# walaj/SeqLib

Hardware: AMD Instinct MI355X
Metric: aligned reads/sec (150 bp) via BWAAligner (higher is better)
Workload: dtype int32

## Files before the change

### seqlib_amd/csrc/dev_chain.h

```cpp
#pragma once
#include "dev_fm.h"
#include "dev_sort.h"
#include "dev_types.h"
#include "dev_pack.h"
#include "dev_kbtree.h"

__device__ __forceinline__ int next_slot(unsigned int *queue, int per_wave = 0)
{
    const int lane = threadIdx.x & 63;
    const unsigned int base = wave_take(queue, per_wave ? 1u : 64u);
    if (per_wave) return lane == 0 ? (int)base : 0x7fffffff;
    return (int)(base + lane);
}

struct ReadWS {
    int64_t *s_rbeg; qp_t *s_ql; int32_t *s_next; int32_t *s_score;
    int64_t *c_pos; int32_t *c_head, *c_tail, *c_n, *c_rid, *c_w, *c_first; int8_t *c_kept;
    int32_t *ia, *ib, *ic; uint64_t *srt;
    DReg *regs; DHit *hits;
    int cap;
    __device__ __forceinline__ int s_qbeg(int s) const { return QP_HI(s_ql[s]); }
    __device__ __forceinline__ int s_len(int s) const { return QP_LO(s_ql[s]); }
};

__device__ __forceinline__ ReadWS make_ws(const Chunk &ck, int r);

__device__ __forceinline__ ReadWS make_ws_uniform(const Chunk &ck, int r)
{
    const uint64_t o = rfl_u64(ck.seed_off[r]);
    ReadWS w;
    w.s_rbeg = ck.s_rbeg + o; w.s_ql = (qp_t *)ck.s_ql + o; w.s_next = ck.s_next + o; w.s_score = ck.s_score ? ck.s_score + o : nullptr;
    w.c_pos = ck.c_pos + o; w.c_head = ck.c_head + o; w.c_tail = ck.c_tail + o; w.c_n = ck.c_n + o;
    w.c_rid = ck.c_rid + o; w.c_w = ck.c_w + o; w.c_first = ck.c_first + o; w.c_kept = ck.c_kept + o;
    w.ia = ck.ia + o; w.ib = ck.ib + o; w.ic = ck.ic + o; w.srt = ck.srt + o;
    w.regs = ck.regs + o; w.hits = ck.hits + o;
    w.cap = (int)(rfl_u64(ck.seed_off[r + 1]) - o);
    return w;
}

__device__ __forceinline__ ReadWS make_ws(const Chunk &ck, int r)
{
    const uint64_t o = ck.seed_off[r];
    ReadWS w;
    w.s_rbeg = ck.s_rbeg + o; w.s_ql = (qp_t *)ck.s_ql + o; w.s_next = ck.s_next + o; w.s_score = ck.s_score ? ck.s_score + o : nullptr;
    w.c_pos = ck.c_pos + o; w.c_head = ck.c_head + o; w.c_tail = ck.c_tail + o; w.c_n = ck.c_n + o;
    w.c_rid = ck.c_rid + o; w.c_w = ck.c_w + o; w.c_first = ck.c_first + o; w.c_kept = ck.c_kept + o;
    w.ia = ck.ia + o; w.ib = ck.ib + o; w.ic = ck.ic + o; w.srt = ck.srt + o;
    w.regs = ck.regs + o; w.hits = ck.hits + o;
    w.cap = (int)(ck.seed_off[r + 1] - o);
    return w;
}

__device__ inline int dev_chain_weight(const ReadWS &w, int c)
{
    int64_t end = 0;
    int wt = 0, tmp;
    for (int s = w.c_head[c]; s >= 0; s = w.s_next[s]) {
        const int qb = w.s_qbeg(s), l = w.s_len(s);
        if (qb >= end) wt += l;
        else if (qb + l > end) wt += (int)(qb + l - end);
        end = end > qb + l ? end : qb + l;
    }
    tmp = wt; wt = 0; end = 0;
    for (int s = w.c_head[c]; s >= 0; s = w.s_next[s]) {
        const int64_t rb = w.s_rbeg[s]; const int l = w.s_len(s);
        if (rb >= end) wt += l;
        else if (rb + l > end) wt += (int)(rb + l - end);
        end = end > rb + l ? end : rb + l;
    }
    wt = wt < tmp ? wt : tmp;
    return wt < 1 << 30 ? wt : (1 << 30) - 1;
}

template <typename I>
__device__ void dev_chain_read(const DevFM<I> &fm, const DevRef &R, const Chunk &ck, const slx_opt &opt, int r)
{
        ReadWS w = make_ws(ck, r);
        const int len = (int)(ck.offs[r + 1] - ck.offs[r]);
        const int n_intv = (int)ck.intv_n[r];
        const qp_t *iinfo = (const qp_t *)ck.intv_info + (size_t)r * ck.cap_intv;
        const I *ix0 = (const I *)ck.intv_x0 + (size_t)r * ck.cap_intv;
        const I *ix2 = (const I *)ck.intv_x2 + (size_t)r * ck.cap_intv;
        int ns = 0, nc = 0;
        int *ord = w.ia;
        KbTree kb;
        bool tree = false;
        int cc = -1, cc_tail = 0, cc_n = 0, cc_rid = 0;
        qp_t cc_fql = 0, cc_lql = 0;
        int64_t cc_frb = 0, cc_lrb = 0;
        for (int i = 0; i < n_intv; ++i) {
            const int qbeg = QP_HI(iinfo[i]), slen = QP_LO(iinfo[i]) - qbeg;
            const I x2 = ix2[i];
            const I step = x2 > (I)opt.max_occ ? x2 / (I)opt.max_occ : (I)1;
            I k = 0;
            for (int count = 0; k < x2 && count < opt.max_occ; k += step, ++count) {
                const int64_t rbeg = intv_pos<I>(fm, ix0[i], k);
                const int rid = dev_intv2rid(R, rbeg, rbeg + slen);
                if (rid < 0) continue;
                int lo = -1, lower_c = -1;
                bool to_add = true;
                if (nc) {
                    if (tree) lower_c = kb.lower(rbeg);
                    else {
                        int b = 0, e = nc;
                        while (b < e) { int m = (b + e) >> 1; if (w.c_pos[ord[m]] < rbeg) b = m + 1; else e = m; }
                        if (b == nc) lo = nc - 1;
                        else lo = rbeg < w.c_pos[ord[b]] ? b - 1 : b;
                        lower_c = lo >= 0 ? ord[lo] : -1;
                    }
                    if (lower_c >= 0) {
                        const int c = lower_c;
                        if (c != cc) {
                            const int first = w.c_head[c];
                            cc = c; cc_tail = w.c_tail[c]; cc_n = w.c_n[c]; cc_rid = w.c_rid[c];
                            cc_fql = w.s_ql[first]; cc_frb = w.s_rbeg[first];
                            cc_lql = w.s_ql[cc_tail]; cc_lrb = w.s_rbeg[cc_tail];
                        }
                        const int last = cc_tail;
                        const int l_qbeg = QP_HI(cc_lql), l_len = QP_LO(cc_lql);
                        const int64_t l_rbeg = cc_lrb;
                        const int64_t qend = l_qbeg + l_len, rend = l_rbeg + l_len;
                        int res;
                        if (rid != cc_rid) res = 0;
                        else if (qbeg >= QP_HI(cc_fql) && qbeg + slen <= qend && rbeg >= cc_frb && rbeg + slen <= rend) res = 1;
                        else if ((l_rbeg < R.l_pac || cc_frb < R.l_pac) && rbeg >= R.l_pac) res = 0;
                        else {
                            const int64_t x = qbeg - l_qbeg, y = rbeg - l_rbeg;
                            if (y >= 0 && x - y <= opt.w && y - x <= opt.w && x - l_len < opt.max_chain_gap && y - l_len < opt.max_chain_gap) {
                                const int s = ns++;
                                const qp_t ql = QP_PACK(qbeg, slen);
                                w.s_rbeg[s] = rbeg; w.s_ql[s] = ql; w.s_next[s] = -1; if (w.s_score) w.s_score[s] = slen;
                                w.s_next[last] = s; w.c_tail[c] = s; w.c_n[c] = ++cc_n;
                                cc_tail = s; cc_lql = ql; cc_lrb = rbeg;
                                res = 1;
                            } else res = 0;
                        }
                        to_add = !res;
                    }
                }
                if (to_add) {
                    const int s = ns++, c = nc;
                    w.s_rbeg[s] = rbeg; w.s_ql[s] = QP_PACK(qbeg, slen); w.s_next[s] = -1; if (w.s_score) w.s_score[s] = slen;
                    w.c_pos[c] = rbeg; w.c_head[c] = w.c_tail[c] = s; w.c_n[c] = 1; w.c_rid[c] = rid;
                    cc = c; cc_tail = s; cc_n = 1; cc_rid = rid; cc_fql = cc_lql = QP_PACK(qbeg, slen); cc_frb = cc_lrb = rbeg;
                    if (!tree && nc == 2 * KB_T - 1) { kb.from_array((int *)w.regs, ord, w.c_pos, nc); tree = true; }
                    if (tree) kb.put(rbeg, c);
                    else {
                        for (int m = nc; m > lo + 1; --m) ord[m] = ord[m - 1];
                        ord[lo + 1] = c;
                    }
                    ++nc;
                }
            }
        }
        if (tree) kb.traverse(ord);
        ck.frac_rep[r] = (float)ck.l_rep[r] / len;
        int n_chn = 0;
        int *a = w.ia;
        for (int i = 0; i < nc; ++i) {
            const int c = a[i];
            w.c_first[c] = -1; w.c_kept[c] = 0;
            w.c_w[c] = dev_chain_weight(w, c);
            if (w.c_w[c] >= opt.min_chain_weight) a[n_chn++] = c;
        }
        int n_out = 0;
        if (n_chn > 0) {
            ks_introsort_idx(n_chn, a, [&](int x, int y) { return w.c_w[x] > w.c_w[y]; });
            int *kept = w.ib, n_kept = 0;
            auto cbeg = [&](int c) { return w.s_qbeg(w.c_head[c]); };
            auto cend = [&](int c) { return w.s_qbeg(w.c_tail[c]) + w.s_len(w.c_tail[c]); };
            w.c_kept[a[0]] = 3;
            kept[n_kept++] = 0;
            for (int i = 1; i < n_chn; ++i) {
                int large_ovlp = 0, k;
                const int ci = a[i];
                for (k = 0; k < n_kept; ++k) {
                    const int j = kept[k], cj = a[j];
                    const int b_max = cbeg(cj) > cbeg(ci) ? cbeg(cj) : cbeg(ci);
                    const int e_min = cend(cj) < cend(ci) ? cend(cj) : cend(ci);
                    if (e_min > b_max && (!ref_is_alt(R, w.c_rid[cj]) || ref_is_alt(R, w.c_rid[ci]))) {
                        const int li = cend(ci) - cbeg(ci), lj = cend(cj) - cbeg(cj);
                        const int min_l = li < lj ? li : lj;
                        if ((float)(e_min - b_max) >= (float)min_l * opt.mask_level && min_l < opt.max_chain_gap) {
                            large_ovlp = 1;
                            if (w.c_first[cj] < 0) w.c_first[cj] = i;
                            if ((float)w.c_w[ci] < (float)w.c_w[cj] * opt.drop_ratio && w.c_w[cj] - w.c_w[ci] >= opt.min_seed_len << 1) break;
                        }
                    }
                }
                if (k == n_kept) { kept[n_kept++] = i; w.c_kept[ci] = large_ovlp ? 2 : 3; }
            }
            for (int i = 0; i < n_kept; ++i) {
                const int c = a[kept[i]];
                if (w.c_first[c] >= 0) w.c_kept[a[w.c_first[c]]] = 1;
            }
            int i, k;
            for (i = k = 0; i < n_chn; ++i) {
                if (w.c_kept[a[i]] == 0 || w.c_kept[a[i]] == 3) continue;
                if (++k >= opt.max_chain_extend) break;
            }
            for (; i < n_chn; ++i) if (w.c_kept[a[i]] < 3) w.c_kept[a[i]] = 0;
            for (i = 0; i < n_chn; ++i) if (w.c_kept[a[i]] != 0) a[n_out++] = a[i];
        }
        const bool flt = ck.s_score && len < ck.log_lut_n && flt_live(opt, len, ck.log_lut[len > 0 ? len : 1], nullptr);
        if (n_out == 1 && opt.w > 0 && !flt) {
            const int c0 = a[0];
            int s_full = -1, cov = 0;
            bool same_diag = true;
            int64_t diag = 0;
            for (int s = w.c_head[c0]; s >= 0; s = w.s_next[s])
                if (w.s_qbeg(s) == 0 && w.s_len(s) == len) { s_full = s; diag = w.s_rbeg[s]; break; }
            if (s_full >= 0) {
                for (int s = w.c_head[c0]; s >= 0; s = w.s_next[s]) {
                    cov += w.s_len(s);
                    if (w.s_rbeg[s] - w.s_qbeg(s) != diag) same_diag = false;
                }
                if (same_diag) {
                    DReg g;
                    g.rb = diag; g.re = g.rb + len; g.qb = 0; g.qe = len; g.rid = w.c_rid[c0];
                    g.score = g.truesc = len * opt.a; g.sub = g.csub = g.sub_n = 0; g.w = opt.w; g.seedcov = cov; g.secondary = 0;
                    g.seedlen0 = len; g.n_comp = 0; g.frac_rep = ck.frac_rep[r]; g.hash = 0;
                    w.regs[0] = g;
                    ck.n_reg[r] = 1;
                    n_out = -1;
                }
            }
        }
        {
            int off = 0;
            for (int i = 0; i < n_out; ++i) {
                const int c = a[i];
                w.c_first[c] = off;
                for (int s = w.c_head[c]; s >= 0; s = w.s_next[s]) w.c_w[off++] = s;
            }
        }
        ck.n_chain[r] = n_out;
}

template <typename I>
__global__ void __launch_bounds__(128) k_chain(DevFM<I> fm, DevRef R, Chunk ck, DevOpt dopt, const int *order, unsigned int *queue, const unsigned int *n_slots, int per_wave)
{
    const slx_opt &opt = dopt.o;
    const int n_todo = (int)*n_slots;
    if (per_wave) __builtin_amdgcn_s_setprio(3);
    while (true) {
        const int slot = next_slot(queue, per_wave);
        if (__all(slot >= n_todo)) break;
        if (slot >= n_todo) continue;
        const int r = order ? order[slot] : slot;
        dev_chain_read<I>(fm, R, ck, opt, r);
    }
}
```

### seqlib_amd/csrc/dev_sort.h

```cpp
#pragma once
#include <hip/hip_runtime.h>

template <typename LT>
__device__ void ks_insertsort_idx(int *s, int *t, LT lt)
{
    for (int *i = s + 1; i < t; ++i)
        for (int *j = i; j > s && lt(*j, *(j - 1)); --j) { int sw = *j; *j = *(j - 1); *(j - 1) = sw; }
}

template <typename LT>
__device__ void ks_combsort_idx(int n, int *a, LT lt)
{
    const double shrink = 1.2473309501039786540366528676643;
    int do_swap, gap = n;
    do {
        if (gap > 2) {
            gap = (int)(gap / shrink);
            if (gap == 9 || gap == 10) gap = 11;
        }
        do_swap = 0;
        for (int *i = a; i < a + n - gap; ++i) {
            int *j = i + gap;
            if (lt(*j, *i)) { int tmp = *i; *i = *j; *j = tmp; do_swap = 1; }
        }
    } while (do_swap || gap > 2);
    if (gap != 1) ks_insertsort_idx(a, a + n, lt);
}

template <typename LT>
__device__ void ks_introsort_idx(int n, int *a, LT lt)
{
    if (n < 1) return;
    if (n == 2) {
        if (lt(a[1], a[0])) { int sw = a[0]; a[0] = a[1]; a[1] = sw; }
        return;
    }
    int d;
    for (d = 2; (1u << d) < (unsigned)n; ++d);
    int st_l[40], st_r[40], st_d[40], top = 0;
    int s = 0, t = n - 1;
    d <<= 1;
    while (true) {
        if (s < t) {
            if (--d == 0) { ks_combsort_idx(t - s + 1, a + s, lt); t = s; continue; }
            int i = s, j = t, k = i + ((j - i) >> 1) + 1;
            if (lt(a[k], a[i])) { if (lt(a[k], a[j])) k = j; }
            else k = lt(a[j], a[i]) ? i : j;
            int rp = a[k];
            if (k != t) { int sw = a[k]; a[k] = a[t]; a[t] = sw; }
            for (;;) {
                do ++i; while (lt(a[i], rp));
                do --j; while (i <= j && lt(rp, a[j]));
                if (j <= i) break;
                int sw = a[i]; a[i] = a[j]; a[j] = sw;
            }
            { int sw = a[i]; a[i] = a[t]; a[t] = sw; }
            if (i - s > t - i) {
                if (i - s > 16) { st_l[top] = s; st_r[top] = i - 1; st_d[top] = d; ++top; }
                s = t - i > 16 ? i + 1 : t;
            } else {
                if (t - i > 16) { st_l[top] = i + 1; st_r[top] = t; st_d[top] = d; ++top; }
                t = i - s > 16 ? i - 1 : s;
            }
        } else {
            if (top == 0) { ks_insertsort_idx(a, a + n, lt); return; }
            --top; s = st_l[top]; t = st_r[top]; d = st_d[top];
        }
    }
}

template <typename LT>
__device__ void std_unguarded_linear_insert(int *a, int last, LT lt)
{
    int val = a[last], next = last - 1;
    while (lt(val, a[next])) { a[last] = a[next]; last = next; --next; }
    a[last] = val;
}

template <typename LT>
__device__ void std_insertion_sort(int *a, int first, int last, LT lt)
{
    if (first == last) return;
    for (int i = first + 1; i != last; ++i) {
        if (lt(a[i], a[first])) {
            int val = a[i];
            for (int k = i; k > first; --k) a[k] = a[k - 1];
            a[first] = val;
        } else std_unguarded_linear_insert(a, i, lt);
    }
}

template <typename LT>
__device__ void std_adjust_heap(int *a, int first, int hole, int len, int value, LT lt)
{
    const int top = hole;
    int child = hole;
    while (child < (len - 1) / 2) {
        child = 2 * (child + 1);
        if (lt(a[first + child], a[first + child - 1])) --child;
        a[first + hole] = a[first + child];
        hole = child;
    }
    if ((len & 1) == 0 && child == (len - 2) / 2) {
        child = 2 * (child + 1);
        a[first + hole] = a[first + child - 1];
        hole = child - 1;
    }
    int parent = (hole - 1) / 2;
    while (hole > top && lt(a[first + parent], value)) {
        a[first + hole] = a[first + parent];
        hole = parent;
        parent = (hole - 1) / 2;
    }
    a[first + hole] = value;
}

template <typename LT>
__device__ void std_heapsort(int *a, int first, int last, LT lt)
{
    int len = last - first;
    if (len >= 2)
        for (int parent = (len - 2) / 2;; --parent) {
            std_adjust_heap(a, first, parent, len, a[first + parent], lt);
            if (parent == 0) break;
        }
    while (last - first > 1) {
        --last;
        int value = a[last];
        a[last] = a[first];
        std_adjust_heap(a, first, 0, last - first, value, lt);
    }
}

template <typename LT>
__device__ void std_sort_idx(int n, int *a, LT lt)
{
    if (n <= 0) return;
    int st_f[48], st_l[48], st_d[48], top = 0;
    int first = 0, last = n, depth = 0;
    for (int m = n; m > 1; m >>= 1) ++depth;
    depth *= 2;
    while (true) {
        while (last - first > 16) {
            if (depth == 0) { std_heapsort(a, first, last, lt); break; }
            --depth;
            int mid = first + (last - first) / 2;
            int ra = first + 1, rb = mid, rc = last - 1, res = first, pick;
            if (lt(a[ra], a[rb])) { if (lt(a[rb], a[rc])) pick = rb; else if (lt(a[ra], a[rc])) pick = rc; else pick = ra; }
            else if (lt(a[ra], a[rc])) pick = ra; else if (lt(a[rb], a[rc])) pick = rc; else pick = rb;
            { int sw = a[res]; a[res] = a[pick]; a[pick] = sw; }
            int f = first + 1, l = last;
            while (true) {
                while (lt(a[f], a[first])) ++f;
                --l;
                while (lt(a[first], a[l])) --l;
                if (!(f < l)) break;
                int sw = a[f]; a[f] = a[l]; a[l] = sw;
                ++f;
            }
            int cut = f;
            st_f[top] = cut; st_l[top] = last; st_d[top] = depth; ++top;
            last = cut;
        }
        if (top == 0) break;
        --top; first = st_f[top]; last = st_l[top]; depth = st_d[top];
    }
    if (n > 16) {
        std_insertion_sort(a, 0, 16, lt);
        for (int i = 16; i < n; ++i) std_unguarded_linear_insert(a, i, lt);
    } else std_insertion_sort(a, 0, n, lt);
}
```

### seqlib_amd/csrc/slx_align.hip

```cpp
#include <hip/hip_runtime.h>
#include <hipcub/hipcub.hpp>
#include <chrono>
#include <cmath>
#include <functional>
#include <unistd.h>
#include <cstdio>
#include <cstdlib>
#include <cstring>
#include <algorithm>
#include <mutex>
#include <string>
#include <thread>
#include <type_traits>
#include <vector>
#include "slx_internal.h"
#include "dev_seed4.h"
#include "dev_fin.h"
#include "dev_ext_wave.h"
#include "dev_ext_reg.h"
#include "dev_ext_lane.h"
#include "dev_ext_block.h"
#include "dev_ext_seg.h"
#include "dev_fin2.h"
#include "dev_chain_coop.h"
#include "dev_long.h"
#include "dev_cig_lane.h"
#include "dev_cig_band.h"
#include "dev_cig_seg.h"

#include "slx_align_types.h"

static const char *STAGE_NAMES[SLX_N_STAGES] = {"encode", "seed", "scan", "chain", "extend", "finalize", "compact", "total"};
extern "C" const char *slx_stage_name(int i) { return i >= 0 && i < SLX_N_STAGES ? STAGE_NAMES[i] : ""; }

#define SLX_BOUNCE_BYTES (256u << 10)
#define SLX_PACK_PARTS 13
struct PackSpec { const unsigned char *src[SLX_PACK_PARTS]; unsigned int bytes[SLX_PACK_PARTS], at[SLX_PACK_PARTS]; int n; long long hdr[4]; };
__global__ void k_pack_small(PackSpec s, unsigned char *dst)
{
    const unsigned int t = blockIdx.x * blockDim.x + threadIdx.x, nt = gridDim.x * blockDim.x;
    if (t < 32 && s.hdr[0] >= 0) dst[t] = ((const unsigned char *)s.hdr)[t];
    for (int i = 0; i < s.n; ++i)
        for (unsigned int b = t; b < s.bytes[i]; b += nt) dst[s.at[i] + b] = s.src[i][b];
}

__global__ void k_len_stats(const uint64_t *offs, int n, unsigned long long *stat)
{
    const int i = blockIdx.x * blockDim.x + threadIdx.x;
    unsigned long long len = 0;
    bool bad = false;
    if (i < n) {
        const uint64_t a = offs[i], b = offs[i + 1];
        if (b < a) bad = true; else len = b - a;
        if (i == 0) stat[2] = a;
        if (i == n - 1) stat[3] = b;
    }
    for (int o = 32; o; o >>= 1) { const unsigned long long t = __shfl_xor(len, o, 64); len = len > t ? len : t; }
    if ((threadIdx.x & 63) == 0 && len > __hip_atomic_load(stat, __ATOMIC_RELAXED, __HIP_MEMORY_SCOPE_AGENT)) atomicMax(stat, len);
    if (bad) atomicOr(stat + 1, 1ull);
}

template <typename I>
__global__ void k_sa_seed(DevFM<I> fm, I *dense, uint64_t n_sa)
{
    uint64_t j = (uint64_t)blockIdx.x * blockDim.x + threadIdx.x;
    if (j >= n_sa) return;
    dense[j * (uint64_t)fm.sa_intv] = j == 0 ? fm.seq_len : (I)fm.sa_samp[j];
}

template <typename I>
__global__ void k_sa_walk(DevFM<I> fm, I *dense, uint64_t n_sa)
{
    uint64_t j = (uint64_t)blockIdx.x * blockDim.x + threadIdx.x;
    if (j >= n_sa) return;
    I k = (I)(j * (uint64_t)fm.sa_intv);
    I v = j == 0 ? fm.seq_len : (I)fm.sa_samp[j];
    const I mask = (I)fm.sa_intv - 1;
    while (true) {
        if (k == fm.primary) break;
        I x = k - (k > fm.primary ? 1 : 0);
        const uint32_t *blk = fm.bwt + ((size_t)(x >> 7) << 4) + 8;
        int jj = (int)(x & 127);
        int c = (blk[jj >> 4] >> ((~jj & 15) << 1)) & 3;
        I tk[4], tl[4];
        occ4_pair<I>(fm, k, k, tk, tl);
        k = fm.L2[c] + tk[c];
        --v;
        if ((k & mask) == 0) break;
        dense[k] = v;
    }
}

template <typename I>
static int build_lut(slx_aligner *al)
{
    DevFM<I> &fm = fm_of<I>(al);
    fm.lut = nullptr; fm.lut_k = 0;
    int K = al->lut_k;
    if (K < 0) {
        int l4 = 0;
        while ((al->host_idx->seq_len >> (2 * (l4 + 1))) != 0) ++l4;
        K = l4 - 1 > 14 ? 14 : l4 - 1;
    }
    if (K < 2) return SLX_OK;
    const uint64_t n = 1ull << (2 * K);
    int rc;
    if ((rc = al->d_lut.ensure(n * sizeof(LutE<I>))) != SLX_OK) return rc;
    hipLaunchKernelGGL(k_kmer_lut<I>, dim3((unsigned)((n + 255) / 256)), dim3(256), 0, al->stream, fm, K, al->d_lut.as<LutE<I>>());
    HIPCHK(hipGetLastError());
    HIPCHK(slx_wait_stream(al->stream));
    fm.lut = al->d_lut.p; fm.lut_k = K;
    return SLX_OK;
}

template <typename I>
static int upload_fm(slx_aligner *al)
{
    const slx_index *idx = al->host_idx;
    int rc;
    DevFM<I> &fm = fm_of<I>(al);
    memset(&fm, 0, sizeof fm);
    fm.bwt = al->d_bwt.as<uint32_t>();
    {
        const uint64_t n_blocks = ((idx->seq_len ? idx->seq_len - 1 : 0) >> 6) + 1;
        const size_t occ_bytes = (n_blocks + 1) * 32;
        if ((rc = al->d_occ.ensure(occ_bytes)) != SLX_OK) return rc;
        HIPCHK(hipMemsetAsync(al->d_occ.p, 0, occ_bytes, al->stream));
        const uint64_t *sup = nullptr;
        if (sizeof(I) == 8) {
            const uint64_t n_sup = (idx->seq_len >> 32) + 1;
            if ((rc = al->d_sup.ensure(n_sup * 32 + 32)) != SLX_OK) return rc;
            hipLaunchKernelGGL(k_occ_sup, dim3((unsigned)((n_sup * 4 + 63) / 64)), dim3(64), 0, al->stream, al->d_bwt.as<uint32_t>(), n_sup, al->d_sup.as<uint64_t>());
            sup = al->d_sup.as<uint64_t>();
        }
        hipLaunchKernelGGL(k_occ_build, dim3((unsigned)((n_blocks + 255) / 256)), dim3(256), 0, al->stream, al->d_bwt.as<uint32_t>(), (uint64_t)idx->seq_len,
                           al->d_occ.as<uint4>(), n_blocks, sup);
        HIPCHK(hipGetLastError());
        HIPCHK(slx_wait_stream(al->stream));
        fm.occ = al->d_occ.as<uint4>();
        fm.sup = sup;
    }
    fm.primary = (I)idx->primary;
    for (int i = 0; i < 5; ++i) fm.L2[i] = (I)idx->L2[i];
    fm.seq_len = (I)idx->seq_len;
    if ((rc = build_lut<I>(al)) != SLX_OK) return rc;
    fm.sa_dense = nullptr;
    fm.sa_samp = al->d_sa_samp.as<uint64_t>();
    fm.sa_intv = idx->sa_intv;
    const uint64_t n1 = idx->seq_len + 1;
    al->have_dense = false;
    if ((rc = al->d_sa_dense.ensure(n1 * sizeof(I))) != SLX_OK) return rc;
    if (sizeof(I) == 4 && idx->dense_sa32.size() == n1) {
        HIPCHK(hipMemcpy(al->d_sa_dense.p, idx->dense_sa32.data(), n1 * 4, hipMemcpyHostToDevice));
    } else {
        const uint64_t n_sa = idx->sa.size();
        const int bs = 256;
        hipLaunchKernelGGL(k_sa_seed<I>, dim3((unsigned)((n_sa + bs - 1) / bs)), dim3(bs), 0, al->stream, fm, al->d_sa_dense.as<I>(), n_sa);
        hipLaunchKernelGGL(k_sa_walk<I>, dim3((unsigned)((n_sa + bs - 1) / bs)), dim3(bs), 0, al->stream, fm, al->d_sa_dense.as<I>(), n_sa);
        HIPCHK(hipGetLastError());
        HIPCHK(slx_wait_stream(al->stream));
    }
    al->have_dense = true;
    return SLX_OK;
}

template <typename I>
static int build_rep_filter(slx_aligner *al)
{
    al->rep_mask = 0;
    if (al->rep_k <= 0 || al->rep_k > 31 || !al->have_dense || al->host_idx->seq_len < 1024) return SLX_OK;
    uint64_t bits = 1ull << 20;
    while (bits < al->host_idx->seq_len * 8ull) bits <<= 1;
    while (al->d_rep.ensure(bits / 8) != SLX_OK) {
        (void)hipGetLastError();
        bits >>= 1;
        if (bits < al->host_idx->seq_len || bits < (1ull << 20)) { al->d_rep.release(); return SLX_OK; }
    }
    HIPCHK(hipMemsetAsync(al->d_rep.p, 0, bits / 8, al->stream));
    DevFM<I> fm = fm_of<I>(al);
    fm.sa_dense = al->d_sa_dense.as<I>();
    hipLaunchKernelGGL(k_rep_filter<I>, dim3(al->n_cu * 64), dim3(256), 0, al->stream, fm, al->ref, al->rep_k, al->d_rep.as<uint32_t>(), bits - 1);
    HIPCHK(hipGetLastError());
    HIPCHK(slx_wait_stream(al->stream));
    al->rep_mask = bits - 1;
    return SLX_OK;
}

#define SLX_MAX_WORKERS 8
static int env_hw_queues() { const char *e = getenv("GPU_MAX_HW_QUEUES"); const int v = e ? atoi(e) : 0; return v > 0 ? v : 4; }

static int default_workers()
{
    if (const char *e = getenv("SEQLIB_AMD_WORKERS")) { const int v = atoi(e); if (v >= 1 && v <= SLX_MAX_WORKERS) return v; }
    return 3;
}

static int make_worker_stream(slx_aligner *al, Worker *wk)
{
    if (al->stream_prio) {
        int least = 0, greatest = 0;
        HIPCHK(hipDeviceGetStreamPriorityRange(&least, &greatest));
        HIPCHK(hipStreamCreateWithPriority(&wk->stream, hipStreamNonBlocking, greatest));
    } else HIPCHK(hipStreamCreateWithFlags(&wk->stream, hipStreamNonBlocking));
    return SLX_OK;
}

static int set_seed_stream(slx_aligner *al, Worker *wk)
{
    if (wk->seed_stream) { HIPCHK(slx_wait_stream(wk->seed_stream)); HIPCHK(hipStreamDestroy(wk->seed_stream)); wk->seed_stream = nullptr; }
    if (al->seed_free_cus <= 0) return SLX_OK;
    const int words = (al->n_cu + 31) / 32;
    std::vector<uint32_t> mask((size_t)words, 0u);
    for (int cu = 0; cu < al->n_cu; ++cu)
        if ((cu & 31) < 32 - al->seed_free_cus) mask[(size_t)(cu >> 5)] |= 1u << (cu & 31);
    HIPCHK(hipExtStreamCreateWithCUMask(&wk->seed_stream, (uint32_t)words, mask.data()));
    if (!wk->ev_seed_in) HIPCHK(hipEventCreateWithFlags(&wk->ev_seed_in, hipEventDisableTiming));
    if (!wk->ev_seed_out) HIPCHK(hipEventCreateWithFlags(&wk->ev_seed_out, hipEventDisableTiming));
    return SLX_OK;
}

static int add_worker(slx_aligner *al)
{
    Worker *wk = new Worker();
    wk->id = (int)al->workers.size();
    wk->collect();
    al->workers.push_back(wk);
    { const int rc = make_worker_stream(al, wk); if (rc != SLX_OK) return rc; }
    { const int rc = set_seed_stream(al, wk); if (rc != SLX_OK) return rc; }
    HIPCHK(hipHostMalloc((void **)&wk->h_mail, 256, hipHostMallocDefault));
    for (int b = 0; b < 6; ++b) HIPCHK(hipEventCreate(&wk->dbg_ev[b]));
    for (int i = 0; i <= SLX_N_STAGES; ++i) HIPCHK(hipEventCreate(&wk->ev[i]));
    for (int i = 0; i < 6; ++i) HIPCHK(hipEventCreate(&wk->ev_probe[i]));
    return SLX_OK;
}

static int aligner_init(slx_aligner *al, const slx_index *idx, const int *devices, int n_dev)
{
    al->device = (devices && n_dev > 0) ? devices[0] : 0;
    if (!(devices && n_dev > 0)) (void)hipGetDevice(&al->device);
    HIPCHK(hipSetDevice(al->device));
    hipDeviceProp_t prop;
    HIPCHK(hipGetDeviceProperties(&prop, al->device));
    al->n_cu = prop.multiProcessorCount;
    al->max_threads = al->n_cu * al->threads_per_cu;
    int rcw;
    al->n_workers = default_workers();
    al->hw_queues = env_hw_queues();
    for (int k = 0; k < al->n_workers; ++k) if ((rcw = add_worker(al)) != SLX_OK) return rcw;
    HIPCHK(hipStreamCreateWithFlags(&al->stream, hipStreamNonBlocking));
    al->host_idx = idx;
    int rc;
    if ((rc = al->d_bwt.ensure(idx->bwt.size() * 4 + 64)) != SLX_OK) return rc;
    HIPCHK(hipMemcpy(al->d_bwt.p, idx->bwt.data(), idx->bwt.size() * 4, hipMemcpyHostToDevice));
    if ((rc = al->d_sa_samp.ensure(idx->sa.size() * 8)) != SLX_OK) return rc;
    HIPCHK(hipMemcpy(al->d_sa_samp.p, idx->sa.data(), idx->sa.size() * 8, hipMemcpyHostToDevice));
    al->wide = idx->seq_len + 1 >= (1ULL << 32);
    if ((rc = al->wide ? upload_fm<uint64_t>(al) : upload_fm<uint32_t>(al)) != SLX_OK) return rc;
    if ((rc = al->d_pac.ensure(idx->pac.size() + 16)) != SLX_OK) return rc;
    HIPCHK(hipMemcpy(al->d_pac.p, idx->pac.data(), idx->pac.size(), hipMemcpyHostToDevice));
    std::vector<int64_t> aoff; std::vector<int32_t> alen;
    for (const slx_ann &a : idx->anns) { aoff.push_back(a.offset); alen.push_back(a.len); }
    if ((rc = al->d_ann_off.ensure(aoff.size() * 8 + 8)) != SLX_OK) return rc;
    if ((rc = al->d_ann_len.ensure(alen.size() * 4 + 8)) != SLX_OK) return rc;
    HIPCHK(hipMemcpy(al->d_ann_off.p, aoff.data(), aoff.size() * 8, hipMemcpyHostToDevice));
    HIPCHK(hipMemcpy(al->d_ann_len.p, alen.data(), alen.size() * 4, hipMemcpyHostToDevice));
    al->ref.pac = al->d_pac.as<uint8_t>();
    al->ref.l_pac = idx->l_pac;
    al->ref.n_seqs = (int)idx->anns.size();
    al->ref.ann_off = al->d_ann_off.as<int64_t>();
    al->ref.ann_len = al->d_ann_len.as<int32_t>();
    {
        std::vector<uint8_t> alt;
        bool any = false;
        for (const slx_ann &a : idx->anns) { alt.push_back(a.is_alt ? 1 : 0); any = any || a.is_alt; }
        al->ref.ann_alt = nullptr;
        if (any) {
            if ((rc = al->d_ann_alt.ensure(alt.size() + 8)) != SLX_OK) return rc;
            HIPCHK(hipMemcpy(al->d_ann_alt.p, alt.data(), alt.size(), hipMemcpyHostToDevice));
            al->ref.ann_alt = al->d_ann_alt.as<uint8_t>();
        }
    }
    if ((rc = al->wide ? build_rep_filter<uint64_t>(al) : build_rep_filter<uint32_t>(al)) != SLX_OK) return rc;
    const int LUT_N = SLX_LOG_LUT_N;
    std::vector<double> lut((size_t)LUT_N);
    lut[0] = -INFINITY;
    for (int i = 1; i < LUT_N; ++i) lut[(size_t)i] = log((double)i);
    if ((rc = al->d_loglut.ensure((size_t)LUT_N * 8)) != SLX_OK) return rc;
    HIPCHK(hipMemcpy(al->d_loglut.p, lut.data(), (size_t)LUT_N * 8, hipMemcpyHostToDevice));
    return SLX_OK;
}


static std::mutex g_live_mu;
static int g_live_aligners = 0;
static void pin_pool_release_all();

static int create_one(const slx_index *idx, int device, bool current, slx_aligner **out)
{
    slx_aligner *al = new slx_aligner();
    { std::lock_guard<std::mutex> g(g_live_mu); ++g_live_aligners; }
    const int rc = aligner_init(al, idx, current ? nullptr : &device, current ? 0 : 1);
    if (rc != SLX_OK) { slx_aligner_free(al); return rc; }
    *out = al;
    return SLX_OK;
}

extern "C" int slx_device_count(void)
{
    int ndev = 0;
    if (hipGetDeviceCount(&ndev) != hipSuccess) { (void)hipGetLastError(); return 0; }
    return ndev;
}

extern "C" int slx_aligner_create(const slx_index *idx, const int *devices, int n_dev, slx_aligner **out)
{
    if (!out) return SLX_EINVAL;
    *out = nullptr;
    if (!idx) { slx_set_error("slx_aligner_create: index is null"); return SLX_EINVAL; }
    const int ndev = slx_device_count();
    if (ndev == 0) {
        slx_set_error("no HIP device: the BWAAligner hot path runs on MI355X only (no CPU fallback)");
        return SLX_ENODEVICE;
    }
    if (n_dev < 0 || (n_dev > 0 && !devices)) { slx_set_error("slx_aligner_create: bad device list"); return SLX_EINVAL; }
    for (int i = 0; i < n_dev; ++i)
        if (devices[i] < 0 || devices[i] >= ndev) { slx_set_error("slx_aligner_create: device %d is not one of the %d visible", devices[i], ndev); return SLX_EINVAL; }
    if (n_dev <= 1) return create_one(idx, n_dev ? devices[0] : 0, n_dev == 0, out);
    slx_aligner *grp = new slx_aligner();
    grp->is_group = true;
    grp->subs.assign((size_t)n_dev, nullptr);
    grp->host_idx = idx;
    std::vector<int> rcs((size_t)n_dev, SLX_OK);
    std::vector<std::string> errs((size_t)n_dev);
    std::vector<std::thread> th;
    for (int i = 0; i < n_dev; ++i)
        th.emplace_back([&, i]() {
            rcs[(size_t)i] = create_one(idx, devices[i], false, &grp->subs[(size_t)i]);
            if (rcs[(size_t)i] != SLX_OK) errs[(size_t)i] = slx_last_error();
        });
    for (auto &t : th) t.join();
    for (int i = 0; i < n_dev; ++i)
        if (rcs[(size_t)i] != SLX_OK) {
            slx_set_error("device %d: %s", devices[i], errs[(size_t)i].c_str());
            const int rc = rcs[(size_t)i];
            slx_aligner_free(grp);
            return rc;
        }
    *out = grp;
    return SLX_OK;
}

extern "C" void slx_aligner_free(slx_aligner *al)
{
    if (!al) return;
    if (al->is_group) {
        for (slx_aligner *sub : al->subs) slx_aligner_free(sub);
        delete al;
        return;
    }
    (void)hipSetDevice(al->device);
    DevBuf *bufs[] = {&al->d_bwt, &al->d_occ, &al->d_sup, &al->d_lut, &al->d_rep, &al->d_sa_samp, &al->d_sa_dense, &al->d_pac, &al->d_ann_off, &al->d_ann_len, &al->d_ann_alt, &al->d_loglut, &al->o_hit_off,
                      &al->o_rid, &al->o_pos, &al->o_flag, &al->o_mapq, &al->o_score, &al->o_nm, &al->o_na, &al->o_ncig, &al->o_cig_off, &al->o_cigar, &al->o_xa, &al->o_sub,
                      &al->st_bases, &al->st_offs, &al->st_pack};
    for (DevBuf *b : bufs) b->release();
    for (Worker *wk : al->workers) {
        for (DevBuf *b : wk->all) b->release();
        for (int i = 0; i <= SLX_N_STAGES; ++i) if (wk->ev[i]) (void)hipEventDestroy(wk->ev[i]);
        for (int i = 0; i < 6; ++i) if (wk->dbg_ev[i]) (void)hipEventDestroy(wk->dbg_ev[i]);
        for (int i = 0; i < 6; ++i) if (wk->ev_probe[i]) (void)hipEventDestroy(wk->ev_probe[i]);
        if (wk->h_mail) (void)hipHostFree(wk->h_mail);
        if (wk->stream) (void)hipStreamDestroy(wk->stream);
        if (wk->seed_stream) (void)hipStreamDestroy(wk->seed_stream);
        if (wk->ev_seed_in) (void)hipEventDestroy(wk->ev_seed_in);
        if (wk->ev_seed_out) (void)hipEventDestroy(wk->ev_seed_out);
        delete wk;
    }
    if (al->h_bounce) (void)hipHostFree(al->h_bounce);
    if (al->stream) (void)hipStreamDestroy(al->stream);
    delete al;
    bool last;
    { std::lock_guard<std::mutex> g(g_live_mu); last = --g_live_aligners == 0; }
    if (last) pin_pool_release_all();
}

extern "C" int slx_aligner_set(slx_aligner *al, const char *key, int64_t value)
{
    if (!al || !key) return SLX_EINVAL;
    if (al->is_group) {
        std::lock_guard<std::mutex> call(al->call_mu);
        for (slx_aligner *sub : al->subs) { const int rc = slx_aligner_set(sub, key, value); if (rc != SLX_OK) return rc; }
        return SLX_OK;
    }
    std::lock_guard<std::mutex> call(al->call_mu);
    if (!strcmp(key, "chunk_reads")) { if (value < 1) return SLX_EINVAL; al->chunk_reads = value; }
    else if (!strcmp(key, "cap_intv")) { if (value < 1) return SLX_EINVAL; al->cap_intv = (int)value; }
    else if (!strcmp(key, "dense_sa")) al->dense_sa = value != 0;
    else if (!strcmp(key, "wide_index")) {
        const bool want = value != 0 || al->host_idx->seq_len + 1 >= (1ULL << 32);
        if (want != al->wide) {
            HIPCHK(hipSetDevice(al->device));
            al->wide = want;
            int rc = want ? upload_fm<uint64_t>(al) : upload_fm<uint32_t>(al);
            if (rc != SLX_OK) return rc;
            if ((rc = want ? build_rep_filter<uint64_t>(al) : build_rep_filter<uint32_t>(al)) != SLX_OK) return rc;
        }
    }
    else if (!strcmp(key, "chain_mode")) al->chain_mode = (int)value;
    else if (!strcmp(key, "keep_stages")) al->keep_stages = (int)value;
    else if (!strcmp(key, "lut_k")) {
        if (value != 0 && value != -1 && (value < 2 || value > 14)) return SLX_EINVAL;
        al->lut_k = (int)value;
        (void)hipSetDevice(al->device);
        return al->wide ? build_lut<uint64_t>(al) : build_lut<uint32_t>(al);
    }
    else if (!strcmp(key, "cand_mode")) al->cand_mode = (int)value;
    else if (!strcmp(key, "cand_seeds")) { if (value < 1) return SLX_EINVAL; al->cand_seeds = (int)value; }
    else if (!strcmp(key, "heavy_sorted")) al->heavy_sorted = (int)value;
    else if (!strcmp(key, "ext_split")) al->ext_split = (int)value;
    else if (!strcmp(key, "coop_lim1")) { if (value < 1) return SLX_EINVAL; al->coop_lim1 = (int)value; }
    else if (!strcmp(key, "coop_lim2")) { if (value < 1) return SLX_EINVAL; al->coop_lim2 = (int)value; }
    else if (!strcmp(key, "long_coop")) al->long_coop = value != 0;
    else if (!strcmp(key, "long_seed3")) al->long_seed3 = value != 0;
    else if (!strcmp(key, "long_predict")) al->long_predict = value != 0;
    else if (!strcmp(key, "long_block")) { if (value < 0 || value > (1 << 24)) return SLX_EINVAL; al->long_block = (int)value; }
    else if (!strcmp(key, "long_guess")) al->long_guess = value != 0;
    else if (!strcmp(key, "long_seg")) al->long_seg = value != 0;
    else if (!strcmp(key, "bwd_direct")) al->bwd_direct = value != 0;
    else if (!strcmp(key, "xseg_wave_min")) { if (value < 0) return SLX_EINVAL; al->xseg_wave_min = (int)value; }
    else if (!strcmp(key, "xseg_fail")) { if (value < 0) return SLX_EINVAL; al->xseg_fail = (int)value; }
    else if (!strcmp(key, "long_budget")) { if (value < 0 || value > (1 << 20)) return SLX_EINVAL; al->long_budget = (int)value; }
    else if (!strcmp(key, "regs_big")) { if (value < 2) return SLX_EINVAL; al->regs_big = (int)value; }
    else if (!strcmp(key, "regs_defer")) al->regs_defer = value != 0;
    else if (!strcmp(key, "hits_wave")) al->hits_wave = value != 0;
    else if (!strcmp(key, "cig_fast_coop")) al->cig_fast_coop = value != 0;
    else if (!strcmp(key, "cig_lane_il")) al->cig_lane_il = value != 0;
    else if (!strcmp(key, "small_coop")) al->small_coop = value != 0;
    else if (!strcmp(key, "small_spread")) al->small_spread = value != 0;
    else if (!strcmp(key, "chain_sorted")) al->chain_sorted = value != 0;
    else if (!strcmp(key, "regs_sorted")) al->regs_sorted = value != 0;
    else if (!strcmp(key, "cand_top")) { if (value < 0) return SLX_EINVAL; al->cand_top = (int)value; }
    else if (!strcmp(key, "cand_rep_max")) { if (value < 0) return SLX_EINVAL; al->cand_rep_max = (int)value; }
    else if (!strcmp(key, "cand_rep")) { if (value < -1 || value > 101) return SLX_EINVAL; al->cand_rep = (int)value; }
    else if (!strcmp(key, "cand_lanes")) { if (value < -1 || value > 1) return SLX_EINVAL; al->cand_lanes = (int)value; }
    else if (!strcmp(key, "cig_lanes")) al->cig_lanes = value != 0;
    else if (!strcmp(key, "first_diag")) al->first_diag = value != 0;
    else if (!strcmp(key, "first_lanes")) al->first_lanes = value != 0;
    else if (!strcmp(key, "lane_narrow")) al->lane_narrow = value != 0;
    else if (!strcmp(key, "lane_pad")) al->lane_pad = (int)value;
    else if (!strcmp(key, "cand_lane_seeds")) { if (value < 1) return SLX_EINVAL; al->cand_lane_seeds = (int)value; }
    else if (!strcmp(key, "cand_cap")) { if (value < 1) return SLX_EINVAL; al->cand_cap = (int)value; }
    else if (!strcmp(key, "split_min")) al->split_min = (int)value;
    else if (!strcmp(key, "heavy_seeds")) { if (value < 1) return SLX_EINVAL; al->heavy_seeds = (int)value; }
    else if (!strcmp(key, "workers")) {
        if (value < 1 || value > SLX_MAX_WORKERS) return SLX_EINVAL;
        HIPCHK(hipSetDevice(al->device));
        while ((int)al->workers.size() < (int)value) { const int rc = add_worker(al); if (rc != SLX_OK) return rc; }
        al->n_workers = (int)value;
    }
    else if (!strcmp(key, "min_split")) { if (value < 1) return SLX_EINVAL; al->min_split = value; }
    else if (!strcmp(key, "seed_quota")) { if (value < 0 || value > (1 << 24)) return SLX_EINVAL; al->seed_quota = (int)value; }
    else if (!strcmp(key, "rep_k")) {
        if (value < 0 || value > 31) return SLX_EINVAL;
        al->rep_k = (int)value;
        HIPCHK(hipSetDevice(al->device));
        return al->wide ? build_rep_filter<uint64_t>(al) : build_rep_filter<uint32_t>(al);
    }
    else if (!strcmp(key, "top_heavy")) al->top_heavy = value != 0;
    else if (!strcmp(key, "top_reuse")) al->top_reuse = value != 0;
    else if (!strcmp(key, "p2_items")) al->p2_items = value != 0;
    else if (!strcmp(key, "p2_coop")) al->p2_coop = value != 0;
    else if (!strcmp(key, "p2_items_cap")) al->p2_items_cap = (int)value;
    else if (!strcmp(key, "seed_free_cus")) {
        if (value < 0 || value > 24) return SLX_EINVAL;
        HIPCHK(hipSetDevice(al->device));
        al->seed_free_cus = (int)value;
        for (Worker *wk : al->workers) { const int rc = set_seed_stream(al, wk); if (rc != SLX_OK) return rc; }
    }
    else if (!strcmp(key, "stream_prio")) {
        if (value < 0 || value > 1) return SLX_EINVAL;
        HIPCHK(hipSetDevice(al->device));
        al->stream_prio = (int)value;
        for (Worker *wk : al->workers) {
            HIPCHK(slx_wait_stream(wk->stream));
            HIPCHK(hipStreamDestroy(wk->stream));
            wk->stream = nullptr;
            const int rc = make_worker_stream(al, wk);
            if (rc != SLX_OK) return rc;
        }
    }
    else if (!strcmp(key, "threads")) { if (value < 64) return SLX_EINVAL; al->max_threads = (int)value; }
    else if (!strcmp(key, "zarena_bytes")) { if (value < 1024) return SLX_EINVAL; al->zcap = (unsigned long long)value; }
    else { slx_set_error("slx_aligner_set: unknown key %s", key); return SLX_EINVAL; }
    return SLX_OK;
}

extern "C" int slx_aligner_stage_ms(const slx_aligner *al, float ms[SLX_N_STAGES])
{
    if (!al || !ms) return SLX_EINVAL;
    if (al->is_group) {
        for (int i = 0; i < SLX_N_STAGES; ++i) { ms[i] = 0; for (const slx_aligner *sub : al->subs) ms[i] = std::max(ms[i], sub->stage_ms[i]); }
        return SLX_OK;
    }
    for (int i = 0; i < SLX_N_STAGES; ++i) ms[i] = al->stage_ms[i];
    return SLX_OK;
}

extern "C" int slx_aligner_probe_ms(const slx_aligner *al, float ms[SLX_N_PROBES], int64_t *n_reads)
{
    if (!al || !ms) return SLX_EINVAL;
    if (al->is_group) {
        int64_t n = 0;
        for (int i = 0; i < SLX_N_PROBES; ++i) ms[i] = 0;
        for (const slx_aligner *sub : al->subs) { for (int i = 0; i < SLX_N_PROBES; ++i) ms[i] += sub->probe_ms[i]; n += sub->probe_reads; }
        if (n_reads) *n_reads = n;
        return SLX_OK;
    }
    for (int i = 0; i < SLX_N_PROBES; ++i) ms[i] = al->probe_ms[i];
    if (n_reads) *n_reads = al->probe_reads;
    return SLX_OK;
}

extern "C" int64_t slx_aligner_counter(const slx_aligner *al, const char *key)
{
    if (!al || !key) return -1;
    if (!strcmp(key, "workers")) return al->is_group ? al->subs[0]->n_workers : al->n_workers;
    if (!strcmp(key, "hw_queues")) return al->hw_queues;
    if (!strcmp(key, "long_rounds") || !strcmp(key, "long_jobs")) {
        long long v = 0;
        const bool rounds = key[5] == 'r';
        auto take = [&](const slx_aligner *a) { for (const Worker *wk : a->workers) v = std::max(v, rounds ? (long long)wk->long_rounds_run : (long long)wk->long_jobs_run); };
        if (al->is_group) for (const slx_aligner *sub : al->subs) take(sub); else take(al);
        return v;
    }
    {
        if (!strcmp(key, "pseg_jobs")) {
            long long v = 0;
            auto take = [&](const slx_aligner *a) { for (const Worker *wk : a->workers) v += wk->pseg_stat; };
            if (al->is_group) for (const slx_aligner *sub : al->subs) take(sub); else take(al);
            return v;
        }
        if (!strcmp(key, "retries")) {
            long long v = 0;
            if (al->is_group) for (const slx_aligner *sub : al->subs) v += sub->n_retries; else v = al->n_retries;
            return v;
        }
        if (!strcmp(key, "regs_deferred") || !strcmp(key, "hits_wave_reads")) {
            long long v = 0;
            const int which = key[0] == 'h';
            auto take = [&](const slx_aligner *a) { for (const Worker *wk : a->workers) v += (long long)wk->fin_stat[which]; };
            if (al->is_group) for (const slx_aligner *sub : al->subs) take(sub); else take(al);
            return v;
        }
        static const char *const gs[3] = {"gseg_ok", "gseg_redo", "gseg_jobs"};
        for (int i = 0; i < 3; ++i)
            if (!strcmp(key, gs[i])) {
                long long v = 0;
                auto take = [&](const slx_aligner *a) { for (const Worker *wk : a->workers) v += wk->gseg_stat[i]; };
                if (al->is_group) for (const slx_aligner *sub : al->subs) take(sub); else take(al);
                return v;
            }
        static const char *const xs[4] = {"xseg_ok", "xseg_redo", "xseg_retry", "xseg_sides"};
        for (int i = 0; i < 4; ++i)
            if (!strcmp(key, xs[i])) {
                long long v = 0;
                auto take = [&](const slx_aligner *a) { for (const Worker *wk : a->workers) v += wk->xseg_stat[i]; };
                if (al->is_group) for (const slx_aligner *sub : al->subs) take(sub); else take(al);
                return v;
            }
    }
    if (!strcmp(key, "group_merge_us")) return al->merge_us;
    if (!strcmp(key, "group_call_us")) return al->call_us;
    static const char *const names[4] = {"heavy_reads", "p2_calls", "p2_coop_calls", "p2_whole_reads"};
    for (int i = 0; i < 4; ++i)
        if (!strcmp(key, names[i])) {
            if (!al->is_group) return al->counters[i];
            long long n = 0;
            for (const slx_aligner *sub : al->subs) n += sub->counters[i];
            return n;
        }
    return -1;
}

extern "C" int slx_aligner_probe_launches(const slx_aligner *al)
{
    if (!al) return 0;
    if (al->is_group) { int n = 0; for (const slx_aligner *sub : al->subs) n += sub->probe_launches; return n; }
    return al->probe_launches;
}

#include "slx_chunk.inc"


__global__ void k_shift_offsets(int64_t *dst, const int64_t *src, int64_t n, int64_t add)
{
    int64_t i = (int64_t)blockIdx.x * blockDim.x + threadIdx.x;
    if (i < n) dst[i] = src[i] + add;
}

template <typename I>
static int worker_run(slx_aligner *al, Worker *wk, const slx_opt *opt, const uint8_t *d_bases, const uint64_t *d_offs, int64_t r_lo, int64_t r_hi,
                      uint64_t rng_state, uint64_t first_ordinal, int hardclip, double keepSecFrac, int maxSecondary, const char *h_bases, const uint64_t *h_offs)
{
    HIPCHK(hipSetDevice(al->device));
    if (h_offs && r_hi > r_lo) {
        const uint64_t b0 = h_offs[r_lo], b1 = h_offs[r_hi];
        if (b0 < al->h_first || b1 < b0 || b1 > al->h_last) { slx_set_error("read offsets are not monotonic (part [%lld, %lld))", (long long)r_lo, (long long)r_hi); return SLX_EINVAL; }
        if (b1 > b0) HIPCHK(hipMemcpyAsync((void *)(d_bases + b0), h_bases + b0, b1 - b0, hipMemcpyHostToDevice, wk->stream));
        HIPCHK(hipMemcpyAsync((void *)(d_offs + r_lo), h_offs + r_lo, ((size_t)(r_hi - r_lo) + 1) * 8, hipMemcpyHostToDevice, wk->stream));
    }
    for (int i = 0; i < SLX_N_STAGES; ++i) wk->stage_ms[i] = 0;
    for (int i = 0; i < SLX_N_PROBES; ++i) wk->probe_ms[i] = 0;
    wk->n_chunks = 0;
    for (long long &c : wk->cnt) c = 0;
    int rc;
    const int64_t n_part = r_hi - r_lo;
    if ((rc = wk->o_hit_off.ensure(((size_t)n_part + 1) * 8)) != SLX_OK) return rc;
    if ((rc = wk->len_stat.ensure(32)) != SLX_OK) return rc;
    int64_t hit_base = 0, cig_base = 0;
    for (int64_t r0 = r_lo, step = 0; r0 < r_hi; r0 += step) {
        const int n = (int)std::min<int64_t>(al->chunk_reads, r_hi - r0);
        step = n;
        unsigned long long stat[4] = {0, 0, 0, 0};
        HIPCHK(hipMemsetAsync(wk->len_stat.p, 0, 32, wk->stream));
        hipLaunchKernelGGL(k_len_stats, dim3((unsigned)((n + 255) / 256)), dim3(256), 0, wk->stream, d_offs + r0, n, wk->len_stat.as<unsigned long long>());
        { MailSpec ms{}; ms.src[0] = wk->len_stat.as<unsigned int>(); ms.words[0] = 8; ms.n = 1;
          hipLaunchKernelGGL(k_mail, dim3(1), dim3(64), 0, wk->stream, ms, wk->h_mail); }
        HIPCHK(slx_wait_stream(wk->stream));
        memcpy(stat, wk->h_mail, 32);
        if (stat[1]) { slx_set_error("read offsets are not monotonic in reads [%lld, %lld)", (long long)r0, (long long)(r0 + n)); return SLX_EINVAL; }
        const int max_len = (int)std::min<unsigned long long>(stat[0], 1u << 30);
        if (max_len > SLX_MAX_READ_LEN) {
            slx_set_error("read of %d bp: the GPU path supports reads up to %d bp", max_len, SLX_MAX_READ_LEN);
            return SLX_EUNSUPPORTED;
        }
        uint64_t pair[2] = {stat[2], stat[3]};
        ChunkCaps caps;
        {
            std::lock_guard<std::mutex> g(al->mu);
            caps.cap_intv = al->cap_intv;
            caps.zcap = std::max<unsigned long long>(al->zcap, (unsigned long long)n * al->z_per_read);
            if (max_len > 704) {
                caps.cap_intv = std::max(std::max(caps.cap_intv, al->cap_intv_long), max_len / 8 + 64);
                caps.zcap = std::max(caps.zcap, std::min<unsigned long long>((unsigned long long)n * (unsigned long long)max_len * 208ull, 4ull << 30));
            }
            caps.cigcap = std::max<unsigned long long>(al->cig_floor, (unsigned long long)n * al->cig_per_read + 4096);
        }
        const unsigned long long lane_blocks = (unsigned long long)std::min<long long>((long long)al->n_cu * 16, (long long)n * 4 / 64 + 1);
        const unsigned long long z_waves = (unsigned long long)std::min(n, al->n_cu * 32) * CIG_WAVE_Z +
                                           (al->cig_lane_il ? lane_blocks * ((unsigned long long)LANE_IL_WORDS(max_len) * 256ull + 255ull) : 0ull);
        const unsigned long long cig_waves = (unsigned long long)std::min(n, al->n_cu * 32) * CIG_WAVE_WORDS;
        caps.zcap += z_waves; caps.cigcap += cig_waves;
        for (int attempt = 0;; ++attempt) {
            uint32_t fl = 0;
            int64_t hb = hit_base, cb = cig_base;
            if (max_len > SLX_NARROW_MAX_LEN)
                rc = sizeof(I) == 8 ? slx_run_chunk_wide_u64(al, wk, opt, d_bases, d_offs, pair, r0, r_lo, n, max_len, rng_state, first_ordinal, hardclip, keepSecFrac, maxSecondary,
                                                             caps, &hb, &cb, &fl)
                                    : slx_run_chunk_wide_u32(al, wk, opt, d_bases, d_offs, pair, r0, r_lo, n, max_len, rng_state, first_ordinal, hardclip, keepSecFrac, maxSecondary,
                                                             caps, &hb, &cb, &fl);
            else
            rc = run_chunk<I>(al, wk, opt, d_bases, d_offs, pair, r0, r_lo, n, max_len, rng_state, first_ordinal, hardclip, keepSecFrac, maxSecondary,
                              caps, &hb, &cb, &fl);
            if (rc != SLX_OK) return rc;
            if (!fl) {
                hit_base = hb; cig_base = cb;
                ++wk->n_chunks;
                std::lock_guard<std::mutex> g(al->mu);
                if (max_len > 704) al->cap_intv_long = std::max(al->cap_intv_long, caps.cap_intv);
                else al->cap_intv = std::max(al->cap_intv, caps.cap_intv);
                if (attempt > 0) {
                    if (n >= 65536) {
                        al->z_per_read = std::max<unsigned long long>(al->z_per_read, (caps.zcap - z_waves + n - 1) / (unsigned long long)n);
                        al->cig_per_read = std::max<unsigned long long>(al->cig_per_read, (caps.cigcap - cig_waves + n - 1) / (unsigned long long)n);
                    } else {
                        al->zcap = std::max(al->zcap, caps.zcap - z_waves);
                        al->cig_floor = std::max(al->cig_floor, caps.cigcap - cig_waves);
                    }
                }
                al->n_retries += attempt;
                break;
            }
            if (getenv("SLX_DEBUG_RETRY")) fprintf(stderr, "[retry] worker %d reads %lld+%d attempt %d flags 0x%x (cap_intv %d zcap %llu cigcap %llu)\n", wk->id,
                                                   (long long)r0, n, attempt, fl, caps.cap_intv, caps.zcap, caps.cigcap);
            if (fl & (ERR_LOGLUT | ERR_INTERNAL)) { slx_set_error("device pipeline error flags 0x%x", fl); return SLX_EINTERNAL; }
            if (attempt >= 12) { slx_set_error("chunk still overflows its work areas after %d retries (flags 0x%x)", attempt, fl); return SLX_ENOMEM; }
            if (fl & OVF_INTV) caps.cap_intv *= 2;
            if (fl & OVF_ZARENA) caps.zcap *= 2;
            if (fl & OVF_CIGAR) caps.cigcap *= 2;
        }
    }
    {
        int64_t last[1] = {hit_base};
        HIPCHK(hipMemcpyAsync(wk->o_hit_off.as<int64_t>() + n_part, last, 8, hipMemcpyHostToDevice, wk->stream));
        if ((rc = wk->o_cig_off.grow(((size_t)hit_base + 2) * 8, (size_t)hit_base * 8, wk->stream)) != SLX_OK) return rc;
        int64_t lastc[1] = {cig_base};
        HIPCHK(hipMemcpyAsync(wk->o_cig_off.as<int64_t>() + hit_base, lastc, 8, hipMemcpyHostToDevice, wk->stream));
        HIPCHK(slx_wait_stream(wk->stream));
    }
    wk->n_hits = hit_base; wk->n_cig = cig_base;
    return SLX_OK;
}

struct EventPair {
    hipEvent_t t0 = nullptr, t1 = nullptr;
    ~EventPair() { if (t0) (void)hipEventDestroy(t0); if (t1) (void)hipEventDestroy(t1); }
};

static int align_device_locked(slx_aligner *al, const slx_opt *opt, const void *d_bases, const void *d_offs_, int64_t n_reads,
                               uint64_t rng_state, uint64_t first_ordinal, int hardclip, double keepSecFrac, int maxSecondary, slx_hits *out,
                               const char *h_bases = nullptr, const uint64_t *h_offs = nullptr)
{
    memset(out, 0, sizeof *out);
    HIPCHK(hipSetDevice(al->device));
    if (opt->e_del <= 0 || opt->e_ins <= 0) { slx_set_error("gap extension penalty must be > 0 on the GPU path (bwa divides by it)"); return SLX_EINVAL; }
    const uint64_t *d_offs = (const uint64_t *)d_offs_;
    const int K = (n_reads >= 2 * al->min_split) ? std::min<int>(al->n_workers, (int)al->workers.size()) : 1;
    al->active_k = K;
    EventPair tp;
    HIPCHK(hipEventCreate(&tp.t0)); HIPCHK(hipEventCreate(&tp.t1));
    HIPCHK(hipEventRecord(tp.t0, al->stream));
    HIPCHK(slx_wait_stream(al->stream));
    std::vector<int64_t> lo((size_t)K + 1);
    for (int k = 0; k <= K; ++k) lo[(size_t)k] = n_reads * k / K;
    const bool wide = al->wide;
    const bool sam = (opt->flag & SLX_F_REG2SAM) != 0;
    auto run_worker = [=](Worker *wk, int64_t a, int64_t b) {
        return wide ? worker_run<uint64_t>(al, wk, opt, (const uint8_t *)d_bases, d_offs, a, b, rng_state, first_ordinal, hardclip, keepSecFrac, maxSecondary, h_bases, h_offs)
                    : worker_run<uint32_t>(al, wk, opt, (const uint8_t *)d_bases, d_offs, a, b, rng_state, first_ordinal, hardclip, keepSecFrac, maxSecondary, h_bases, h_offs);
    };
    if (K == 1) {
        Worker *wk = al->workers[0];
        wk->rc = run_worker(wk, 0, n_reads);
        if (wk->rc != SLX_OK) return wk->rc;
    } else {
        std::vector<std::thread> th;
        for (int k = 0; k < K; ++k) {
            Worker *wk = al->workers[(size_t)k];
            const int64_t a = lo[(size_t)k], b = lo[(size_t)k + 1];
            th.emplace_back([=]() {
                wk->rc = run_worker(wk, a, b);
                if (wk->rc != SLX_OK) wk->err = slx_last_error();
            });
        }
        for (auto &t : th) t.join();
        for (int k = 0; k < K; ++k)
            if (al->workers[(size_t)k]->rc != SLX_OK) { slx_set_error("%s", al->workers[(size_t)k]->err.c_str()); return al->workers[(size_t)k]->rc; }
    }
    for (int i = 0; i < SLX_N_STAGES; ++i) {
        al->stage_ms[i] = 0;
        for (int k = 0; k < K; ++k) al->stage_ms[i] += al->workers[(size_t)k]->stage_ms[i];
    }
    al->probe_reads = n_reads;
    al->probe_launches = 0;
    for (int k = 0; k < K; ++k) al->probe_launches += al->workers[(size_t)k]->n_chunks;
    for (int i = 0; i < 4; ++i) { al->counters[i] = 0; for (int k = 0; k < K; ++k) al->counters[i] += al->workers[(size_t)k]->cnt[i]; }
    for (int i = 0; i < SLX_N_PROBES; ++i) {
        al->probe_ms[i] = 0;
        for (int k = 0; k < K; ++k) al->probe_ms[i] += al->workers[(size_t)k]->probe_ms[i];
    }
    slx_hits r;
    memset(&r, 0, sizeof r);
    r.n_reads = n_reads; r.on_device = 1;
    if (K == 1) {
        Worker *wk = al->workers[0];
        r.n_hits = wk->n_hits; r.n_cigar = wk->n_cig;
        r.hit_off = wk->o_hit_off.as<int64_t>(); r.rid = wk->o_rid.as<int32_t>(); r.pos = wk->o_pos.as<int64_t>();
        r.flag = wk->o_flag.as<uint16_t>(); r.mapq = wk->o_mapq.as<uint8_t>(); r.score = wk->o_score.as<int32_t>();
        r.nm = wk->o_nm.as<int32_t>(); r.na = wk->o_na.as<int32_t>(); r.n_cigar_ops = wk->o_ncig.as<int32_t>();
        r.cig_off = wk->o_cig_off.as<int64_t>(); r.cigar = wk->o_cigar.as<uint32_t>();
        if (sam) { r.xa_parent = wk->o_xa.as<int32_t>(); r.sub = wk->o_sub.as<int32_t>(); }
    } else {
        int64_t H = 0, C = 0;
        for (int k = 0; k < K; ++k) { H += al->workers[(size_t)k]->n_hits; C += al->workers[(size_t)k]->n_cig; }
        int rc;
#define ENSO(buf, bytes) if ((rc = al->buf.ensure((size_t)(bytes))) != SLX_OK) return rc
        ENSO(o_hit_off, ((size_t)n_reads + 1) * 8); ENSO(o_rid, ((size_t)H + 1) * 4); ENSO(o_pos, ((size_t)H + 1) * 8); ENSO(o_flag, ((size_t)H + 1) * 2);
        ENSO(o_mapq, (size_t)H + 1); ENSO(o_score, ((size_t)H + 1) * 4); ENSO(o_nm, ((size_t)H + 1) * 4); ENSO(o_na, ((size_t)H + 1) * 4);
        ENSO(o_ncig, ((size_t)H + 1) * 4); ENSO(o_cig_off, ((size_t)H + 2) * 8); ENSO(o_cigar, ((size_t)C + 1) * 4);
        if (sam) { ENSO(o_xa, ((size_t)H + 1) * 4); ENSO(o_sub, ((size_t)H + 1) * 4); }
#undef ENSO
        int64_t hb = 0, cb = 0;
        hipStream_t st = al->stream;
        for (int k = 0; k < K; ++k) {
            Worker *wk = al->workers[(size_t)k];
            const int64_t np = lo[(size_t)k + 1] - lo[(size_t)k], h = wk->n_hits, c = wk->n_cig;
            const int last = k == K - 1 ? 1 : 0;
            hipLaunchKernelGGL(k_shift_offsets, dim3((unsigned)((np + last + 255) / 256)), dim3(256), 0, st, al->o_hit_off.as<int64_t>() + lo[(size_t)k],
                               wk->o_hit_off.as<int64_t>(), np + last, hb);
            hipLaunchKernelGGL(k_shift_offsets, dim3((unsigned)((h + last + 255) / 256)), dim3(256), 0, st, al->o_cig_off.as<int64_t>() + hb,
                               wk->o_cig_off.as<int64_t>(), h + last, cb);
#define CAT(buf, type, cnt, base) if ((cnt) > 0) HIPCHK(hipMemcpyAsync(al->buf.as<type>() + (base), wk->buf.as<type>(), (size_t)(cnt) * sizeof(type), hipMemcpyDeviceToDevice, st))
            CAT(o_rid, int32_t, h, hb); CAT(o_pos, int64_t, h, hb); CAT(o_flag, uint16_t, h, hb); CAT(o_mapq, uint8_t, h, hb); CAT(o_score, int32_t, h, hb);
            CAT(o_nm, int32_t, h, hb); CAT(o_na, int32_t, h, hb); CAT(o_ncig, int32_t, h, hb); CAT(o_cigar, uint32_t, c, cb);
            if (sam) { CAT(o_xa, int32_t, h, hb); CAT(o_sub, int32_t, h, hb); }
#undef CAT
            hb += h; cb += c;
        }
        HIPCHK(hipGetLastError());
        r.n_hits = H; r.n_cigar = C;
        r.hit_off = al->o_hit_off.as<int64_t>(); r.rid = al->o_rid.as<int32_t>(); r.pos = al->o_pos.as<int64_t>();
        r.flag = al->o_flag.as<uint16_t>(); r.mapq = al->o_mapq.as<uint8_t>(); r.score = al->o_score.as<int32_t>();
        r.nm = al->o_nm.as<int32_t>(); r.na = al->o_na.as<int32_t>(); r.n_cigar_ops = al->o_ncig.as<int32_t>();
        r.cig_off = al->o_cig_off.as<int64_t>(); r.cigar = al->o_cigar.as<uint32_t>();
        if (sam) { r.xa_parent = al->o_xa.as<int32_t>(); r.sub = al->o_sub.as<int32_t>(); }
    }
    HIPCHK(hipEventRecord(tp.t1, al->stream));
    HIPCHK(slx_wait_stream(al->stream));
    float tot = 0;
    (void)hipEventElapsedTime(&tot, tp.t0, tp.t1);
    al->stage_ms[7] = tot;
    *out = r;
    return SLX_OK;
}

extern "C" int slx_align_batch_device(slx_aligner *al, const slx_opt *opt, const void *d_bases, const void *d_offs, int64_t n_reads,
                                      uint64_t rng_state, uint64_t first_ordinal, int hardclip, double keepSecFrac, int maxSecondary,
                                      slx_hits *out)
{
    if (!al || !opt || !out || n_reads < 0) { slx_set_error("slx_align_batch_device: bad argument"); return SLX_EINVAL; }
    if (al->is_group) { slx_set_error("slx_align_batch_device: reads resident on one GPU cannot be sharded -- use one aligner per device, or slx_align_batch"); return SLX_EINVAL; }
    std::lock_guard<std::mutex> call(al->call_mu);
    return align_device_locked(al, opt, d_bases, d_offs, n_reads, rng_state, first_ordinal, hardclip, keepSecFrac, maxSecondary, out);
}

namespace {
struct PinBlock { void *p; uint64_t cap; };
std::mutex g_pin_mu;
std::vector<PinBlock> g_pin_pool;
const size_t PIN_KEEP = 4;
const uint64_t PIN_KEEP_BYTES = 8ull << 30;
void *pin_acquire(uint64_t bytes, uint64_t *cap)
{
    {
        std::lock_guard<std::mutex> g(g_pin_mu);
        size_t best = g_pin_pool.size();
        for (size_t i = 0; i < g_pin_pool.size(); ++i)
            if (g_pin_pool[i].cap >= bytes && (best == g_pin_pool.size() || g_pin_pool[i].cap < g_pin_pool[best].cap)) best = i;
        if (best < g_pin_pool.size()) { void *p = g_pin_pool[best].p; *cap = g_pin_pool[best].cap; g_pin_pool.erase(g_pin_pool.begin() + (long)best); return p; }
    }
    void *p = nullptr;
    const uint64_t want = bytes + bytes / 16;
    if (hipHostMalloc(&p, want, hipHostMallocPortable | hipHostMallocMapped) != hipSuccess) { (void)hipGetLastError(); return nullptr; }
    *cap = want;
    return p;
}
void pin_release(void *p, uint64_t cap)
{
    {
        std::lock_guard<std::mutex> g(g_pin_mu);
        uint64_t held = cap;
        for (const PinBlock &b : g_pin_pool) held += b.cap;
        bool alive;
        { std::lock_guard<std::mutex> g2(g_live_mu); alive = g_live_aligners > 0; }
        if (alive && g_pin_pool.size() < PIN_KEEP && held <= PIN_KEEP_BYTES) { g_pin_pool.push_back({p, cap}); return; }
    }
    (void)hipHostFree(p);
}
}
static void pin_pool_release_all()
{
    std::vector<PinBlock> drop;
    { std::lock_guard<std::mutex> g(g_pin_mu); drop.swap(g_pin_pool); }
    for (const PinBlock &b : drop) (void)hipHostFree(b.p);
}

extern "C" void *slx_host_alloc(uint64_t bytes)
{
    void *p = nullptr;
    if (hipHostMalloc(&p, bytes ? bytes : 1, hipHostMallocDefault) != hipSuccess) { (void)hipGetLastError(); slx_set_error("cannot pin %llu bytes of host memory", (unsigned long long)bytes); return nullptr; }
    return p;
}
extern "C" void slx_host_free(void *p) { if (p) (void)hipHostFree(p); }
extern "C" void slx_host_trim(void) { pin_pool_release_all(); }

static uint64_t packed_base(uint64_t N, uint64_t H, uint64_t Cg) { return 32 + 8 * (N + 1) + 8 * H + 8 * (H + 1) + 5 * 4 * H + 4 * Cg + 2 * H + H; }
static uint64_t packed_size(uint64_t N, uint64_t H, uint64_t Cg, bool sam = false) { const uint64_t b = packed_base(N, H, Cg); return sam ? ((b + 3) & ~3ull) + 8 * H : b; }

static int pack_locked(slx_aligner *al, const slx_hits *h, void *dst);

static void view_packed(slx_hits *out, uint8_t *blk, int64_t N, int64_t H, int64_t C, bool sam = false)
{
    uint8_t *d = blk + 32;
    out->hit_off = (int64_t *)d; d += 8 * ((size_t)N + 1);
    out->pos = (int64_t *)d; d += 8 * (size_t)H;
    out->cig_off = (int64_t *)d; d += 8 * ((size_t)H + 1);
    out->rid = (int32_t *)d; d += 4 * (size_t)H;
    out->score = (int32_t *)d; d += 4 * (size_t)H;
    out->nm = (int32_t *)d; d += 4 * (size_t)H;
    out->na = (int32_t *)d; d += 4 * (size_t)H;
    out->n_cigar_ops = (int32_t *)d; d += 4 * (size_t)H;
    out->cigar = (uint32_t *)d; d += 4 * (size_t)C;
    out->flag = (uint16_t *)d; d += 2 * (size_t)H;
    out->mapq = (uint8_t *)d;
    out->xa_parent = out->sub = nullptr;
    if (sam) {
        uint8_t *e = blk + ((packed_base((uint64_t)N, (uint64_t)H, (uint64_t)C) + 3) & ~3ull);
        out->xa_parent = (int32_t *)e; out->sub = (int32_t *)(e + 4 * (size_t)H);
    }
}

static int align_host_locked(slx_aligner *al, const slx_opt *opt, const char *bases, const uint64_t *offs, int64_t n_reads, uint64_t rng_state,
                             uint64_t first_ordinal, int hardclip, double keepSecFrac, int maxSecondary, slx_hits *dv);

static int group_align_batch(slx_aligner *grp, const slx_opt *opt, const char *bases, const uint64_t *offs, int64_t n_reads, uint64_t rng_state,
                             uint64_t first_ordinal, int hardclip, double keepSecFrac, int maxSecondary, slx_hits *out)
{
    std::lock_guard<std::mutex> call(grp->call_mu);
    const auto t_call = std::chrono::steady_clock::now();
    const int G = (int)grp->subs.size();
    std::vector<int64_t> lo((size_t)G + 1);
    for (int g = 0; g <= G; ++g) lo[(size_t)g] = n_reads * g / G;
    std::vector<slx_hits> part((size_t)G);
    std::vector<int> rcs((size_t)G, SLX_OK);
    std::vector<std::string> errs((size_t)G);
    for (auto &h : part) memset(&h, 0, sizeof h);
    auto on_all = [&](const std::function<int(int)> &fn) {
// ... 275 lines not shown
```

### seqlib_amd/csrc/slx_align_types.h

```cpp
#pragma once
#include <hip/hip_runtime.h>
#include <mutex>
#include <string>
#include <vector>
#include "slx_internal.h"
#include "dev_fm.h"
#include "dev_types.h"

#define HIPCHK(x)                                                                                   \
    do {                                                                                            \
        hipError_t e_ = (x);                                                                        \
        if (e_ != hipSuccess) {                                                                     \
            slx_set_error("HIP error %s at %s:%d (%s)", hipGetErrorString(e_), __FILE__, __LINE__, #x); \
            return e_ == hipErrorOutOfMemory ? SLX_ENOMEM : SLX_ENODEVICE;                          \
        }                                                                                           \
    } while (0)

struct DevBuf {
    void *p = nullptr;
    size_t cap = 0;
    int ensure(size_t bytes)
    {
        if (bytes <= cap) return SLX_OK;
        if (p) (void)hipFree(p);
        p = nullptr; cap = 0;
        size_t want = bytes + bytes / 8 + 256;
        HIPCHK(hipMalloc(&p, want));
        cap = want;
        return SLX_OK;
    }
    int grow(size_t bytes, size_t keep, hipStream_t st)
    {
        if (bytes <= cap) return SLX_OK;
        void *q = nullptr;
        size_t want = bytes + bytes / 2 + 256;
        HIPCHK(hipMalloc(&q, want));
        if (p && keep) {
            hipError_t e = hipMemcpyAsync(q, p, keep, hipMemcpyDeviceToDevice, st);
            if (e == hipSuccess) e = hipStreamSynchronize(st);
            if (e != hipSuccess) { (void)hipFree(q); HIPCHK(e); }
        }
        if (p) (void)hipFree(p);
        p = q; cap = want;
        return SLX_OK;
    }
    void release() { if (p) (void)hipFree(p); p = nullptr; cap = 0; }
    template <typename T> T *as() const { return (T *)p; }
};

#define SLX_MAIL_PARTS 6
struct MailSpec { const unsigned int *src[SLX_MAIL_PARTS]; int words[SLX_MAIL_PARTS]; int n; };
static __global__ void k_mail(MailSpec s, unsigned int *dst)
{
    int at = 0;
    for (int i = 0; i < s.n; ++i) {
        for (int w = (int)threadIdx.x; w < s.words[i]; w += (int)blockDim.x) dst[at + w] = s.src[i][w];
        at += s.words[i];
    }
}
struct slx_aligner;
#define SMALL_SPREAD_MAX 512

struct Worker {
    hipStream_t stream = nullptr;
    hipStream_t seed_stream = nullptr;
    hipEvent_t ev_seed_in = nullptr, ev_seed_out = nullptr;
    unsigned int *h_mail = nullptr;
    DevBuf codes, offs_rel, intv_n, intv_info, intv_x0, intv_x2, l_rep, seed_cnt, seed_off, scan_tmp;
    DevBuf s_rbeg, s_ql, s_next, c_pos, c_head, c_tail, c_n, c_rid, c_w, c_first, c_kept, ia, ib, ic, srt, regs, hits;
    DevBuf n_chain, n_reg, n_hit, na, frac_rep, zarena, cigpool, counters, lists, hit_cnt, cig_cnt, hit_off_c, cig_off_c;
    DevBuf order_key_in, order_key_out, order_in, order_out, queues, sort_tmp, jobs, fast_list, dp_list, part_flag, part_pos, cand, cand_base,
        cand_cnt, cand_off, dbg_cyc, order_tmp, first_tab, first_cnt, first_off, fb_list, first_jobs, len_stat, s_score, long_list, long_scratch, huge_rows;
    DevBuf order_bin, bin_cnt;
    DevBuf defer_list, hits_big;
    DevBuf first_sorted, first_bins;
    DevBuf p2mask, p2list, p2items, p2long, lane_jobs, first_dp, cig_lane_list;
    DevBuf job_key_in, job_key_out, job_val_in, job_val_out, job_sort_tmp;
    DevBuf seed3_buf;
    DevBuf memo_idx, memo_jobs, memo_tab, round_list, todo_a, todo_b, spec_cnt;
    int long_rounds_run = 0; unsigned int long_jobs_run = 0;
    DevBuf xseg_jobs, xseg_state, xseg_units, xseg_out, xseg_wrec, xseg_wout, xseg_scratch, xseg_cnt;
    DevBuf gseg_jobs, gseg_units, gseg_wrec, gseg_wout, gseg_scratch, gseg_cnt;
    DevBuf pseg_jobs, pseg_idx, pseg_cnt;
    unsigned long long fin_stat[2] = {0, 0};
    unsigned int pseg_stat = 0;
    unsigned int gseg_stat[3] = {0, 0, 0};
    unsigned int xseg_stat[4] = {0, 0, 0, 0};
    DevBuf snap_ia, snap_regs, snap_nreg;
    Chunk last_ck;
    size_t last_S1 = 0;
    bool last_valid = false, last_wide = false;
    int id = 0;
    unsigned int max_seed_cnt = 0;
    hipEvent_t dbg_ev[6] = {nullptr, nullptr, nullptr, nullptr, nullptr, nullptr};
    DevBuf o_hit_off, o_rid, o_pos, o_flag, o_mapq, o_score, o_nm, o_na, o_ncig, o_cig_off, o_cigar, o_xa, o_sub;
    hipEvent_t ev[SLX_N_STAGES + 1];
    hipEvent_t ev_probe[6] = {nullptr, nullptr, nullptr, nullptr, nullptr, nullptr};
    float stage_ms[SLX_N_STAGES];
    float probe_ms[SLX_N_PROBES] = {0, 0, 0, 0, 0, 0};
    int n_chunks = 0;
    long long cnt[4] = {0, 0, 0, 0};
    int64_t n_hits = 0, n_cig = 0;
    int rc = SLX_OK;
    std::string err;
    std::vector<DevBuf *> all;
    void collect()
    {
        all = {&codes, &offs_rel, &intv_n, &intv_info, &intv_x0, &intv_x2, &l_rep, &seed_cnt, &seed_off, &scan_tmp, &s_rbeg, &s_ql, &s_next,
               &c_pos, &c_head, &c_tail, &c_n, &c_rid, &c_w, &c_first, &c_kept, &ia, &ib, &ic, &srt, &regs, &hits, &n_chain, &n_reg, &n_hit,
               &na, &frac_rep, &zarena, &cigpool, &counters, &lists, &hit_cnt, &cig_cnt, &hit_off_c, &cig_off_c, &order_key_in,
               &order_key_out, &order_in, &order_out, &queues, &sort_tmp, &jobs, &fast_list, &dp_list, &part_flag, &part_pos, &cand, &cand_base,
               &cand_cnt, &cand_off, &dbg_cyc, &order_tmp, &first_tab, &first_cnt, &first_off, &fb_list, &first_jobs, &len_stat, &s_score, &long_list, &long_scratch, &huge_rows, &p2mask, &p2list, &p2items, &p2long, &lane_jobs, &first_dp, &first_sorted, &first_bins, &cig_lane_list, &defer_list, &hits_big, &order_bin, &bin_cnt, &snap_ia, &snap_regs, &snap_nreg,
               &memo_idx, &memo_jobs, &memo_tab, &round_list, &todo_a, &todo_b, &spec_cnt, &seed3_buf, &job_key_in, &job_key_out, &job_val_in, &job_val_out, &job_sort_tmp, &pseg_jobs, &pseg_idx, &pseg_cnt, &gseg_jobs, &gseg_units, &gseg_wrec, &gseg_wout, &gseg_scratch, &gseg_cnt, &xseg_jobs, &xseg_state, &xseg_units, &xseg_out, &xseg_wrec, &xseg_wout, &xseg_scratch, &xseg_cnt,
               &o_hit_off, &o_rid, &o_pos, &o_flag, &o_mapq, &o_score, &o_nm, &o_na, &o_ncig, &o_cig_off, &o_cigar, &o_xa, &o_sub};
        for (auto &e : ev) e = nullptr;
    }
};

struct slx_aligner {
    std::vector<slx_aligner *> subs;
    bool is_group = false;
    int64_t merge_us = 0, call_us = 0;
    int device = 0;
    hipStream_t stream = nullptr;
    DevBuf d_bwt, d_occ, d_sup, d_lut, d_rep, d_sa_samp, d_sa_dense, d_pac, d_ann_off, d_ann_len, d_ann_alt, d_loglut;
    uint64_t rep_mask = 0;
    int rep_k = 19;
    bool wide = false;
    DevFM<uint32_t> fm32;
    DevFM<uint64_t> fm64;
    DevRef ref;
    bool dense_sa = true;
    bool have_dense = false;
    const slx_index *host_idx = nullptr;
    int64_t chunk_reads = 1 << 24;
    int cap_intv = 40;
    int cap_intv_long = 0;
    int long_predict = 0;
    int long_block = 32768;
    int long_seed3 = 1;
    int long_coop = 1;
    int bwd_direct = 0;
    int long_seg = 1;
    int xseg_wave_min = 2048;
    int xseg_fail = 0;
    int long_guess = 0;
    int long_budget = 1024;
    int regs_sorted = 0;
    int chain_sorted = 0;
    int small_spread = 1;
    int cig_fast_coop = 1;
    int cig_lane_il = 1;
    int hits_wave = 1;
    int small_coop = 1;
    int regs_defer = 1;
    int regs_big = 48;
    int coop_lim1 = 1 << 30, coop_lim2 = 1 << 30;
    int ext_split = 1;
    int heavy_sorted = 1;
    int cand_lanes = -1;
    int cand_lane_seeds = 64;
    int cig_lanes = 1;
    int first_lanes = 1;
    int first_diag = 1;
    int lane_narrow = 1;
    int lane_pad = 0;
    int cand_mode = 1;
    int cand_seeds = 256;
    int cand_top = 512;
    int cand_rep = -1;
    int cand_rep_max = 4096;
    int cand_cap = 1 << 23;
    int lut_k = -1;
    int keep_stages = 0;
    int chain_mode = 1;
    int heavy_seeds = 64;
    int split_min = 4096;
    int seed_quota = 0;
    int top_heavy = 0;
    int p2_items = 1;
    int p2_coop = 1;
    int p2_items_cap = 0;
    int top_reuse = 1;
    int seed_free_cus = 0;
    int stream_prio = 0;
    int n_workers = 3;
    int hw_queues = 4;
    int active_k = 1;
    int64_t min_split = 1 << 18;
    int max_threads = 0;
    int threads_per_cu = 1536;
    int n_cu = 256;
    unsigned long long zcap = 1ull << 26;
    unsigned long long z_per_read = 512;
    unsigned long long cig_per_read = 8;
    unsigned long long cig_floor = 0;
    int n_retries = 0;
    std::mutex mu;
    std::mutex call_mu;
    std::vector<Worker *> workers;
    DevBuf o_hit_off, o_rid, o_pos, o_flag, o_mapq, o_score, o_nm, o_na, o_ncig, o_cig_off, o_cigar, o_xa, o_sub;
    DevBuf st_bases, st_offs, st_pack;
    unsigned char *h_bounce = nullptr;
    float stage_ms[SLX_N_STAGES];
    float probe_ms[SLX_N_PROBES] = {0, 0, 0, 0, 0, 0};
    int64_t probe_reads = 0;
    long long counters[4] = {0, 0, 0, 0};
    int probe_launches = 0;
    uint64_t h_first = 0, h_last = 0;
};

template <typename I> static DevFM<I> &fm_of(slx_aligner *al);
template <> DevFM<uint32_t> &fm_of<uint32_t>(slx_aligner *al) { return al->fm32; }
template <> DevFM<uint64_t> &fm_of<uint64_t>(slx_aligner *al) { return al->fm64; }

struct ChunkCaps { int cap_intv; unsigned long long zcap, cigcap; };

#define SLX_LOG_LUT_N (1 << 21)
#define SLX_NARROW_MAX_LEN 65000

int slx_run_chunk_wide_u32(slx_aligner *al, Worker *wk, const slx_opt *opt, const uint8_t *d_ascii, const uint64_t *d_offs, const uint64_t *h_offs_pair,
                           int64_t r0, int64_t part_lo, int n, int max_len, uint64_t rng_state, uint64_t first_ordinal, int hardclip, double ksf, int maxsec,
                           const ChunkCaps &caps, int64_t *hit_base, int64_t *cig_base, uint32_t *flags_out);
int slx_run_chunk_wide_u64(slx_aligner *al, Worker *wk, const slx_opt *opt, const uint8_t *d_ascii, const uint64_t *d_offs, const uint64_t *h_offs_pair,
                           int64_t r0, int64_t part_lo, int n, int max_len, uint64_t rng_state, uint64_t first_ordinal, int hardclip, double ksf, int maxsec,
                           const ChunkCaps &caps, int64_t *hit_base, int64_t *cig_base, uint32_t *flags_out);
```

### seqlib_amd/csrc/slx_chunk.inc

```

__device__ __forceinline__ uint32_t nt4_of(uint32_t b)
{
    const uint32_t u = b & 0xDFu;
    const uint32_t x = (b >> 1) & 3u;
    const bool letter = u == 'A' || u == 'C' || u == 'G' || u == 'T';
    return b < 4u ? b : (letter ? (x ^ (x >> 1)) : 4u);
}

__global__ void k_encode(const uint8_t *ascii, uint8_t *codes, size_t n)
{
    const size_t n16 = (n + 15) >> 4;
    const size_t stride = (size_t)gridDim.x * blockDim.x;
    const bool aligned = ((uintptr_t)ascii & 3) == 0;
    for (size_t t = (size_t)blockIdx.x * blockDim.x + threadIdx.x; t < n16; t += stride) {
        const size_t i = t << 4;
        uint32_t w[4];
        if (aligned && i + 16 <= n) {
            const uint32_t *src = (const uint32_t *)(ascii + i);
#pragma unroll
            for (int k = 0; k < 4; ++k) w[k] = src[k];
        } else {
#pragma unroll
            for (int k = 0; k < 4; ++k) {
                w[k] = 0;
// ... 174 lines not shown
    return sort_keys_largest_first(wk, st, n);
}

static bool sort_keys_largest_first(Worker *wk, hipStream_t st, unsigned int n)
{
    if (wk->job_key_in.ensure((size_t)n * 4) != SLX_OK || wk->job_key_out.ensure((size_t)n * 4) != SLX_OK || wk->job_val_in.ensure((size_t)n * 4) != SLX_OK ||
        wk->job_val_out.ensure((size_t)n * 4) != SLX_OK) return false;
    size_t tb = 0;
    if (hipcub::DeviceRadixSort::SortPairsDescending(nullptr, tb, wk->job_key_in.as<unsigned int>(), wk->job_key_out.as<unsigned int>(), wk->job_val_in.as<unsigned int>(),
                                                     wk->job_val_out.as<unsigned int>(), (int)n, 0, 32, st) != hipSuccess) return false;
    if (wk->job_sort_tmp.ensure(tb + 256) != SLX_OK) return false;
    return hipcub::DeviceRadixSort::SortPairsDescending(wk->job_sort_tmp.p, tb, wk->job_key_in.as<unsigned int>(), wk->job_key_out.as<unsigned int>(), wk->job_val_in.as<unsigned int>(),
                                                        wk->job_val_out.as<unsigned int>(), (int)n, 0, 32, st) == hipSuccess;
}

static bool launch_ext_jobs_seg(slx_aligner *al, Worker *wk, const Chunk &ck, const DevOpt &dopt, hipStream_t st, unsigned int n_jobs, const FirstJob *jobs, DReg *out,
                                const unsigned int *job_list, unsigned first_smem)
{
    if (!al->long_seg || n_jobs == 0) return false;
    if (wk->xseg_jobs.ensure((size_t)n_jobs * sizeof(XJob)) != SLX_OK || wk->xseg_state.ensure((size_t)n_jobs * sizeof(XState)) != SLX_OK || wk->xseg_cnt.ensure(64) != SLX_OK) return false;
    XPlan P;
    P.xjobs = wk->xseg_jobs.as<XJob>(); P.state = wk->xseg_state.as<XState>(); P.cnt = wk->xseg_cnt.as<unsigned int>(); P.fail_mod = al->xseg_fail;
    P.units = nullptr; P.out = nullptr; P.wrec = P.wout = P.scratch = nullptr;
    if (hipMemsetAsync(P.cnt, 0, 64, st) != hipSuccess) return false;
    const int g_join = std::max(1, std::min((int)std::min<unsigned int>(n_jobs, 1u << 30), HUGE_BLOCKS));
    size_t slots_have = 0;
    auto mid_pass_failure = [&]() { (void)hipGetLastError(); hipLaunchKernelGGL(k_or_u32, dim3(1), dim3(1), 0, st, ck.flags, (unsigned int)ERR_INTERNAL); (void)slx_wait_stream(st); };
    for (int pass = 0; pass < 3; ++pass) {
        P.pass = pass;
        (void)hipMemsetAsync(P.cnt + 1, 0, 12, st);
        (void)hipMemsetAsync(P.cnt + 8, 0, 4, st);
        hipLaunchKernelGGL(k_xseg_plan, dim3((n_jobs + 255) / 256), dim3(256), 0, st, ck, dopt, jobs, job_list, n_jobs, P);
        unsigned int h[2] = {0, 0};
        if (hipMemcpyAsync(h, P.cnt, 8, hipMemcpyDeviceToHost, st) != hipSuccess || slx_wait_stream(st) != hipSuccess) {
            if (pass == 0) return false;
            mid_pass_failure();
            return true;
        }
        if (pass == 0 && h[1] == 0) return false;
        if (wk->xseg_units.ensure((size_t)std::max(h[1], 1u) * sizeof(XUnit)) != SLX_OK || wk->xseg_out.grow((size_t)h[0] * sizeof(XSegOut), slots_have * sizeof(XSegOut), st) != SLX_OK ||
            wk->xseg_wrec.grow((size_t)h[0] * XSEG_WIN * 4, slots_have * XSEG_WIN * 4, st) != SLX_OK || wk->xseg_wout.grow((size_t)h[0] * XSEG_WIN * 4, slots_have * XSEG_WIN * 4, st) != SLX_OK ||
            wk->xseg_scratch.ensure((size_t)g_join * XSEG_WIN * 4) != SLX_OK) {
            (void)hipGetLastError();
            if (pass == 0) return false;
            mid_pass_failure();
            return true;
        }
        slots_have = h[0];
        P.units = wk->xseg_units.as<XUnit>(); P.out = wk->xseg_out.as<XSegOut>(); P.wrec = wk->xseg_wrec.as<int>(); P.wout = wk->xseg_wout.as<int>(); P.scratch = wk->xseg_scratch.as<int>();
        if (h[1]) {
            hipLaunchKernelGGL(k_xseg_units, dim3((n_jobs + 255) / 256), dim3(256), 0, st, n_jobs, P);
            if (al->xseg_wave_min > 0 && h[1] >= (unsigned int)al->xseg_wave_min)
                hipLaunchKernelGGL(k_xseg_run_w, dim3(std::max(1, std::min((int)std::min<unsigned int>((h[1] + 3) / 4, 1u << 30), al->n_cu * 8))), dim3(XB_THREADS), 0, st, al->ref, ck, dopt, jobs, job_list, P, h[1]);
            else
            hipLaunchKernelGGL(k_xseg_run, dim3(std::max(1, std::min((int)std::min<unsigned int>(h[1], 1u << 30), al->n_cu * 8))), dim3(XB_THREADS), 0, st, al->ref, ck, dopt, jobs, job_list, P, h[1]);
        }
        hipLaunchKernelGGL(k_xseg_join, dim3(g_join), dim3(XB_THREADS), first_smem, st, al->ref, ck, dopt, jobs, out, job_list, n_jobs, P);
        unsigned int waiting = 0;
        if (hipMemcpyAsync(&waiting, P.cnt + 8, 4, hipMemcpyDeviceToHost, st) != hipSuccess || slx_wait_stream(st) != hipSuccess) { mid_pass_failure(); return true; }
        if (waiting == 0) break;
    }
    unsigned int stat[4] = {0, 0, 0, 0};
    if (hipMemcpyAsync(stat, P.cnt + 4, 16, hipMemcpyDeviceToHost, st) == hipSuccess && slx_wait_stream(st) == hipSuccess)
        for (int i = 0; i < 4; ++i) wk->xseg_stat[i] += stat[i];
    return true;
}

template <int MAXQ>
static void launch_tail(slx_aligner *al, Worker *wk, const Chunk &ck, const DevOpt &dopt, unsigned int *q, const unsigned int *n_slots, int grid, int bs, int n,
                        const int *ext_light, const int *ext_heavy, const unsigned int *n_heavy, const unsigned int *ext_slots,
                        const unsigned int *top_off = nullptr, unsigned int top_cap = 0, const DReg *top_tab = nullptr, bool predict = false)
{
    hipStream_t st = wk->stream;
    hipEvent_t *dbg = wk->dbg_ev;
    const bool dbg_on = getenv("SLX_DEBUG_SUB") != nullptr;
    if (dbg_on) (void)hipEventRecord(dbg[1], st);
    const int g = std::max(1, std::min(n, ck.huge_rows ? HUGE_BLOCKS : al->n_cu * 32));
    const unsigned ext_smem = (MAXQ > 704 && !ck.huge_rows) ? (unsigned)(3 * ck.long_stride * 4) : 0u;
    if (ext_heavy) hipLaunchKernelGGL(k_extend_reg<MAXQ>, dim3(g), dim3(64), ext_smem, st, al->ref, ck, dopt, ext_light, q + 1, ext_slots ? ext_slots : n_slots, 0,
                                      ext_heavy, n_heavy, top_off, top_cap, top_tab);
    else {
        bool in_rounds = false;
        if constexpr (MAXQ > 704) {
            const size_t S1 = wk->last_S1;
            if (al->long_budget > 0 && (top_tab || predict) && top_off && S1 > 0 && wk->memo_idx.ensure(S1 * 4) == SLX_OK && wk->memo_jobs.ensure(S1 * sizeof(FirstJob)) == SLX_OK &&
                wk->memo_tab.ensure(S1 * sizeof(DReg)) == SLX_OK && wk->round_list.ensure(S1 * 4) == SLX_OK && wk->todo_a.ensure((size_t)n * 4 + 4) == SLX_OK &&
                wk->todo_b.ensure((size_t)n * 4 + 4) == SLX_OK && wk->spec_cnt.ensure(64) == SLX_OK) {
                in_rounds = true;
                unsigned int *cnt = wk->spec_cnt.as<unsigned int>();
                (void)hipMemsetAsync(wk->memo_idx.p, 0xff, S1 * 4, st);
                (void)hipMemsetAsync(cnt, 0, 64, st);
                ExtSpec sp;
                sp.memo_idx = wk->memo_idx.as<int>(); sp.memo_jobs = wk->memo_jobs.as<FirstJob>(); sp.memo_tab = wk->memo_tab.as<DReg>();
                sp.n_jobs = cnt; sp.round_list = wk->round_list.as<unsigned int>(); sp.n_round = cnt + 1; sp.n_todo_next = cnt + 2; sp.budget = al->long_budget; sp.guess = al->long_guess;
                const int *todo = nullptr;
                int n_todo = n, round = 0;
                unsigned int jobs_total = 0;
                for (;; ++round) {
                    sp.todo_next = (round & 1 ? wk->todo_b : wk->todo_a).as<int>();
                    sp.predict = predict && round == 0;
                    (void)hipMemsetAsync(cnt + 1, 0, 12, st);
                    const int gw = std::max(1, std::min(n_todo, g));
                    hipLaunchKernelGGL(k_extend_reg<MAXQ>, dim3(gw), dim3(64), ext_smem, st, al->ref, ck, dopt, todo, cnt + 3, round ? cnt + 4 : n_slots, 0, (const int *)nullptr,
                                       (const unsigned int *)nullptr, top_off, top_cap, top_tab, sp);
                    unsigned int h[3] = {0, 0, 0};
                    if (hipMemcpyAsync(h, cnt, 12, hipMemcpyDeviceToHost, st) != hipSuccess || slx_wait_stream(st) != hipSuccess) break;
                    if (h[1]) {
                        (void)hipMemsetAsync(cnt + 3, 0, 4, st);
                        const unsigned first_smem = ck.huge_rows ? 0u : (unsigned)(2 * ck.long_stride * 4);
                        if (h[1] > 1 && sort_jobs_longest_first(wk, st, wk->memo_jobs.as<FirstJob>(), wk->round_list.as<unsigned int>(), h[1]))
                            (void)hipMemcpyAsync(wk->round_list.p, wk->job_val_out.p, (size_t)h[1] * 4, hipMemcpyDeviceToDevice, st);
                        const int gj = std::max(1, std::min((int)std::min<unsigned int>(h[1], 1u << 30), ck.huge_rows ? HUGE_BLOCKS : al->n_cu * 8));
                        if (al->long_block && h[1] <= (unsigned int)al->long_block && launch_ext_jobs_seg(al, wk, ck, dopt, st, h[1], wk->memo_jobs.as<FirstJob>(), wk->memo_tab.as<DReg>(),
                                                                                                         wk->round_list.as<unsigned int>(), first_smem)) {}
                        else if (al->long_block && h[1] <= (unsigned int)al->long_block)
                            hipLaunchKernelGGL(k_ext_block, dim3(std::max(1, std::min((int)h[1], HUGE_BLOCKS))), dim3(XB_THREADS), first_smem, st, al->ref, ck, dopt, top_off + n, top_cap,
                                               cnt + 3, wk->memo_jobs.as<FirstJob>(), wk->memo_tab.as<DReg>(), wk->round_list.as<unsigned int>(), cnt + 1);
                        else
                        hipLaunchKernelGGL(k_ext_first<MAXQ>, dim3(gj), dim3(64), first_smem, st, al->ref, ck, dopt, n, top_off, top_cap, cnt + 3, wk->memo_jobs.as<FirstJob>(),
                                           wk->memo_tab.as<DReg>(), wk->round_list.as<unsigned int>(), cnt + 1);
                    }
                    jobs_total = h[0];
                    if (h[2] == 0) break;
                    (void)hipMemcpyAsync(cnt + 4, cnt + 2, 4, hipMemcpyDeviceToDevice, st);
                    todo = sp.todo_next; n_todo = (int)h[2];
                }
                wk->long_rounds_run = round + 1; wk->long_jobs_run = jobs_total;
            }
        }
        if (!in_rounds)
            hipLaunchKernelGGL(k_extend_reg<MAXQ>, dim3(g), dim3(64), ext_smem, st, al->ref, ck, dopt, (const int *)nullptr, q + 1, n_slots, 0, (const int *)nullptr,
                               (const unsigned int *)nullptr, top_off, top_cap, top_tab);
    }
#ifdef EXT_STATS
    ext_stats_print(st, "extend_reg", n, nullptr);
#endif
    if (al->keep_stages && wk->last_S1) {
        if (wk->snap_ia.ensure(wk->last_S1 * 4) == SLX_OK && wk->snap_regs.ensure(wk->last_S1 * sizeof(DReg)) == SLX_OK && wk->snap_nreg.ensure((size_t)n * 4) == SLX_OK) {
            (void)hipMemcpyAsync(wk->snap_ia.p, ck.ia, wk->last_S1 * 4, hipMemcpyDeviceToDevice, st);
            (void)hipMemcpyAsync(wk->snap_regs.p, ck.regs, wk->last_S1 * sizeof(DReg), hipMemcpyDeviceToDevice, st);
            (void)hipMemcpyAsync(wk->snap_nreg.p, ck.n_reg, (size_t)n * 4, hipMemcpyDeviceToDevice, st);
        }
    }
    (void)hipEventRecord(wk->ev[5], st);
    (void)hipEventRecord(wk->ev_probe[3], st);
    if (dbg_on) (void)hipEventRecord(dbg[2], st);
    FinLists fl;
    fl.jobs = wk->jobs.as<DJob>();
    fl.fast_list = wk->fast_list.as<uint32_t>();
    fl.dp_list = wk->dp_list.as<uint32_t>();
    fl.n_fast = q + 4; fl.n_dp = q + 5; fl.q_dp = q + 6;
    bool cig_lanes = al->cig_lanes && MAXQ <= 704 && n >= 256;
    {
        int pen = std::max(std::max(dopt.o.e_del, dopt.o.e_ins), 1), amax = 0;
        for (int i = 0; i < 25; ++i) { pen = std::max(pen, -(int)dopt.o.mat[i]); amax = std::max(amax, (int)dopt.o.mat[i]); }
        if ((int64_t)(LANE_CIG_MAXQ + LANE_CIG_MAXT) * pen + dopt.o.o_del + dopt.o.o_ins >= LANE_FIN_LIMIT || (int64_t)amax * LANE_CIG_MAXQ >= LANE_FIN_LIMIT ||
            dopt.o.o_del < 0 || dopt.o.o_ins < 0 || dopt.o.e_del < 1 || dopt.o.e_ins < 1) cig_lanes = false;
    }
    fl.lane_list = cig_lanes ? wk->cig_lane_list.as<uint32_t>() : nullptr; fl.n_lane = q + 42;
    unsigned int *cnt2 = q + 32;
    hipLaunchKernelGGL(k_part_flags_nreg, dim3((unsigned)((n + 255) / 256)), dim3(256), 0, st, ck.n_reg, n, wk->part_flag.as<unsigned int>());
    size_t tb = wk->scan_tmp.cap;
    (void)hipcub::DeviceScan::ExclusiveSum(wk->scan_tmp.p, tb, wk->part_flag.as<unsigned int>(), wk->part_pos.as<unsigned int>(), n, st);
    hipLaunchKernelGGL(k_part_scatter, dim3((unsigned)((n + 255) / 256)), dim3(256), 0, st, wk->part_flag.as<unsigned int>(),
                       wk->part_pos.as<unsigned int>(), n, wk->order_in.as<int>(), wk->order_out.as<int>(), cnt2);
    hipLaunchKernelGGL(k_regs1, dim3(std::max(1, std::min(n / 256 + 1, al->n_cu * 8))), dim3(256), 0, st, ck, dopt, fl, wk->order_in.as<int>(), cnt2);
    int *multi = wk->order_out.as<int>();
    if constexpr (MAXQ <= 704) {
        if (al->regs_sorted && wk->order_bin.ensure((size_t)n * 4) == SLX_OK && wk->bin_cnt.ensure(512) == SLX_OK && hipMemsetAsync(wk->bin_cnt.p, 0, 512, st) == hipSuccess) {
            const dim3 gb((unsigned)((n + 255) / 256));
            unsigned int *bins = wk->bin_cnt.as<unsigned int>();
            hipLaunchKernelGGL(k_nreg_bin_count<int>, gb, dim3(256), 0, st, (const int *)wk->order_out.as<int>(), (const unsigned int *)(cnt2 + 1), (const int *)ck.n_reg, bins);
            hipLaunchKernelGGL(k_nreg_bin_scan, dim3(1), dim3(64), 0, st, bins);
            hipLaunchKernelGGL(k_nreg_bin_scatter<int>, gb, dim3(256), 0, st, (const int *)wk->order_out.as<int>(), (const unsigned int *)(cnt2 + 1), (const int *)ck.n_reg, bins, wk->order_bin.as<int>());
            multi = wk->order_bin.as<int>();
        } else (void)hipGetLastError();
    }
    if constexpr (MAXQ <= 704) {
        if (al->regs_big < (1 << 20)) {
            const int mid = std::max(al->regs_big, REGS_MID_N);
            if (al->regs_big <= REGS_MID_N)
                hipLaunchKernelGGL((k_regs_wave<MAXQ, REGS_MID_N>), dim3(std::max(1, std::min(n / 64 + 1, al->n_cu * 8))), dim3(64), 0, st, al->ref, ck, dopt, fl,
                                   multi, q + 11, cnt2 + 1, al->regs_big, REGS_MID_N);
            if (mid < 512 || wk->max_seed_cnt > (unsigned int)mid)
                hipLaunchKernelGGL((k_regs_wave<MAXQ, REGS_BIG_N>), dim3(std::max(1, std::min(n / 4096 + 1, al->n_cu))), dim3(64), 0, st, al->ref, ck, dopt, fl,
                                   multi, q + 15, cnt2 + 1, al->regs_big <= REGS_MID_N ? mid + 1 : al->regs_big, 1 << 30);
        }
        int *defer_list = (al->regs_defer && wk->defer_list.ensure((size_t)n * 4) == SLX_OK) ? wk->defer_list.as<int>() : nullptr;
        hipLaunchKernelGGL(k_regs<MAXQ>, dim3(ck.spread > 1 ? std::max(grid, (n + 1) / 2) : grid), dim3(bs), 0, st, al->ref, ck, dopt, fl, multi, q + 9, cnt2 + 1, ck.spread > 1 ? 1 : 0, al->regs_big,
                           defer_list, q + 46);
        if (defer_list)
            hipLaunchKernelGGL((k_regs_wave<MAXQ, REGS_SMALL_N>), dim3(std::max(1, std::min(n / 64 + 1, al->n_cu * 16))), dim3(64), 0, st, al->ref, ck, dopt, fl, (const int *)defer_list, q + 47,
                               (const unsigned int *)(q + 46), 0, 1 << 30);
    } else {
        unsigned int n_multi = 0;
        if (hipMemcpyAsync(&n_multi, cnt2 + 1, 4, hipMemcpyDeviceToHost, st) == hipSuccess && slx_wait_stream(st) == hipSuccess && n_multi > 1 &&
            wk->job_key_in.ensure((size_t)n_multi * 4) == SLX_OK && wk->job_val_in.ensure((size_t)n_multi * 4) == SLX_OK) {
            hipLaunchKernelGGL(k_read_len_keys, dim3((n_multi + 255) / 256), dim3(256), 0, st, ck.offs, (const int *)wk->order_out.as<int>(), n_multi, wk->job_key_in.as<unsigned int>(),
                               wk->job_val_in.as<unsigned int>());
            if (sort_keys_largest_first(wk, st, n_multi)) (void)hipMemcpyAsync(wk->order_out.p, wk->job_val_out.p, (size_t)n_multi * 4, hipMemcpyDeviceToDevice, st);
        }
        PMemo pm; pm.jobs = nullptr; pm.off = pm.n = nullptr;
        if (al->long_seg && n_multi > 0) {
            const unsigned int job_cap = n_multi * PSEG_MAX_PAIRS;
            const unsigned int g_pj = (unsigned int)std::max(1, std::min((int)std::min<unsigned int>(job_cap, 1u << 20), al->n_cu * 4));
            if (wk->pseg_jobs.ensure((size_t)job_cap * sizeof(GJob)) == SLX_OK && wk->pseg_idx.ensure((size_t)n * 8 + 64) == SLX_OK && wk->pseg_cnt.ensure(64) == SLX_OK &&
                wk->gseg_scratch.ensure((size_t)g_pj * GSEG_WIN * 4) == SLX_OK && hipMemsetAsync(wk->pseg_cnt.p, 0, 64, st) == hipSuccess &&
                hipMemsetAsync(wk->pseg_idx.p, 0, (size_t)n * 8, st) == hipSuccess) {
                GPlan PP;
                PP.gjobs = wk->pseg_jobs.as<GJob>(); PP.units = nullptr; PP.wrec = PP.wout = nullptr; PP.scratch = wk->gseg_scratch.as<int>(); PP.cnt = wk->pseg_cnt.as<unsigned int>();
                PP.fail_mod = al->xseg_fail;
                int *memo_off = wk->pseg_idx.as<int>(), *memo_n = memo_off + n;
                hipLaunchKernelGGL(k_pseg_plan, dim3((n_multi + 255) / 256), dim3(256), 0, st, al->ref, ck, dopt, (const int *)wk->order_out.as<int>(), n_multi, PP, memo_off, memo_n, job_cap);
                unsigned int hp[8] = {0, 0, 0, 0, 0, 0, 0, 0};
                if (hipMemcpyAsync(hp, PP.cnt, 32, hipMemcpyDeviceToHost, st) == hipSuccess && slx_wait_stream(st) == hipSuccess && hp[7] > 0 && hp[7] <= job_cap &&
                    wk->gseg_units.ensure((size_t)std::max(hp[1], 1u) * sizeof(GUnit)) == SLX_OK && wk->gseg_wrec.ensure((size_t)std::max(hp[0], 1u) * GSEG_WIN * 4) == SLX_OK &&
                    wk->gseg_wout.ensure((size_t)std::max(hp[0], 1u) * GSEG_WIN * 4) == SLX_OK) {
                    PP.units = wk->gseg_units.as<GUnit>(); PP.wrec = wk->gseg_wrec.as<int>(); PP.wout = wk->gseg_wout.as<int>();
                    if (hp[1]) {
                        hipLaunchKernelGGL(k_gseg_units, dim3((hp[7] + 255) / 256), dim3(256), 0, st, (const unsigned int *)nullptr, hp[7], PP);
                        hipLaunchKernelGGL(k_gseg_run, dim3(std::max(1u, std::min(hp[1], (unsigned int)(al->n_cu * 8)))), dim3(GB_THREADS), 0, st, al->ref, ck, dopt, PP, hp[1]);
                    }
                    hipLaunchKernelGGL(k_pseg_join, dim3(std::min(g_pj, hp[7])), dim3(GB_THREADS), 0, st, al->ref, ck, dopt, PP, hp[7]);
                    pm.jobs = PP.gjobs; pm.off = memo_off; pm.n = memo_n;
                    wk->pseg_stat += hp[7];
                } else (void)hipGetLastError();
            } else (void)hipGetLastError();
        }
        hipLaunchKernelGGL((k_regs_wave_long<MAXQ, REGS_BIG_N>), dim3(std::max(1, std::min(n, ck.long_threads / 64))), dim3(GB_THREADS), 0, st, al->ref, ck, dopt, fl,
                           wk->order_out.as<int>(), q + 9, cnt2 + 1, pm);
    }
    if (dbg_on) (void)hipEventRecord(dbg[3], st);
    (void)hipEventRecord(wk->ev_probe[4], st);
    if (al->cig_fast_coop) hipLaunchKernelGGL(k_cig_fast_coop, dim3(std::max(1, std::min(n / 256 + 1, al->n_cu * 8))), dim3(256), 0, st, al->ref, ck, fl);
    else hipLaunchKernelGGL(k_cig_fast, dim3(std::max(1, std::min(n / 256 + 1, al->n_cu * 8))), dim3(256), 0, st, al->ref, ck, fl);
    if (cig_lanes) {
        if (al->cig_lane_il) hipLaunchKernelGGL(k_cig_lanes<true>, dim3(al->n_cu * 16), dim3(64), 0, st, al->ref, ck, dopt, fl, wk->cig_lane_list.as<uint32_t>(), q + 42, q + 43);
        else hipLaunchKernelGGL(k_cig_lanes<false>, dim3(al->n_cu * 16), dim3(64), 0, st, al->ref, ck, dopt, fl, wk->cig_lane_list.as<uint32_t>(), q + 42, q + 43);
    }
    if constexpr (MAXQ <= 704) hipLaunchKernelGGL(k_cig_dp<MAXQ>, dim3(g), dim3(64), 0, st, al->ref, ck, dopt, fl, 0);
    else {
        FinLists rest = fl;
        rest.dp_list = wk->cig_lane_list.as<uint32_t>(); rest.n_dp = q + 42; rest.q_dp = q + 43;
        unsigned int n_dp_h = 0;
        if (hipMemcpyAsync(&n_dp_h, fl.n_dp, 4, hipMemcpyDeviceToHost, st) == hipSuccess && slx_wait_stream(st) == hipSuccess && n_dp_h > 1 &&
            wk->job_key_in.ensure((size_t)n_dp_h * 4) == SLX_OK && wk->job_val_in.ensure((size_t)n_dp_h * 4) == SLX_OK) {
            (void)hipMemsetAsync(q + 44, 0, 8, st);
            hipLaunchKernelGGL(k_cig_job_keys, dim3((n_dp_h + 255) / 256), dim3(256), 0, st, (const DJob *)fl.jobs, (const uint32_t *)fl.dp_list, n_dp_h, dopt, wk->job_key_in.as<unsigned int>(),
                               wk->job_val_in.as<unsigned int>(), q + 44, al->long_seg);
            if (sort_keys_largest_first(wk, st, n_dp_h)) {
                (void)hipMemcpyAsync(fl.dp_list, wk->job_val_out.p, (size_t)n_dp_h * 4, hipMemcpyDeviceToDevice, st);
                unsigned int n_big = 0;
                if (al->long_block && hipMemcpyAsync(&n_big, q + 44, 4, hipMemcpyDeviceToHost, st) == hipSuccess && slx_wait_stream(st) == hipSuccess && n_big) {
                    const unsigned int bb = std::min(n_big, (unsigned int)(al->n_cu * 4));
                    const unsigned int wb = std::min((n_dp_h - std::min(n_dp_h, n_big) + 3) / 4, (unsigned int)(al->n_cu * 4));
                    GPlan GP;
                    GP.gjobs = nullptr; GP.units = nullptr; GP.wrec = GP.wout = GP.scratch = nullptr; GP.cnt = nullptr; GP.fail_mod = al->xseg_fail;
                    if (al->long_seg && wk->gseg_jobs.ensure((size_t)n_big * sizeof(GJob)) == SLX_OK && wk->gseg_cnt.ensure(64) == SLX_OK &&
                        wk->gseg_scratch.ensure((size_t)(bb + wb) * GSEG_WIN * 4) == SLX_OK && hipMemsetAsync(wk->gseg_cnt.p, 0, 64, st) == hipSuccess) {
                        GP.gjobs = wk->gseg_jobs.as<GJob>(); GP.cnt = wk->gseg_cnt.as<unsigned int>(); GP.scratch = wk->gseg_scratch.as<int>();
                        (void)hipMemcpyAsync(GP.cnt + 8, ck.zused, 8, hipMemcpyDeviceToDevice, st);
                        hipLaunchKernelGGL(k_gseg_plan, dim3((n_big + 255) / 256), dim3(256), 0, st, al->ref, ck, dopt, fl, n_big, GP);
                        unsigned int hh[2] = {0, 0};
                        if (hipMemcpyAsync(hh, GP.cnt, 8, hipMemcpyDeviceToHost, st) != hipSuccess || slx_wait_stream(st) != hipSuccess) hh[1] = 0;
                        if (hh[1] && wk->gseg_units.ensure((size_t)hh[1] * sizeof(GUnit)) == SLX_OK && wk->gseg_wrec.ensure((size_t)hh[0] * GSEG_WIN * 4) == SLX_OK &&
                            wk->gseg_wout.ensure((size_t)hh[0] * GSEG_WIN * 4) == SLX_OK) {
                            GP.units = wk->gseg_units.as<GUnit>(); GP.wrec = wk->gseg_wrec.as<int>(); GP.wout = wk->gseg_wout.as<int>();
                            hipLaunchKernelGGL(k_gseg_units, dim3((n_big + 255) / 256), dim3(256), 0, st, (const unsigned int *)fl.n_dp, n_big, GP);
                            hipLaunchKernelGGL(k_gseg_run, dim3(std::max(1u, std::min(hh[1], (unsigned int)(al->n_cu * 8)))), dim3(GB_THREADS), 0, st, al->ref, ck, dopt, GP, hh[1]);
                        } else if (hh[1]) {
                            (void)hipGetLastError();
                            (void)hipMemcpyAsync(ck.zused, GP.cnt + 8, 8, hipMemcpyDeviceToDevice, st);
                            GP.gjobs = nullptr;
                        } else GP.gjobs = nullptr;
                    } else (void)hipGetLastError();
                    hipLaunchKernelGGL(k_set_u32, dim3(1), dim3(1), 0, st, fl.q_dp, n_big);
                    hipLaunchKernelGGL(k_cig_band_block, dim3(bb + wb), dim3(GB_THREADS), 0, st, al->ref, ck, dopt, fl, n_big, bb, q + 45,
                                       wk->cig_lane_list.as<uint32_t>(), q + 42, GP);
                    if (GP.gjobs) {
                        unsigned int stat[3] = {0, 0, 0};
                        if (hipMemcpyAsync(stat, GP.cnt + 4, 12, hipMemcpyDeviceToHost, st) == hipSuccess && slx_wait_stream(st) == hipSuccess)
                            for (int i = 0; i < 3; ++i) wk->gseg_stat[i] += stat[i];
                    }
                }
            }
        }
        hipLaunchKernelGGL(k_cig_band, dim3(std::max(1, std::min(n * 4, al->n_cu * 16))), dim3(64), 0, st, al->ref, ck, dopt, fl, wk->cig_lane_list.as<uint32_t>(), q + 42);
        hipLaunchKernelGGL(k_cig_long, dim3(grid), dim3(bs), 0, st, al->ref, ck, dopt, rest);
    }
    (void)hipEventRecord(wk->ev_probe[5], st);
    if (dbg_on) (void)hipEventRecord(dbg[4], st);
    if (ck.sam_mode) hipLaunchKernelGGL(k_hits_sam, dim3(grid), dim3(bs), 0, st, al->ref, ck, dopt, (const int *)multi, q + 3, q + 33);
    else {
        int *big = (al->hits_wave && wk->hits_big.ensure((size_t)n * 4) == SLX_OK) ? wk->hits_big.as<int>() : nullptr;
        hipLaunchKernelGGL(k_hits, dim3(ck.spread > 1 ? std::max(grid, (n + 1) / 2) : grid), dim3(bs), 0, st, ck, (const int *)multi, q + 3, q + 33, ck.spread > 1 ? 1 : 0, big, q + 48);
        if (big) hipLaunchKernelGGL(k_hits_wave, dim3(std::max(1, std::min(n / 256 + 1, al->n_cu * 4))), dim3(64), 0, st, ck, (const int *)big, (const unsigned int *)(q + 48), q + 49);
    }
    if (dbg_on) (void)hipEventRecord(dbg[5], st);
}

struct CvtI32U64 { __host__ __device__ unsigned long long operator()(int v) const { return (unsigned long long)v; } };

template <typename I>
static void launch_coop(slx_aligner *al, Worker *wk, const Chunk &ck, const DevOpt &dopt, const DevFM<I> &fm, hipStream_t st, unsigned int *q,
                        unsigned int *counts, int n, bool both_tables = false)
{
    constexpr int N1 = COOP_N1;
    constexpr int WAVES_PER_CU = N1 <= 512 ? 8 : N1 <= 768 ? 6 : N1 <= 1024 ? 4 : 3;
    hipLaunchKernelGGL((k_chain_coop<I, N1, false>), dim3(std::max(1, std::min(n / 8 + 1, al->n_cu * WAVES_PER_CU))), dim3(64), 0, st, fm, al->ref, ck, dopt,
                       wk->order_out.as<int>(), q + 8, counts + 1, al->coop_lim1);
    if (both_tables || std::min(N1, al->coop_lim1) < 512 || wk->max_seed_cnt > (unsigned int)std::min(N1, al->coop_lim1))
        hipLaunchKernelGGL((k_chain_coop<I, 4096, true>), dim3(std::max(1, std::min(n / 4096 + 1, N1 < 1536 ? al->n_cu : 16))), dim3(64), 0, st, fm, al->ref, ck, dopt,
                           wk->order_out.as<int>(), q + 10, counts + 1, al->coop_lim2);
}


static bool production_seed(const slx_aligner *al, int n, bool has_long) { return n >= al->split_min && !has_long; }

template <typename I>
static int run_chunk(slx_aligner *al, Worker *wk, const slx_opt *opt, const uint8_t *d_ascii, const uint64_t *d_offs, const uint64_t *h_offs_pair,
                     int64_t r0, int64_t part_lo, int n, int max_len, uint64_t rng_state, uint64_t first_ordinal, int hardclip, double ksf, int maxsec,
                     const ChunkCaps &caps, int64_t *hit_base, int64_t *cig_base, uint32_t *flags_out)
{
    hipStream_t st = wk->stream;
    int rc;
    const uint64_t base0 = h_offs_pair[0], n_bases = h_offs_pair[1] - h_offs_pair[0];
    const int bs = 128;
    const bool has_long = max_len > 704 || flt_live(*opt, max_len, log((double)std::max(max_len, 1)), nullptr);
    int n_threads = (int)std::min<int64_t>(((int64_t)n + bs - 1) / bs * bs, (int64_t)(has_long ? std::min(al->max_threads, 16384) : al->max_threads));
    if (has_long) {
        const int64_t per_thread = (int64_t)2 * (max_len + 1) * (int64_t)sizeof(IntvE<I>) + (int64_t)2 * (max_len + 8) * 4;
        const int64_t fit = std::max<int64_t>(bs, ((int64_t)8 << 30) / per_thread / bs * bs);
        n_threads = (int)std::min<int64_t>(n_threads, fit);
    }
    const int grid = n_threads / bs;
    int seed_grid = grid;
    uint32_t seed_quota = 0;
    if (al->seed_quota > 0 && !has_long && n >= al->split_min) {
        seed_quota = (uint32_t)((al->seed_quota + SEED_POOL - 1) / SEED_POOL * SEED_POOL);
        seed_grid = (int)(((int64_t)n + 2 * (int64_t)seed_quota - 1) / (2 * (int64_t)seed_quota));
        n_threads = std::max(n_threads, seed_grid * bs);
    }
    const int spread = (al->small_spread && n <= SMALL_SPREAD_MAX && n >= 2 && !has_long && n < al->split_min) ? 64 : 1;
    if (spread > 1) {
        seed_grid = std::max(seed_grid, (n + 1) / 2);
        n_threads = std::max(n_threads, seed_grid * bs);
    }
    const int cap_list = max_len + 1;
#define ENS(buf, bytes) if ((rc = wk->buf.ensure((size_t)(bytes))) != SLX_OK) return rc
    ENS(codes, n_bases + 16); ENS(offs_rel, ((size_t)n + 1) * 8);
    ENS(intv_n, (size_t)n * 4); ENS(intv_info, (size_t)n * caps.cap_intv * sizeof(qp_t)); ENS(intv_x0, (size_t)n * caps.cap_intv * sizeof(I));
    ENS(intv_x2, (size_t)n * caps.cap_intv * sizeof(I)); ENS(l_rep, (size_t)n * 4); ENS(seed_cnt, ((size_t)n + 1) * 8); ENS(seed_off, ((size_t)n + 1) * 8);
    ENS(n_chain, (size_t)n * 4); ENS(n_reg, (size_t)n * 4); ENS(n_hit, ((size_t)n + 1) * 4); ENS(na, (size_t)n * 4); ENS(frac_rep, (size_t)n * 4);
    ENS(lists, (size_t)2 * cap_list * n_threads * sizeof(IntvE<I>));
    ENS(zarena, caps.zcap); ENS(cigpool, caps.cigcap * 4);
    ENS(hit_cnt, ((size_t)n + 1) * 8); ENS(cig_cnt, ((size_t)n + 1) * 8); ENS(hit_off_c, ((size_t)n + 1) * 8); ENS(cig_off_c, ((size_t)n + 1) * 8);
    ENS(counters, 64); ENS(p2mask, (size_t)n * 8); ENS(p2list, (size_t)n * 4); ENS(p2items, (size_t)n * 4); ENS(p2long, (size_t)n * 4);
    HIPCHK(hipMemsetAsync(wk->counters.p, 0, 64, st));
    ENS(queues, 256);
    HIPCHK(hipMemsetAsync(wk->queues.p, 0, 256, st));
    HIPCHK(hipMemsetAsync(wk->seed_cnt.as<unsigned long long>() + n, 0, 8, st));

    Chunk ck;
    memset(&ck, 0, sizeof ck);
    ck.n_reads = n;
    ck.spread = spread;
    ck.codes = wk->codes.as<uint8_t>();
    ck.offs = wk->offs_rel.as<uint64_t>();
    ck.first_ordinal = first_ordinal + (uint64_t)r0;
    ck.rng_state = rng_state;
    ck.cap_intv = caps.cap_intv;
    ck.intv_n = wk->intv_n.as<uint32_t>(); ck.intv_info = wk->intv_info.as<uint32_t>();
    ck.intv_x0 = wk->intv_x0.p; ck.intv_x2 = wk->intv_x2.p;
    ck.l_rep = wk->l_rep.as<int32_t>();
    ck.seed_off = wk->seed_off.as<uint64_t>();
    ck.n_chain = wk->n_chain.as<int32_t>(); ck.n_reg = wk->n_reg.as<int32_t>(); ck.n_hit = wk->n_hit.as<int32_t>();
    ck.na = wk->na.as<int32_t>(); ck.frac_rep = wk->frac_rep.as<float>();
    ck.zarena = wk->zarena.as<uint8_t>(); ck.zcap = caps.zcap; ck.zused = wk->counters.as<unsigned long long>();
    ck.cigpool = wk->cigpool.as<uint32_t>(); ck.cigcap = caps.cigcap; ck.cigused = wk->counters.as<unsigned long long>() + 1;
    ck.flags = (uint32_t *)(wk->counters.as<unsigned long long>() + 2);
    ck.log_lut = al->d_loglut.as<double>(); ck.log_lut_n = SLX_LOG_LUT_N;
    ck.lists = wk->lists.p; ck.cap_list = cap_list; ck.n_threads = n_threads;
    ck.hardclip = hardclip; ck.keepSecFrac = ksf; ck.maxSecondary = maxsec;
    ck.sam_mode = (opt->flag & SLX_F_REG2SAM) ? 1 : 0;
    ck.seed_cnt = wk->seed_cnt.as<unsigned long long>();
    const bool production = al->chain_mode == 1 && n >= al->split_min && !has_long;
    const bool use_cand = al->cand_mode == 1 && production;
    if (use_cand) {
        ENS(cand, (size_t)al->cand_cap * sizeof(DReg)); ENS(cand_base, (size_t)n * 4); ENS(cand_cnt, ((size_t)n + 2) * 8); ENS(cand_off, ((size_t)n + 2) * 8);
        HIPCHK(hipMemsetAsync(wk->cand_base.p, 0xff, (size_t)n * 4, st));
        ck.cand = wk->cand.as<DReg>(); ck.cand_base = wk->cand_base.as<int32_t>();
    }
    if (getenv("SLX_DEBUG_CYC")) {
        ENS(dbg_cyc, (size_t)n * 32);
        HIPCHK(hipMemsetAsync(wk->dbg_cyc.p, 0, (size_t)n * 32, st));
        ck.dbg_cyc = wk->dbg_cyc.as<unsigned long long>();
        ck.dbg_stage = atoi(getenv("SLX_DEBUG_CYC"));
    }
    DevOpt dopt; dopt.o = *opt;
    DevFM<I> fm = fm_of<I>(al);
    fm.sa_dense = (al->dense_sa && al->have_dense) ? al->d_sa_dense.as<I>() : nullptr;
    fm.rep = al->rep_mask ? al->d_rep.as<uint32_t>() : nullptr; fm.rep_mask = al->rep_mask; fm.rep_k = al->rep_k;
    fm.bwd_direct = (al->bwd_direct && fm.sa_dense && (sizeof(I) == 8 || (uint64_t)fm.seq_len < (1ULL << 31))) ? 1 : 0;

    (void)hipEventRecord(wk->ev[0], st);
    {
        const unsigned g = (unsigned)std::min<uint64_t>((n_bases / 16 + 255) / 256 + 1, 65535u * 4);
        hipLaunchKernelGGL(k_encode, dim3(g), dim3(256), 0, st, d_ascii + base0, wk->codes.as<uint8_t>(), (size_t)n_bases);
        hipLaunchKernelGGL(k_rel_offsets, dim3((unsigned)((n + 1 + 255) / 256)), dim3(256), 0, st, d_offs + r0, wk->offs_rel.as<uint64_t>(), n, base0);
    }
    (void)hipEventRecord(wk->ev[1], st);
    (void)hipEventRecord(wk->ev_probe[0], st);
    {
        hipStream_t ss = st;
        if (wk->seed_stream && production_seed(al, n, has_long)) {
            ss = wk->seed_stream;
            HIPCHK(hipEventRecord(wk->ev_seed_in, st));
            HIPCHK(hipStreamWaitEvent(ss, wk->ev_seed_in, 0));
        }
        unsigned int *qq = wk->queues.as<unsigned int>();
        hipLaunchKernelGGL((k_seed12m<I, 1>), dim3(seed_grid), dim3(bs), 0, ss, fm, al->ref, ck, dopt, qq + 29, seed_quota,
                           (const int *)nullptr, (const unsigned int *)nullptr, (const unsigned long long *)nullptr, (const uint32_t *)nullptr, (const unsigned int *)nullptr, 0u,
                           (uint32_t *)nullptr, (unsigned int *)nullptr, 0u);
        const uint32_t cap_items = (al->p2_items && n < (1 << 26)) ? (uint32_t)(al->p2_items_cap > 0 ? std::min(al->p2_items_cap, n) : n) : 0u;
        const uint32_t cap_long = (cap_items && al->p2_coop) ? cap_items : 0u;
        hipLaunchKernelGGL(k_seed2_select<I>, dim3((unsigned)(((int64_t)n * spread + bs - 1) / bs)), dim3(bs), 0, ss, fm, ck, dopt, wk->p2mask.as<unsigned long long>(), wk->p2list.as<int>(), qq + 35,
                           wk->p2items.as<uint32_t>(), qq + 37, cap_items);
        hipLaunchKernelGGL((k_seed12m<I, 2>), dim3(grid), dim3(bs), 0, ss, fm, al->ref, ck, dopt, qq + 36, 0u, wk->p2list.as<int>(), qq + 35,
                           wk->p2mask.as<unsigned long long>(), wk->p2items.as<uint32_t>(), qq + 37, cap_items, wk->p2long.as<uint32_t>(), qq + 38, cap_long);
        if (cap_long) hipLaunchKernelGGL(k_seed2_coop<I>, dim3((unsigned)(al->n_cu * 8)), dim3(64), 0, ss, fm, al->ref, ck, dopt, qq + 39, wk->p2long.as<uint32_t>(), qq + 38, cap_long);
        const int seed3_par = (max_len > 8192 && al->long_seed3) ? 4096 : 0x7fffffff;
        hipLaunchKernelGGL(k_seed3m<I>, dim3((unsigned)(((int64_t)n * spread + bs - 1) / bs)), dim3(bs), 0, ss, fm, al->ref, ck, dopt, seed3_par);
        if (seed3_par != 0x7fffffff) {
            ENS(seed3_buf, (size_t)n_bases * sizeof(Seed3Next<I>));
            hipLaunchKernelGGL(k_seed3_next<I>, dim3((unsigned)((n_bases + 255) / 256)), dim3(256), 0, ss, fm, al->ref, ck, dopt, seed3_par, (uint64_t)n_bases, wk->seed3_buf.as<Seed3Next<I>>());
            hipLaunchKernelGGL(k_seed3_chase<I>, dim3((unsigned)((n + 63) / 64)), dim3(64), 0, ss, ck, dopt, seed3_par, (const Seed3Next<I> *)wk->seed3_buf.as<Seed3Next<I>>());
        }
        hipLaunchKernelGGL(k_seed_epi<I>, dim3((unsigned)((n + 63) / 64)), dim3(64), 0, ss, ck, dopt, wk->queues.as<unsigned int>() + 31,
                           (unsigned int)al->heavy_seeds, wk->queues.as<unsigned int>() + 34);
        if (ss != st) {
            HIPCHK(hipEventRecord(wk->ev_seed_out, ss));
            HIPCHK(hipStreamWaitEvent(st, wk->ev_seed_out, 0));
        }
    }
    (void)hipEventRecord(wk->ev_probe[1], st);
    (void)hipEventRecord(wk->ev[2], st);
    {
        size_t tmp_bytes = 0;
        hipcub::DeviceScan::ExclusiveSum(nullptr, tmp_bytes, (unsigned long long *)wk->seed_cnt.p, (unsigned long long *)wk->seed_off.p, n + 1, st);
        ENS(scan_tmp, tmp_bytes + 256);
        HIPCHK(hipcub::DeviceScan::ExclusiveSum(wk->scan_tmp.p, tmp_bytes, (unsigned long long *)wk->seed_cnt.p, (unsigned long long *)wk->seed_off.p, n + 1, st));
    }
    {
        MailSpec ms{};
        ms.src[0] = (const unsigned int *)(wk->seed_off.as<uint64_t>() + n); ms.words[0] = 2;
        ms.src[1] = (const unsigned int *)ck.flags; ms.words[1] = 1;
        ms.src[2] = wk->queues.as<unsigned int>() + 31; ms.words[2] = 1;
        ms.src[3] = wk->queues.as<unsigned int>() + 34; ms.words[3] = 1;
        ms.src[4] = wk->queues.as<unsigned int>() + 35; ms.words[4] = 4;
        ms.n = 5;
        hipLaunchKernelGGL(k_mail, dim3(1), dim3(64), 0, st, ms, wk->h_mail);
    }
    HIPCHK(slx_wait_stream(st));
    unsigned long long S = 0;
    memcpy(&S, wk->h_mail, 8);
    const uint32_t fl0 = wk->h_mail[2];
    const unsigned int max_cnt = wk->h_mail[3], n_heavy_h = wk->h_mail[4];
    unsigned int n_p2_h = 0, n_long_h = 0, n_it_h = 0;
    unsigned int p2c[4] = {wk->h_mail[5], wk->h_mail[6], wk->h_mail[7], wk->h_mail[8]};
    n_p2_h = p2c[0]; n_it_h = p2c[2]; n_long_h = p2c[3];
    wk->cnt[0] += n_heavy_h; wk->cnt[1] += n_it_h; wk->cnt[2] += n_long_h; wk->cnt[3] += n_p2_h;
    if (getenv("SLX_DEBUG_SEED")) fprintf(stderr, "[seed] worker %d: %d reads, pass 2: %u single calls (%u of them one wave each) + %u whole reads (repeat filter k = %d), %u heavy\n", wk->id, n, n_it_h, n_long_h, n_p2_h, fm.rep ? fm.rep_k : 0, n_heavy_h);
    if (fl0) { *flags_out = fl0; return SLX_OK; }
    wk->max_seed_cnt = max_cnt;
    const size_t S1 = (size_t)S + 1;
    ENS(s_rbeg, S1 * 8); ENS(s_ql, S1 * sizeof(qp_t)); ENS(s_next, S1 * 4); ENS(c_pos, S1 * 8); ENS(c_head, S1 * 4); ENS(c_tail, S1 * 4);
    ENS(c_n, S1 * 4); ENS(c_rid, S1 * 4); ENS(c_w, S1 * 4); ENS(c_first, S1 * 4); ENS(c_kept, S1); ENS(ia, S1 * 4); ENS(ib, S1 * 4);
    ENS(ic, S1 * 4); ENS(srt, S1 * 8); ENS(regs, S1 * sizeof(DReg)); ENS(hits, S1 * sizeof(DHit));
    ENS(jobs, S1 * sizeof(DJob)); ENS(fast_list, S1 * 4); ENS(dp_list, S1 * 4); ENS(cig_lane_list, S1 * 4);
    ck.s_rbeg = wk->s_rbeg.as<int64_t>(); ck.s_ql = wk->s_ql.as<uint32_t>(); ck.s_next = wk->s_next.as<int32_t>();
    ck.c_pos = wk->c_pos.as<int64_t>(); ck.c_head = wk->c_head.as<int32_t>(); ck.c_tail = wk->c_tail.as<int32_t>();
    ck.c_n = wk->c_n.as<int32_t>(); ck.c_rid = wk->c_rid.as<int32_t>(); ck.c_w = wk->c_w.as<int32_t>();
    ck.c_first = wk->c_first.as<int32_t>(); ck.c_kept = wk->c_kept.as<int8_t>();
    ck.ia = wk->ia.as<int32_t>(); ck.ib = wk->ib.as<int32_t>(); ck.ic = wk->ic.as<int32_t>(); ck.srt = wk->srt.as<uint64_t>();
    ck.regs = wk->regs.as<DReg>(); ck.hits = wk->hits.as<DHit>();
    wk->last_S1 = S1;
    if (has_long) {
        ENS(s_score, S1 * 4); ENS(long_list, (size_t)n * 4);
        ck.s_score = wk->s_score.as<int32_t>();
        ck.long_stride = max_len + 8; ck.long_threads = n_threads;
        ENS(long_scratch, (size_t)n_threads * 2 * ck.long_stride * 4);
        ck.long_scratch = wk->long_scratch.as<int>();
        if (3 * (max_len + 8) * 4 > 64 * 1024) {
            ck.huge_stride = max_len + 8;
            ENS(huge_rows, (size_t)HUGE_BLOCKS * 3 * ck.huge_stride * 4);
            ck.huge_rows = wk->huge_rows.as<int>();
        }
    }
    (void)hipEventRecord(wk->ev[3], st);
    {
        unsigned int *q = wk->queues.as<unsigned int>();
        unsigned int *counts = q + 24;
        ENS(part_flag, (size_t)n * 4); ENS(part_pos, (size_t)n * 4); ENS(order_in, (size_t)n * 4); ENS(order_out, (size_t)n * 4);
        {
            size_t tb = 0;
            HIPCHK(hipcub::DeviceScan::ExclusiveSum(nullptr, tb, wk->part_flag.as<unsigned int>(), wk->part_pos.as<unsigned int>(), n + 1, st));
            ENS(scan_tmp, tb + 256);
        }
        const bool dbg_on = getenv("SLX_DEBUG_SUB") != nullptr;
        if (dbg_on) (void)hipEventRecord(wk->dbg_ev[0], st);
        const bool hsort = al->heavy_sorted && al->heavy_seeds <= 0xfffff;
        if (!production) {
            if ((max_len > 704 && al->long_coop) || (max_len <= 704 && al->small_coop && n_heavy_h > 0)) {
                hipLaunchKernelGGL(k_part_flags, dim3((unsigned)((n + 255) / 256)), dim3(256), 0, st, wk->seed_cnt.as<unsigned long long>(), n,
                                   (unsigned int)al->heavy_seeds, wk->part_flag.as<unsigned int>());
                size_t tb = wk->scan_tmp.cap;
                HIPCHK(hipcub::DeviceScan::ExclusiveSum(wk->scan_tmp.p, tb, wk->part_flag.as<unsigned int>(), wk->part_pos.as<unsigned int>(), n, st));
                hipLaunchKernelGGL(k_part_scatter, dim3((unsigned)((n + 255) / 256)), dim3(256), 0, st, wk->part_flag.as<unsigned int>(),
                                   wk->part_pos.as<unsigned int>(), n, wk->order_in.as<int>(), wk->order_out.as<int>(), counts);
                hipLaunchKernelGGL(k_chain<I>, dim3(spread > 1 ? seed_grid : grid), dim3(bs), 0, st, fm, al->ref, ck, dopt, wk->order_in.as<int>(), q + 0, counts, spread > 1 ? 1 : 0);
                launch_coop<I>(al, wk, ck, dopt, fm, st, q, counts, n, max_len > 704);
                hipLaunchKernelGGL(k_set_u32, dim3(1), dim3(1), 0, st, counts, (unsigned int)n);
            } else {
            hipLaunchKernelGGL(k_set_u32, dim3(1), dim3(1), 0, st, counts, (unsigned int)n);
            hipLaunchKernelGGL(k_chain<I>, dim3(spread > 1 ? seed_grid : grid), dim3(bs), 0, st, fm, al->ref, ck, dopt, (const int *)nullptr, q + 0, counts, spread > 1 ? 1 : 0);
            }
            if (has_long) {
                hipLaunchKernelGGL(k_long_list, dim3((unsigned)((n + 255) / 256)), dim3(256), 0, st, ck, dopt, wk->long_list.as<int>(), q + 16);
                hipLaunchKernelGGL(k_flt_score, dim3((unsigned)std::min<int64_t>((int64_t)n * FLT_PARTS, 0x7fffffff)), dim3(64), 0, st, al->ref, ck, dopt, wk->long_list.as<int>(), q + 16);
                hipLaunchKernelGGL(k_flt_seeds, dim3(std::max(1, std::min(n, al->n_cu * 8))), dim3(64), 0, st, al->ref, ck, dopt, wk->long_list.as<int>(), q + 16, q + 17);
            }
            (void)hipEventRecord(wk->ev_probe[2], st);
            (void)hipEventRecord(wk->ev[4], st);
            if (max_len > 8192 && al->long_budget > 0 && al->long_predict) {
                ENS(first_off, ((size_t)n + 2) * 4);
                HIPCHK(hipMemsetAsync(wk->first_off.p, 0, ((size_t)n + 2) * 4, st));
                launch_tail<MAXQ_LONG>(al, wk, ck, dopt, q, counts, grid, bs, n, nullptr, nullptr, nullptr, nullptr, wk->first_off.as<unsigned int>(), 0u, (const DReg *)nullptr, true);
            }
            else if (max_len > 704) {
                const unsigned int top_cap = (unsigned int)std::min<uint64_t>((uint64_t)S1, 0x7fffffffu);
                ENS(first_tab, (size_t)top_cap * sizeof(DReg)); ENS(first_cnt, ((size_t)n + 2) * 4); ENS(first_off, ((size_t)n + 2) * 4);
                ENS(first_jobs, (size_t)top_cap * sizeof(FirstJob));
                HIPCHK(hipMemsetAsync(wk->first_cnt.p, 0, ((size_t)n + 2) * 4, st));
                hipLaunchKernelGGL(k_first_count, dim3((unsigned)((n + 255) / 256)), dim3(256), 0, st, ck, n, 0xffffffffu, wk->first_cnt.as<unsigned int>(), 0);
                size_t tb = wk->scan_tmp.cap;
                HIPCHK(hipcub::DeviceScan::ExclusiveSum(wk->scan_tmp.p, tb, wk->first_cnt.as<unsigned int>(), wk->first_off.as<unsigned int>(), n + 1, st));
                hipLaunchKernelGGL(k_first_prep, dim3(std::max(1, std::min(n / 128 + 1, al->n_cu * 12))), dim3(128), 0, st, al->ref, ck, dopt, n, wk->first_off.as<unsigned int>(),
                                   top_cap, wk->first_jobs.as<FirstJob>());
                const unsigned first_smem = ck.huge_rows ? 0u : (unsigned)(2 * ck.long_stride * 4);
                if (al->long_block && n <= al->long_block / 4 && max_len > 8192) {
                    unsigned int n_top_h = 0;
                    HIPCHK(hipMemcpyAsync(&n_top_h, wk->first_off.as<unsigned int>() + n, 4, hipMemcpyDeviceToHost, st));
                    HIPCHK(slx_wait_stream(st));
                    n_top_h = std::min(n_top_h, top_cap);
                    const bool sorted = n_top_h > 1 && sort_jobs_longest_first(wk, st, wk->first_jobs.as<FirstJob>(), nullptr, n_top_h);
                    if (n_top_h && launch_ext_jobs_seg(al, wk, ck, dopt, st, n_top_h, wk->first_jobs.as<FirstJob>(), wk->first_tab.as<DReg>(),
                                                       sorted ? (const unsigned int *)wk->job_val_out.as<unsigned int>() : (const unsigned int *)nullptr, first_smem)) {}
                    else
                    hipLaunchKernelGGL(k_ext_block, dim3(HUGE_BLOCKS), dim3(XB_THREADS), first_smem, st, al->ref, ck, dopt, wk->first_off.as<unsigned int>() + n, top_cap, q + 22,
                                       wk->first_jobs.as<FirstJob>(), wk->first_tab.as<DReg>(), sorted ? (const unsigned int *)wk->job_val_out.as<unsigned int>() : (const unsigned int *)nullptr,
                                       sorted ? (const unsigned int *)(wk->first_off.as<unsigned int>() + n) : (const unsigned int *)nullptr);
                }
                else
                hipLaunchKernelGGL(k_ext_first<MAXQ_LONG>, dim3(ck.huge_rows ? HUGE_BLOCKS : al->n_cu * 8), dim3(64), first_smem, st, al->ref, ck, dopt, n, wk->first_off.as<unsigned int>(),
                                   top_cap, q + 22, wk->first_jobs.as<FirstJob>(), wk->first_tab.as<DReg>(), (const unsigned int *)nullptr, (const unsigned int *)nullptr);
                launch_tail<MAXQ_LONG>(al, wk, ck, dopt, q, counts, grid, bs, n, nullptr, nullptr, nullptr, nullptr, wk->first_off.as<unsigned int>(), top_cap, wk->first_tab.as<DReg>());
            }
            else with_maxq(max_len, [&](auto mq) {
                launch_tail<decltype(mq)::value>(al, wk, ck, dopt, q, counts, grid, bs, n, nullptr, nullptr, nullptr, nullptr);
            });
        } else {
            hipLaunchKernelGGL(k_part_flags, dim3((unsigned)((n + 255) / 256)), dim3(256), 0, st, wk->seed_cnt.as<unsigned long long>(), n,
                               (unsigned int)al->heavy_seeds, wk->part_flag.as<unsigned int>());
            size_t tb = wk->scan_tmp.cap;
            HIPCHK(hipcub::DeviceScan::ExclusiveSum(wk->scan_tmp.p, tb, wk->part_flag.as<unsigned int>(), wk->part_pos.as<unsigned int>(), n, st));
            hipLaunchKernelGGL(k_part_scatter, dim3((unsigned)((n + 255) / 256)), dim3(256), 0, st, wk->part_flag.as<unsigned int>(),
                               wk->part_pos.as<unsigned int>(), n, wk->order_in.as<int>(), wk->order_out.as<int>(), counts);
            if (hsort && n_heavy_h > 1) {
                const unsigned int nh = n_heavy_h;
                ENS(order_key_in, (size_t)nh * 4); ENS(order_key_out, (size_t)nh * 4); ENS(order_tmp, (size_t)nh * 4);
                hipLaunchKernelGGL(k_heavy_keys, dim3((nh + 255) / 256), dim3(256), 0, st, wk->seed_cnt.as<unsigned long long>(), wk->order_out.as<int>(), nh,
                                   wk->order_key_in.as<unsigned int>());
                size_t tb2 = 0;
                HIPCHK(hipcub::DeviceRadixSort::SortPairsDescending(nullptr, tb2, wk->order_key_in.as<unsigned int>(), wk->order_key_out.as<unsigned int>(),
                                                                    wk->order_out.as<int>(), wk->order_tmp.as<int>(), (int)nh, 0, 20, st));
                ENS(sort_tmp, tb2 + 256);
                HIPCHK(hipcub::DeviceRadixSort::SortPairsDescending(wk->sort_tmp.p, tb2, wk->order_key_in.as<unsigned int>(), wk->order_key_out.as<unsigned int>(),
                                                                    wk->order_out.as<int>(), wk->order_tmp.as<int>(), (int)nh, 0, 20, st));
                HIPCHK(hipMemcpyAsync(wk->order_out.p, wk->order_tmp.p, (size_t)nh * 4, hipMemcpyDeviceToDevice, st));
            }
            hipLaunchKernelGGL(k_set_u32, dim3(1), dim3(1), 0, st, counts + 2, (unsigned int)n);
            const int *light = wk->order_in.as<int>();
            if (al->chain_sorted && wk->order_bin.ensure((size_t)n * 4) == SLX_OK && wk->bin_cnt.ensure(512) == SLX_OK && hipMemsetAsync(wk->bin_cnt.p, 0, 512, st) == hipSuccess) {
                const dim3 gbn((unsigned)((n + 255) / 256));
                unsigned int *bins = wk->bin_cnt.as<unsigned int>();
                hipLaunchKernelGGL(k_nreg_bin_count<unsigned long long>, gbn, dim3(256), 0, st, light, (const unsigned int *)counts, (const unsigned long long *)wk->seed_cnt.as<unsigned long long>(), bins);
                hipLaunchKernelGGL(k_nreg_bin_scan, dim3(1), dim3(64), 0, st, bins);
                hipLaunchKernelGGL(k_nreg_bin_scatter<unsigned long long>, gbn, dim3(256), 0, st, light, (const unsigned int *)counts, (const unsigned long long *)wk->seed_cnt.as<unsigned long long>(), bins,
                                   wk->order_bin.as<int>());
                light = wk->order_bin.as<int>();
            } else (void)hipGetLastError();
            hipLaunchKernelGGL(k_chain<I>, dim3(grid), dim3(bs), 0, st, fm, al->ref, ck, dopt, light, q + 0, counts, 0);
            launch_coop<I>(al, wk, ck, dopt, fm, st, q, counts, n);
            (void)hipEventRecord(wk->ev_probe[2], st);
            if (use_cand) {
                const int nh = (int)n_heavy_h;
                const unsigned gb = (unsigned)((nh + 255) / 256) + 1;
                HIPCHK(hipMemsetAsync(wk->cand_cnt.p, 0, ((size_t)nh + 2) * 8, st));
                unsigned int *slot_cnt = wk->cand_cnt.as<unsigned int>(), *job_cnt = slot_cnt + (nh + 2);
                unsigned int *slot_off = wk->cand_off.as<unsigned int>(), *job_off = slot_off + (nh + 2);
                int amax = 0;
                for (int i = 0; i < 25; ++i) amax = std::max(amax, (int)opt->mat[i]);
                amax = std::max(amax, opt->a);
                const int lane_cols = max_len - std::min(opt->min_seed_len, max_len) + 2 + al->lane_pad;
                const bool lane_narrow = al->lane_narrow && amax * max_len < 256;
                const bool lanes = (al->cand_lanes > 0 || (al->cand_lanes < 0 && n <= CAND_REP_AUTO_READS)) && max_len <= 704 && (lane_narrow ? LaneNarrow::bytes(lane_cols) : LaneWide::bytes(lane_cols)) <= 64 * 1024 &&
                                   (int64_t)amax * max_len < LANE_SCORE_LIMIT;
                const int cand_rep = lanes ? 0 : (al->cand_rep >= 0 ? al->cand_rep : (n <= CAND_REP_AUTO_READS ? 75 : 0));
                for (int pass = cand_rep > 0 ? 1 : 0; pass >= 0; --pass)
                    hipLaunchKernelGGL(k_cand_count, dim3(gb), dim3(256), 0, st, ck, wk->order_out.as<int>(), counts + 1, slot_cnt, job_cnt,
                                       (unsigned int)(lanes ? al->cand_lane_seeds : al->cand_seeds), (hsort && !lanes) ? (unsigned int)al->cand_top : 0xffffffffu,
                                       (unsigned int)cand_rep, q + 30, (unsigned int)al->cand_rep_max, pass, lanes ? 1 : CAND_PART);
                tb = wk->scan_tmp.cap;
                HIPCHK(hipcub::DeviceScan::ExclusiveSum(wk->scan_tmp.p, tb, slot_cnt, slot_off, nh + 1, st));
                hipLaunchKernelGGL(k_cand_base, dim3(gb), dim3(256), 0, st, wk->order_out.as<int>(), counts + 1, slot_off, (unsigned int)al->cand_cap,
                                   wk->cand_base.as<int32_t>(), job_cnt);
                tb = wk->scan_tmp.cap;
                HIPCHK(hipcub::DeviceScan::ExclusiveSum(wk->scan_tmp.p, tb, job_cnt, job_off, nh + 1, st));
                const int gc = al->n_cu * 32;
                if (lanes) {
                    const size_t max_jobs = std::min<size_t>((size_t)al->cand_cap, S1);
                    ENS(lane_jobs, max_jobs * sizeof(LaneJob));
                    auto go = [&](auto mq) {
                        constexpr int MAXQ = decltype(mq)::value;
                        hipLaunchKernelGGL(k_cand_lane_prep<MAXQ>, dim3(std::max(1, std::min(nh, al->n_cu * 16))), dim3(64), 0, st, al->ref, ck, dopt, wk->order_out.as<int>(), counts + 1,
                                           job_off, wk->lane_jobs.as<LaneJob>());
                        if (lane_narrow) hipLaunchKernelGGL(k_ext_lanes<LaneNarrow>, dim3(al->n_cu * 8), dim3(64), LaneNarrow::bytes(lane_cols), st, al->ref, ck, dopt, counts + 1, job_off,
                                                            q + 14, wk->lane_jobs.as<LaneJob>(), wk->cand.as<DReg>(), lane_cols);
                        else hipLaunchKernelGGL(k_ext_lanes<LaneWide>, dim3(al->n_cu * 4), dim3(64), LaneWide::bytes(lane_cols), st, al->ref, ck, dopt, counts + 1, job_off, q + 14,
                                                wk->lane_jobs.as<LaneJob>(), wk->cand.as<DReg>(), lane_cols);
                    };
                    with_maxq(max_len, go);
                } else
                with_maxq(max_len, [&](auto mq) {
                    hipLaunchKernelGGL(k_extend_cand<decltype(mq)::value>, dim3(gc), dim3(64), 0, st, al->ref, ck, dopt, wk->order_out.as<int>(), counts + 1,
                                       job_off, q + 14, wk->cand.as<DReg>());
                });
            }
            if (hsort && al->ext_split) {
                const unsigned int top_cap = (unsigned int)std::min<uint64_t>((uint64_t)n + std::min<uint64_t>((uint64_t)S1, (uint64_t)n), 0x7fffffffu);
                ENS(first_tab, (size_t)top_cap * sizeof(DReg)); ENS(first_cnt, ((size_t)n + 2) * 4); ENS(first_off, ((size_t)n + 2) * 4); ENS(fb_list, (size_t)n * 4);
                unsigned int *n_fb = q + 20, *ext_tot = q + 21;
                HIPCHK(hipMemsetAsync(wk->first_cnt.p, 0, ((size_t)n + 2) * 4, st));
                hipLaunchKernelGGL(k_first_count, dim3((unsigned)((n + 255) / 256)), dim3(256), 0, st, ck, n, (unsigned int)al->heavy_seeds, wk->first_cnt.as<unsigned int>(),
                                   al->top_heavy);
                tb = wk->scan_tmp.cap;
                HIPCHK(hipcub::DeviceScan::ExclusiveSum(wk->scan_tmp.p, tb, wk->first_cnt.as<unsigned int>(), wk->first_off.as<unsigned int>(), n + 1, st));
                const int gf = al->n_cu * 32;
                ENS(first_jobs, (size_t)top_cap * sizeof(FirstJob));
                if (al->first_diag) ENS(first_dp, (size_t)top_cap * 4);
                int fl_amax = 0;
                for (int i = 0; i < 25; ++i) fl_amax = std::max(fl_amax, (int)opt->mat[i]);
                fl_amax = std::max(fl_amax, opt->a);
                const int fl_cols = max_len - std::min(opt->min_seed_len, max_len) + 2 + al->lane_pad;
                const bool fl_narrow = al->lane_narrow && fl_amax * max_len < 256;
                const bool first_lanes = al->first_lanes && al->first_diag && max_len <= 704 && (fl_narrow ? LaneNarrow::bytes(fl_cols) : LaneWide::bytes(fl_cols)) <= 64 * 1024 &&
                                         (int64_t)fl_amax * max_len < LANE_SCORE_LIMIT;
                if (first_lanes) {
                    ENS(first_sorted, (size_t)top_cap * 4); ENS(first_bins, 1024);
                    HIPCHK(hipMemsetAsync(wk->first_bins.p, 0, 512, st));
                }
                hipLaunchKernelGGL(k_first_prep, dim3(std::max(1, std::min(n / 128 + 1, al->n_cu * 12))), dim3(128), 0, st, al->ref, ck, dopt, n, wk->first_off.as<unsigned int>(),
                                   top_cap, wk->first_jobs.as<FirstJob>());
                with_maxq(max_len, [&](auto mq) {
                    constexpr int MAXQ = decltype(mq)::value;
                    if (al->first_diag) {
                        hipLaunchKernelGGL(k_first_diag, dim3((top_cap + 255) / 256), dim3(256), 0, st, al->ref, ck, dopt, n, wk->first_off.as<unsigned int>(), top_cap,
                                           wk->first_jobs.as<FirstJob>(), wk->first_tab.as<DReg>(), wk->first_dp.as<unsigned int>(), q + 40);
                    }
                    if (first_lanes) {
                        unsigned int *bins = wk->first_bins.as<unsigned int>(), *sorted = wk->first_sorted.as<unsigned int>();
                        const FirstJob *fj = wk->first_jobs.as<FirstJob>();
                        hipLaunchKernelGGL(k_first_bin_count, dim3(al->n_cu * 4), dim3(256), 0, st, fj, (const unsigned int *)wk->first_dp.as<unsigned int>(), (const unsigned int *)(q + 40), max_len, bins);
                        hipLaunchKernelGGL(k_first_bin_scan, dim3(1), dim3(1), 0, st, bins);
                        hipLaunchKernelGGL(k_first_bin_scatter, dim3(al->n_cu * 4), dim3(256), 0, st, fj, (const unsigned int *)wk->first_dp.as<unsigned int>(), (const unsigned int *)(q + 40), max_len, bins, sorted);
                        if (fl_narrow) hipLaunchKernelGGL(k_first_lanes<LaneNarrow>, dim3(al->n_cu * 8), dim3(64), LaneNarrow::bytes(fl_cols), st, al->ref, ck, dopt, q + 22, fj, wk->first_tab.as<DReg>(),
                                                          (const unsigned int *)sorted, (const unsigned int *)(q + 40), fl_cols);
                        else hipLaunchKernelGGL(k_first_lanes<LaneWide>, dim3(al->n_cu * 4), dim3(64), LaneWide::bytes(fl_cols), st, al->ref, ck, dopt, q + 22, fj, wk->first_tab.as<DReg>(),
                                                (const unsigned int *)sorted, (const unsigned int *)(q + 40), fl_cols);
                    } else
                    hipLaunchKernelGGL(k_ext_first<MAXQ>, dim3(gf), dim3(64), 0, st, al->ref, ck, dopt, n, wk->first_off.as<unsigned int>(), top_cap, q + 22,
                                       wk->first_jobs.as<FirstJob>(), wk->first_tab.as<DReg>(), al->first_diag ? wk->first_dp.as<unsigned int>() : (const unsigned int *)nullptr, q + 40);
#ifdef EXT_STATS
                    ext_stats_print(st, "cand + ext_first", n, wk->first_off.as<unsigned int>() + n);
#endif
                    hipLaunchKernelGGL(k_ext_replay<MAXQ>, dim3(grid), dim3(bs), 0, st, al->ref, ck, dopt, n, (unsigned int)al->heavy_seeds, wk->first_off.as<unsigned int>(),
                                       top_cap, wk->first_tab.as<DReg>(), q + 23, wk->fb_list.as<int>(), n_fb);
                });
                hipLaunchKernelGGL(k_add_u32, dim3(1), dim3(1), 0, st, counts + 1, n_fb, ext_tot);
                (void)hipEventRecord(wk->ev[4], st);
                with_maxq(max_len, [&](auto mq) {
                    launch_tail<decltype(mq)::value>(al, wk, ck, dopt, q, counts + 2, grid, bs, n, wk->fb_list.as<int>(), wk->order_out.as<int>(), counts + 1, ext_tot,
                                                     al->top_reuse ? wk->first_off.as<unsigned int>() : nullptr, top_cap, wk->first_tab.as<DReg>());
                });
            } else {
                (void)hipEventRecord(wk->ev[4], st);
                with_maxq(max_len, [&](auto mq) {
                    if (hsort) launch_tail<decltype(mq)::value>(al, wk, ck, dopt, q, counts + 2, grid, bs, n, wk->order_in.as<int>(), wk->order_out.as<int>(), counts + 1, nullptr);
                    else launch_tail<decltype(mq)::value>(al, wk, ck, dopt, q, counts + 2, grid, bs, n, nullptr, nullptr, nullptr, nullptr);
                });
            }
        }
    }
    (void)hipEventRecord(wk->ev[6], st);
    hipLaunchKernelGGL(k_hit_counts, dim3((unsigned)((n + 255) / 256)), dim3(256), 0, st, ck, wk->cig_cnt.as<unsigned long long>());
    {
        hipcub::TransformInputIterator<unsigned long long, CvtI32U64, const int *> it(wk->n_hit.as<int>(), CvtI32U64());
        size_t tb = 0;
        hipcub::DeviceScan::ExclusiveSum(nullptr, tb, it, wk->hit_off_c.as<unsigned long long>(), n + 1, st);
        ENS(scan_tmp, tb + 256);
        HIPCHK(hipcub::DeviceScan::ExclusiveSum(wk->scan_tmp.p, tb, it, wk->hit_off_c.as<unsigned long long>(), n + 1, st));
        size_t tb2 = 0;
        hipcub::DeviceScan::ExclusiveSum(nullptr, tb2, wk->cig_cnt.as<unsigned long long>(), wk->cig_off_c.as<unsigned long long>(), n + 1, st);
        ENS(scan_tmp, tb2 + 256);
        HIPCHK(hipcub::DeviceScan::ExclusiveSum(wk->scan_tmp.p, tb2, wk->cig_cnt.as<unsigned long long>(), wk->cig_off_c.as<unsigned long long>(), n + 1, st));
    }
    unsigned long long Hc = 0, Cc = 0;
    {
        MailSpec ms{};
        ms.src[0] = (const unsigned int *)(wk->hit_off_c.as<unsigned long long>() + n); ms.words[0] = 2;
        ms.src[1] = (const unsigned int *)(wk->cig_off_c.as<unsigned long long>() + n); ms.words[1] = 2;
        ms.src[2] = (const unsigned int *)ck.flags; ms.words[2] = 1;
        ms.src[3] = wk->queues.as<unsigned int>() + 46; ms.words[3] = 1;
        ms.src[4] = wk->queues.as<unsigned int>() + 48; ms.words[4] = 1;
        ms.n = 5;
        hipLaunchKernelGGL(k_mail, dim3(1), dim3(64), 0, st, ms, wk->h_mail);
    }
    HIPCHK(slx_wait_stream(st));
    memcpy(&Hc, wk->h_mail, 8); memcpy(&Cc, wk->h_mail + 2, 8);
    const uint32_t fl = wk->h_mail[4];
    wk->fin_stat[0] += wk->h_mail[5]; wk->fin_stat[1] += wk->h_mail[6];
    if (fl) { *flags_out = fl; return SLX_OK; }
    const size_t H = (size_t)*hit_base + Hc, C = (size_t)*cig_base + Cc;
#define GROW(buf, bytes, keep) if ((rc = wk->buf.grow((size_t)(bytes), (size_t)(keep), st)) != SLX_OK) return rc
    GROW(o_rid, (H + 1) * 4, *hit_base * 4); GROW(o_pos, (H + 1) * 8, *hit_base * 8); GROW(o_flag, (H + 1) * 2, *hit_base * 2);
    GROW(o_mapq, (H + 1), *hit_base); GROW(o_score, (H + 1) * 4, *hit_base * 4); GROW(o_nm, (H + 1) * 4, *hit_base * 4);
    GROW(o_na, (H + 1) * 4, *hit_base * 4); GROW(o_ncig, (H + 1) * 4, *hit_base * 4); GROW(o_cig_off, (H + 2) * 8, *hit_base * 8);
    GROW(o_cigar, (C + 1) * 4, *cig_base * 4);
    if (ck.sam_mode) { GROW(o_xa, (H + 1) * 4, *hit_base * 4); GROW(o_sub, (H + 1) * 4, *hit_base * 4); }
    HitsSoA so;
    so.hit_off = wk->o_hit_off.as<int64_t>(); so.rid = wk->o_rid.as<int32_t>(); so.pos = wk->o_pos.as<int64_t>();
    so.flag = wk->o_flag.as<uint16_t>(); so.mapq = wk->o_mapq.as<uint8_t>(); so.score = wk->o_score.as<int32_t>();
    so.nm = wk->o_nm.as<int32_t>(); so.na = wk->o_na.as<int32_t>(); so.n_cigar_ops = wk->o_ncig.as<int32_t>();
    so.cig_off = wk->o_cig_off.as<int64_t>(); so.cigar = wk->o_cigar.as<uint32_t>();
    so.xa_parent = ck.sam_mode ? wk->o_xa.as<int32_t>() : nullptr; so.sub = ck.sam_mode ? wk->o_sub.as<int32_t>() : nullptr;
    hipLaunchKernelGGL(k_compact, dim3((unsigned)((n + 255) / 256)), dim3(256), 0, st, ck, wk->hit_off_c.as<unsigned long long>(),
                       wk->cig_off_c.as<unsigned long long>(), so, r0 - part_lo, *hit_base, *cig_base);
    (void)hipEventRecord(wk->ev[7], st);
    HIPCHK(hipGetLastError());
    HIPCHK(slx_wait_stream(st));
    for (int i = 0; i < 7; ++i) {
        float ms = 0;
        if (hipEventElapsedTime(&ms, wk->ev[i], wk->ev[i + 1]) == hipSuccess) wk->stage_ms[i] += ms;
    }
    for (int i = 0; i < 3; ++i) {
        float ms = 0;
        if (hipEventElapsedTime(&ms, wk->ev_probe[2 * i], wk->ev_probe[2 * i + 1]) == hipSuccess) wk->probe_ms[i] += ms;
    }
    {
        hipEvent_t a[3] = {wk->ev[3], wk->ev_probe[3], wk->ev_probe[5]}, b[3] = {wk->ev_probe[2], wk->ev_probe[4], wk->ev[6]};
        for (int i = 0; i < 3; ++i) {
            float ms = 0;
            if (hipEventElapsedTime(&ms, a[i], b[i]) == hipSuccess) wk->probe_ms[3 + i] += ms;
        }
    }
    if (ck.dbg_cyc && ck.dbg_stage == 3) {
        unsigned long long c6[32];
        HIPCHK(hipMemcpy(c6, wk->dbg_cyc.p, 256, hipMemcpyDeviceToHost));
        fprintf(stderr, "[seed12m] calls with min_intv <= 2: %llu, %.1f backward steps each; others: %llu, %.1f each; by length < 64 / < 256 / < 1024 / more: %llu (%.3g steps), %llu (%.3g), %llu (%.3g), %llu (%.3g); longest %llu\n",
                c6[16], c6[16] ? (double)c6[17] / (double)c6[16] : 0., c6[18], c6[18] ? (double)c6[19] / (double)c6[18] : 0., c6[20], (double)c6[21], c6[22], (double)c6[23], c6[24], (double)c6[25],
                c6[26], (double)c6[27], c6[30]);
        {
            std::vector<unsigned long long> life((size_t)grid * 2);
            HIPCHK(hipMemcpy(life.data(), wk->dbg_cyc.as<unsigned long long>() + 64, life.size() * 8, hipMemcpyDeviceToHost));
            std::vector<unsigned long long> lv;
            for (unsigned long long v : life) if (v) lv.push_back(v);
            std::sort(lv.begin(), lv.end());
            if (!lv.empty()) {
                fprintf(stderr, "[seed12m] wave lifetimes (cycle-counter ticks), %zu waves: min %.3g  p10 %.3g  p50 %.3g  p90 %.3g  p99 %.3g  max %.3g\n", lv.size(), (double)lv[0],
                        (double)lv[lv.size() / 10], (double)lv[lv.size() / 2], (double)lv[lv.size() * 9 / 10], (double)lv[lv.size() * 99 / 100], (double)lv.back());
            }
        }
        fprintf(stderr, "[seed12m] lanes per round by phase: fetch %.1f init %.1f start %.1f fwd %.1f dir %.1f row %.1f bwd %.1f done %.1f\n", (double)c6[8] / (double)c6[4],
                (double)c6[9] / (double)c6[4], (double)c6[10] / (double)c6[4], (double)c6[11] / (double)c6[4], (double)c6[12] / (double)c6[4], (double)c6[13] / (double)c6[4],
                (double)c6[14] / (double)c6[4], (double)c6[15] / (double)c6[4]);
        fprintf(stderr, "[seed12m] forward loop: %.4g wave-steps, %.1f lanes active; backward loop: %.4g wave-steps, %.1f lanes active; %.4g rounds, %.4g with events; direct loop: %.4g wave-steps (32 bases each), %.1f lanes active; %d reads\n",
                (double)c6[0], (double)c6[1] / (double)(c6[0] ? c6[0] : 1), (double)c6[2], (double)c6[3] / (double)(c6[2] ? c6[2] : 1), (double)c6[4], (double)c6[5], (double)c6[6], (double)c6[7] / (double)(c6[6] ? c6[6] : 1), n);
    } else if (ck.dbg_cyc) {
        std::vector<unsigned long long> cyc((size_t)n * 4), sc((size_t)n);
        std::vector<int> nch((size_t)n), nrg((size_t)n), lrep((size_t)n);
        HIPCHK(hipMemcpy(lrep.data(), wk->l_rep.p, (size_t)n * 4, hipMemcpyDeviceToHost));
        HIPCHK(hipMemcpy(cyc.data(), wk->dbg_cyc.p, (size_t)n * 32, hipMemcpyDeviceToHost));
        HIPCHK(hipMemcpy(sc.data(), wk->seed_cnt.p, (size_t)n * 8, hipMemcpyDeviceToHost));
        HIPCHK(hipMemcpy(nch.data(), wk->n_chain.p, (size_t)n * 4, hipMemcpyDeviceToHost));
        HIPCHK(hipMemcpy(nrg.data(), wk->n_reg.p, (size_t)n * 4, hipMemcpyDeviceToHost));
        std::vector<int> ord((size_t)n);
        for (int i = 0; i < n; ++i) ord[(size_t)i] = i;
        const int top = std::min(n, 12);
        std::partial_sort(ord.begin(), ord.begin() + top, ord.end(), [&](int a, int b) { return cyc[(size_t)a] > cyc[(size_t)b]; });
        unsigned long long tot = 0, tot_heavy = 0;
        unsigned long long ph[3] = {0, 0, 0};
        for (int i = 0; i < n; ++i) {
            tot += cyc[(size_t)i];
            if (sc[(size_t)i] >= (unsigned long long)al->heavy_seeds) tot_heavy += cyc[(size_t)i];
            for (int k = 0; k < 3; ++k) ph[k] += cyc[(size_t)(k + 1) * (size_t)n + (size_t)i];
        }
        float ext_ms = 0;
        (void)hipEventElapsedTime(&ext_ms, wk->ev[4], wk->ev[5]);
        fprintf(stderr, "[ext phases] sort %.3g  covered tests %.3g  extend+store %.3g ticks; extension stage %.1f ms\n", (double)ph[0], (double)ph[1], (double)ph[2], ext_ms);
        {
            const int lim[6] = {2, 8, 48, 128, 256, 640};
            for (int b = 0; b < 6; ++b) {
                long cnt = 0; unsigned long long cy = 0, a = 0, bb = 0, c = 0;
                for (int i = 0; i < n; ++i)
                    if (nrg[(size_t)i] >= lim[b] && (b == 5 || nrg[(size_t)i] < lim[b + 1])) {
                        ++cnt; cy += cyc[(size_t)i]; a += cyc[(size_t)n + i]; bb += cyc[2 * (size_t)n + i]; c += cyc[3 * (size_t)n + i];
                    }
                fprintf(stderr, "[regions >= %d] reads %ld  ticks %.3g (A %.3g B %.3g C %.3g)\n", lim[b], cnt, (double)cy, (double)a, (double)bb, (double)c);
            }
        }
        {
            const int lb[5] = {0, 1, 50, 100, 140};
            for (int b = 0; b < 5; ++b) {
                long cnt = 0; unsigned long long cy = 0;
                for (int i = 0; i < n; ++i)
                    if (nrg[(size_t)i] >= 256 && lrep[(size_t)i] >= lb[b] && (b == 4 || lrep[(size_t)i] < lb[b + 1])) { ++cnt; cy += cyc[(size_t)i]; }
                fprintf(stderr, "[>= 256 regions, l_rep >= %d] reads %ld  mean ticks %.3g\n", lb[b], cnt, cnt ? (double)cy / (double)cnt : 0.0);
            }
        }
        fprintf(stderr, "[ext cycles] n=%d total=%.3g (100 MHz ticks) heavy share=%.3f\n", n, (double)tot, tot ? (double)tot_heavy / (double)tot : 0.0);
        for (int i = 0; i < top; ++i) {
            const size_t r = (size_t)ord[(size_t)i];
            fprintf(stderr, "  read %zu: %.3g ticks (A %.3g, B %.3g, C %.3g; stage 1: sort, covered tests, extend+store; stage 2: sort by end, dedup/patch, second sort)  seeds=%llu chains=%d regions=%d l_rep=%d\n", r, (double)cyc[r],
                    (double)cyc[(size_t)n + r], (double)cyc[2 * (size_t)n + r], (double)cyc[3 * (size_t)n + r], sc[r], nch[r], nrg[r], lrep[r]);
        }
    }
    if (getenv("SLX_DEBUG_SUB")) {
        const char *nm[5] = {"chain", "extend", "regs", "cig", "hits"};
        fprintf(stderr, "[worker %d n=%d]", wk->id, n);
        for (int i = 0; i < 5; ++i) { float ms = -1; (void)hipEventElapsedTime(&ms, wk->dbg_ev[i], wk->dbg_ev[i + 1]); fprintf(stderr, " %s=%.1f", nm[i], ms); }
        float tot = -1; (void)hipEventElapsedTime(&tot, wk->dbg_ev[0], wk->dbg_ev[5]);
        fprintf(stderr, " total=%.1f\n", tot);
    }
    wk->last_ck = ck; wk->last_valid = true; wk->last_wide = sizeof(I) == 8;
    *hit_base += (int64_t)Hc;
    *cig_base += (int64_t)Cc;
    *flags_out = 0;
    return SLX_OK;
#undef ENS
#undef GROW
}
```

Measured before the change: 68.74 million.

## Run chaining for small-seed reads in LDS workspace with global fallback

Adds a k_chain_lds kernel that keeps each read's chaining workspace (seeds, chains, order arrays) in a per-lane, column-interleaved LDS slice whenever the read has at most 12 seeds. Reads that overflow bail out to a list, which the existing global-memory k_chain kernel then processes. The chaining body is templated over the workspace type, and results are committed back to global memory once chaining finishes. This targets the scattered global-memory traffic of chaining on short reads, at the cost of an extra kernel launch, recomputation for reads that bail, and lower occupancy from the LDS footprint.

Measured after the change: 69.90 million (median of 6 runs). 1.7% higher.

```diff
diff --git a/seqlib_amd/csrc/dev_chain.h b/seqlib_amd/csrc/dev_chain.h
--- a/seqlib_amd/csrc/dev_chain.h
+++ b/seqlib_amd/csrc/dev_chain.h
@@ -21,6 +21,9 @@
     int cap;
     __device__ __forceinline__ int s_qbeg(int s) const { return QP_HI(s_ql[s]); }
     __device__ __forceinline__ int s_len(int s) const { return QP_LO(s_ql[s]); }
+    static constexpr bool in_lds = false;
+    __device__ __forceinline__ bool full(int, int) const { return false; }
+    __device__ __forceinline__ void commit(int, int) const {}
 };
 
 __device__ __forceinline__ ReadWS make_ws(const Chunk &ck, int r);
@@ -51,7 +54,8 @@
     return w;
 }
 
-__device__ inline int dev_chain_weight(const ReadWS &w, int c)
+template <typename W>
+__device__ inline int dev_chain_weight(const W &w, int c)
 {
     int64_t end = 0;
     int wt = 0, tmp;
@@ -72,17 +76,16 @@
     return wt < 1 << 30 ? wt : (1 << 30) - 1;
 }
 
-template <typename I>
-__device__ void dev_chain_read(const DevFM<I> &fm, const DevRef &R, const Chunk &ck, const slx_opt &opt, int r)
-{
-        ReadWS w = make_ws(ck, r);
+template <typename I, typename W>
+__device__ __forceinline__ bool dev_chain_body(const DevFM<I> &fm, const DevRef &R, const Chunk &ck, const slx_opt &opt, int r, W &w)
+{
         const int len = (int)(ck.offs[r + 1] - ck.offs[r]);
         const int n_intv = (int)ck.intv_n[r];
         const qp_t *iinfo = (const qp_t *)ck.intv_info + (size_t)r * ck.cap_intv;
         const I *ix0 = (const I *)ck.intv_x0 + (size_t)r * ck.cap_intv;
         const I *ix2 = (const I *)ck.intv_x2 + (size_t)r * ck.cap_intv;
         int ns = 0, nc = 0;
-        int *ord = w.ia;
+        auto ord = w.ia;
         KbTree kb;
         bool tree = false;
         int cc = -1, cc_tail = 0, cc_n = 0, cc_rid = 0;
@@ -127,6 +130,7 @@
                         else {
                             const int64_t x = qbeg - l_qbeg, y = rbeg - l_rbeg;
                             if (y >= 0 && x - y <= opt.w && y - x <= opt.w && x - l_len < opt.max_chain_gap && y - l_len < opt.max_chain_gap) {
+                                if (w.full(ns, c)) return false;
                                 const int s = ns++;
                                 const qp_t ql = QP_PACK(qbeg, slen);
                                 w.s_rbeg[s] = rbeg; w.s_ql[s] = ql; w.s_next[s] = -1; if (w.s_score) w.s_score[s] = slen;
@@ -139,13 +143,16 @@
                     }
                 }
                 if (to_add) {
+                    if (w.full(ns, nc)) return false;
                     const int s = ns++, c = nc;
                     w.s_rbeg[s] = rbeg; w.s_ql[s] = QP_PACK(qbeg, slen); w.s_next[s] = -1; if (w.s_score) w.s_score[s] = slen;
                     w.c_pos[c] = rbeg; w.c_head[c] = w.c_tail[c] = s; w.c_n[c] = 1; w.c_rid[c] = rid;
                     cc = c; cc_tail = s; cc_n = 1; cc_rid = rid; cc_fql = cc_lql = QP_PACK(qbeg, slen); cc_frb = cc_lrb = rbeg;
+                    if constexpr (!W::in_lds) {
                     if (!tree && nc == 2 * KB_T - 1) { kb.from_array((int *)w.regs, ord, w.c_pos, nc); tree = true; }
                     if (tree) kb.put(rbeg, c);
-                    else {
+                    }
+                    if (!tree) {
                         for (int m = nc; m > lo + 1; --m) ord[m] = ord[m - 1];
                         ord[lo + 1] = c;
                     }
@@ -153,10 +160,10 @@
                 }
             }
         }
-        if (tree) kb.traverse(ord);
+        if constexpr (!W::in_lds) if (tree) kb.traverse(ord);
         ck.frac_rep[r] = (float)ck.l_rep[r] / len;
         int n_chn = 0;
-        int *a = w.ia;
+        auto a = w.ia;
         for (int i = 0; i < nc; ++i) {
             const int c = a[i];
             w.c_first[c] = -1; w.c_kept[c] = 0;
@@ -166,7 +173,7 @@
         int n_out = 0;
         if (n_chn > 0) {
             ks_introsort_idx(n_chn, a, [&](int x, int y) { return w.c_w[x] > w.c_w[y]; });
-            int *kept = w.ib, n_kept = 0;
+            auto kept = w.ib; int n_kept = 0;
             auto cbeg = [&](int c) { return w.s_qbeg(w.c_head[c]); };
             auto cend = [&](int c) { return w.s_qbeg(w.c_tail[c]) + w.s_len(w.c_tail[c]); };
             w.c_kept[a[0]] = 3;
@@ -234,7 +241,16 @@
                 for (int s = w.c_head[c]; s >= 0; s = w.s_next[s]) w.c_w[off++] = s;
             }
         }
+        w.commit(ns, nc);
         ck.n_chain[r] = n_out;
+        return true;
+}
+
+template <typename I>
+__device__ void dev_chain_read(const DevFM<I> &fm, const DevRef &R, const Chunk &ck, const slx_opt &opt, int r)
+{
+    ReadWS w = make_ws(ck, r);
+    dev_chain_body<I>(fm, R, ck, opt, r, w);
 }
 
 template <typename I>
diff --git a/seqlib_amd/csrc/dev_chain_lds.h b/seqlib_amd/csrc/dev_chain_lds.h
--- /dev/null
+++ b/seqlib_amd/csrc/dev_chain_lds.h
@@ -0,0 +1,116 @@
+#pragma once
+#include "dev_chain.h"
+
+#ifndef SLX_WIDE
+
+#ifndef CHAIN_LDS_SEEDS
+#define CHAIN_LDS_SEEDS 12
+#endif
+
+#define LDS_AS __attribute__((address_space(3)))
+
+template <typename T, typename S>
+struct LdsRef {
+    LDS_AS S *p;
+    __device__ __forceinline__ operator T() const { return (T)*p; }
+    __device__ __forceinline__ LdsRef &operator=(T v) { *p = (S)v; return *this; }
+    __device__ __forceinline__ LdsRef &operator=(const LdsRef &o) { *p = *o.p; return *this; }
+};
+
+template <typename T, typename S>
+struct LdsCol {
+    LDS_AS char *b;
+    int k;
+    static_assert(sizeof(S) == 1 || sizeof(S) == 4 || sizeof(S) == 8, "LdsCol: 1-, 4- or 8-byte elements");
+    static __host__ __device__ constexpr int rows(int n) { return sizeof(S) == 1 ? (n + 3) / 4 : n * (int)(sizeof(S) / 4); }
+    __device__ __forceinline__ void init(LDS_AS char *slice, int row, int lane) { b = slice + row * 256 + lane * (sizeof(S) == 8 ? 8 : 4); k = 0; }
+    __device__ __forceinline__ LdsRef<T, S> operator[](int i) const
+    {
+        const int e = k + i;
+        return LdsRef<T, S>{(LDS_AS S *)(b + (sizeof(S) == 1 ? (e >> 2) * 256 + (e & 3) : e * 64 * (int)sizeof(S)))};
+    }
+    __device__ __forceinline__ LdsRef<T, S> operator*() const { return (*this)[0]; }
+    __device__ __forceinline__ LdsCol operator+(int n) const { return LdsCol{b, k + n}; }
+    __device__ __forceinline__ LdsCol operator-(int n) const { return LdsCol{b, k - n}; }
+    __device__ __forceinline__ LdsCol &operator++() { ++k; return *this; }
+    __device__ __forceinline__ LdsCol &operator--() { --k; return *this; }
+    __device__ __forceinline__ bool operator<(const LdsCol &o) const { return k < o.k; }
+    __device__ __forceinline__ bool operator>(const LdsCol &o) const { return k > o.k; }
+};
+
+template <typename I, int NS>
+struct LdsWS {
+    static constexpr bool in_lds = true;
+    static constexpr int NC = NS < 2 * KB_T - 1 ? NS : 2 * KB_T - 1;
+    static_assert(NS >= 1 && NS < 128, "LdsWS: handles are stored as signed bytes");
+    static_assert(sizeof(qp_t) == 4, "LdsWS: 16 + 16-bit packed query positions");
+    typedef LdsCol<int64_t, I> PosCol;
+    typedef LdsCol<qp_t, qp_t> QlCol;
+    typedef LdsCol<int32_t, int32_t> IntCol;
+    typedef LdsCol<int32_t, int8_t> HandleCol;
+    typedef LdsCol<int8_t, int8_t> ByteCol;
+    PosCol s_rbeg, c_pos;
+    QlCol s_ql;
+    IntCol c_rid, c_w;
+    HandleCol s_next, c_head, c_tail, c_n, c_first, ia, ib;
+    ByteCol c_kept;
+    static constexpr int32_t *s_score = nullptr;
+    DReg *regs;
+    ReadWS g;
+    static constexpr int R_SRBEG = 0, R_CPOS = R_SRBEG + PosCol::rows(NS), R_SQL = R_CPOS + PosCol::rows(NC), R_CRID = R_SQL + QlCol::rows(NS),
+                         R_CW = R_CRID + IntCol::rows(NC), R_SNEXT = R_CW + IntCol::rows(NS), R_CHEAD = R_SNEXT + HandleCol::rows(NS),
+                         R_CTAIL = R_CHEAD + HandleCol::rows(NC), R_CN = R_CTAIL + HandleCol::rows(NC), R_CFIRST = R_CN + HandleCol::rows(NC),
+                         R_IA = R_CFIRST + HandleCol::rows(NC), R_IB = R_IA + HandleCol::rows(NC), R_CKEPT = R_IB + HandleCol::rows(NC),
+                         ROWS = R_CKEPT + ByteCol::rows(NC);
+    static __host__ __device__ constexpr size_t bytes() { return (size_t)ROWS * 256; }
+    __device__ __forceinline__ void init(LDS_AS char *slice, int lane)
+    {
+        s_rbeg.init(slice, R_SRBEG, lane); c_pos.init(slice, R_CPOS, lane); s_ql.init(slice, R_SQL, lane); c_rid.init(slice, R_CRID, lane);
+        c_w.init(slice, R_CW, lane); s_next.init(slice, R_SNEXT, lane); c_head.init(slice, R_CHEAD, lane); c_tail.init(slice, R_CTAIL, lane);
+        c_n.init(slice, R_CN, lane); c_first.init(slice, R_CFIRST, lane); ia.init(slice, R_IA, lane); ib.init(slice, R_IB, lane);
+        c_kept.init(slice, R_CKEPT, lane);
+    }
+    __device__ __forceinline__ void bind(const ReadWS &ws) { g = ws; regs = ws.regs; }
+    __device__ __forceinline__ int s_qbeg(int s) const { return QP_HI((qp_t)s_ql[s]); }
+    __device__ __forceinline__ int s_len(int s) const { return QP_LO((qp_t)s_ql[s]); }
+    __device__ __forceinline__ bool full(int ns, int c) const { return ns >= NS || c >= NC; }
+    __device__ __forceinline__ void commit(int ns, int nc) const
+    {
+        for (int s = 0; s < ns; ++s) { g.s_rbeg[s] = s_rbeg[s]; g.s_ql[s] = s_ql[s]; g.s_next[s] = s_next[s]; g.c_w[s] = c_w[s]; }
+        for (int c = 0; c < nc; ++c) {
+            g.c_pos[c] = c_pos[c]; g.c_head[c] = c_head[c]; g.c_n[c] = c_n[c]; g.c_rid[c] = c_rid[c]; g.c_first[c] = c_first[c]; g.ia[c] = ia[c];
+        }
+    }
+};
+
+template <typename I>
+__global__ void __launch_bounds__(64) k_chain_lds(DevFM<I> fm, DevRef R, Chunk ck, DevOpt dopt, const int *order, unsigned int *queue, const unsigned int *n_slots,
+                                                  int *left, unsigned int *n_left, unsigned int *stat)
+{
+    typedef LdsWS<I, CHAIN_LDS_SEEDS> LW;
+    extern __shared__ __attribute__((aligned(16))) unsigned char chain_lds_slice[];
+    const slx_opt &opt = dopt.o;
+    const int n_todo = (int)*n_slots;
+    const int lane = threadIdx.x & 63;
+    LW lw;
+    lw.init((LDS_AS char *)chain_lds_slice, lane);
+    unsigned int n_bail = 0, n_lds = 0;
+    while (true) {
+        const int slot = next_slot(queue);
+        if (__all(slot >= n_todo)) break;
+        if (slot >= n_todo) continue;
+        const int r = order ? order[slot] : slot;
+        const ReadWS ws = make_ws(ck, r);
+        bool done = false;
+        if (ws.cap <= CHAIN_LDS_SEEDS) {
+            lw.bind(ws);
+            done = dev_chain_body<I>(fm, R, ck, opt, r, lw);
+            if (done) ++n_lds; else ++n_bail;
+        }
+        if (!done) left[wave_fetch_inc(n_left)] = r;
+    }
+    for (int d = 32; d; d >>= 1) { n_bail += __shfl_xor(n_bail, d); n_lds += __shfl_xor(n_lds, d); }
+    if (lane == 0) { if (n_bail) atomicAdd(stat, n_bail); if (n_lds) atomicAdd(stat + 1, n_lds); }
+}
+
+#endif
diff --git a/seqlib_amd/csrc/dev_sort.h b/seqlib_amd/csrc/dev_sort.h
--- a/seqlib_amd/csrc/dev_sort.h
+++ b/seqlib_amd/csrc/dev_sort.h
@@ -1,15 +1,15 @@
 #pragma once
 #include <hip/hip_runtime.h>
 
-template <typename LT>
-__device__ void ks_insertsort_idx(int *s, int *t, LT lt)
+template <typename P, typename LT>
+__device__ void ks_insertsort_idx(P s, P t, LT lt)
 {
-    for (int *i = s + 1; i < t; ++i)
-        for (int *j = i; j > s && lt(*j, *(j - 1)); --j) { int sw = *j; *j = *(j - 1); *(j - 1) = sw; }
+    for (P i = s + 1; i < t; ++i)
+        for (P j = i; j > s && lt(*j, *(j - 1)); --j) { int sw = *j; *j = *(j - 1); *(j - 1) = sw; }
 }
 
-template <typename LT>
-__device__ void ks_combsort_idx(int n, int *a, LT lt)
+template <typename P, typename LT>
+__device__ void ks_combsort_idx(int n, P a, LT lt)
 {
     const double shrink = 1.2473309501039786540366528676643;
     int do_swap, gap = n;
@@ -19,16 +19,16 @@
             if (gap == 9 || gap == 10) gap = 11;
         }
         do_swap = 0;
-        for (int *i = a; i < a + n - gap; ++i) {
-            int *j = i + gap;
+        for (P i = a; i < a + (n - gap); ++i) {
+            P j = i + gap;
             if (lt(*j, *i)) { int tmp = *i; *i = *j; *j = tmp; do_swap = 1; }
         }
     } while (do_swap || gap > 2);
     if (gap != 1) ks_insertsort_idx(a, a + n, lt);
 }
 
-template <typename LT>
-__device__ void ks_introsort_idx(int n, int *a, LT lt)
+template <typename P, typename LT>
+__device__ void ks_introsort_idx(int n, P a, LT lt)
 {
     if (n < 1) return;
     if (n == 2) {
diff --git a/seqlib_amd/csrc/slx_align.hip b/seqlib_amd/csrc/slx_align.hip
--- a/seqlib_amd/csrc/slx_align.hip
+++ b/seqlib_amd/csrc/slx_align.hip
@@ -23,6 +23,7 @@
 #include "dev_ext_seg.h"
 #include "dev_fin2.h"
 #include "dev_chain_coop.h"
+#include "dev_chain_lds.h"
 #include "dev_long.h"
 #include "dev_cig_lane.h"
 #include "dev_cig_band.h"
@@ -445,6 +446,7 @@
     else if (!strcmp(key, "cig_lanes")) al->cig_lanes = value != 0;
     else if (!strcmp(key, "first_diag")) al->first_diag = value != 0;
     else if (!strcmp(key, "first_lanes")) al->first_lanes = value != 0;
+    else if (!strcmp(key, "chain_lds")) al->chain_lds = value != 0;
     else if (!strcmp(key, "lane_narrow")) al->lane_narrow = value != 0;
     else if (!strcmp(key, "lane_pad")) al->lane_pad = (int)value;
     else if (!strcmp(key, "cand_lane_seeds")) { if (value < 1) return SLX_EINVAL; al->cand_lane_seeds = (int)value; }
@@ -536,6 +538,13 @@
         if (!strcmp(key, "pseg_jobs")) {
             long long v = 0;
             auto take = [&](const slx_aligner *a) { for (const Worker *wk : a->workers) v += wk->pseg_stat; };
+            if (al->is_group) for (const slx_aligner *sub : al->subs) take(sub); else take(al);
+            return v;
+        }
+        if (!strcmp(key, "chain_lds_bail") || !strcmp(key, "chain_lds_reads")) {
+            long long v = 0;
+            const int which = key[10] == 'r';
+            auto take = [&](const slx_aligner *a) { for (const Worker *wk : a->workers) v += (long long)wk->chain_stat[which]; };
             if (al->is_group) for (const slx_aligner *sub : al->subs) take(sub); else take(al);
             return v;
         }
@@ -612,6 +621,7 @@
     for (int i = 0; i < SLX_N_PROBES; ++i) wk->probe_ms[i] = 0;
     wk->n_chunks = 0;
     for (long long &c : wk->cnt) c = 0;
+    wk->chain_stat[0] = wk->chain_stat[1] = 0;
     int rc;
     const int64_t n_part = r_hi - r_lo;
     if ((rc = wk->o_hit_off.ensure(((size_t)n_part + 1) * 8)) != SLX_OK) return rc;
diff --git a/seqlib_amd/csrc/slx_align_types.h b/seqlib_amd/csrc/slx_align_types.h
--- a/seqlib_amd/csrc/slx_align_types.h
+++ b/seqlib_amd/csrc/slx_align_types.h
@@ -48,7 +48,7 @@
     template <typename T> T *as() const { return (T *)p; }
 };
 
-#define SLX_MAIL_PARTS 6
+#define SLX_MAIL_PARTS 8
 struct MailSpec { const unsigned int *src[SLX_MAIL_PARTS]; int words[SLX_MAIL_PARTS]; int n; };
 static __global__ void k_mail(MailSpec s, unsigned int *dst)
 {
@@ -71,6 +71,7 @@
     DevBuf n_chain, n_reg, n_hit, na, frac_rep, zarena, cigpool, counters, lists, hit_cnt, cig_cnt, hit_off_c, cig_off_c;
     DevBuf order_key_in, order_key_out, order_in, order_out, queues, sort_tmp, jobs, fast_list, dp_list, part_flag, part_pos, cand, cand_base,
         cand_cnt, cand_off, dbg_cyc, order_tmp, first_tab, first_cnt, first_off, fb_list, first_jobs, len_stat, s_score, long_list, long_scratch, huge_rows;
+    DevBuf chain_left;
     DevBuf order_bin, bin_cnt;
     DevBuf defer_list, hits_big;
     DevBuf first_sorted, first_bins;
@@ -83,6 +84,7 @@
     DevBuf gseg_jobs, gseg_units, gseg_wrec, gseg_wout, gseg_scratch, gseg_cnt;
     DevBuf pseg_jobs, pseg_idx, pseg_cnt;
     unsigned long long fin_stat[2] = {0, 0};
+    unsigned long long chain_stat[2] = {0, 0};
     unsigned int pseg_stat = 0;
     unsigned int gseg_stat[3] = {0, 0, 0};
     unsigned int xseg_stat[4] = {0, 0, 0, 0};
@@ -110,7 +112,7 @@
                &c_pos, &c_head, &c_tail, &c_n, &c_rid, &c_w, &c_first, &c_kept, &ia, &ib, &ic, &srt, &regs, &hits, &n_chain, &n_reg, &n_hit,
                &na, &frac_rep, &zarena, &cigpool, &counters, &lists, &hit_cnt, &cig_cnt, &hit_off_c, &cig_off_c, &order_key_in,
                &order_key_out, &order_in, &order_out, &queues, &sort_tmp, &jobs, &fast_list, &dp_list, &part_flag, &part_pos, &cand, &cand_base,
-               &cand_cnt, &cand_off, &dbg_cyc, &order_tmp, &first_tab, &first_cnt, &first_off, &fb_list, &first_jobs, &len_stat, &s_score, &long_list, &long_scratch, &huge_rows, &p2mask, &p2list, &p2items, &p2long, &lane_jobs, &first_dp, &first_sorted, &first_bins, &cig_lane_list, &defer_list, &hits_big, &order_bin, &bin_cnt, &snap_ia, &snap_regs, &snap_nreg,
+               &cand_cnt, &cand_off, &dbg_cyc, &order_tmp, &first_tab, &first_cnt, &first_off, &fb_list, &first_jobs, &len_stat, &s_score, &long_list, &long_scratch, &huge_rows, &p2mask, &p2list, &p2items, &p2long, &lane_jobs, &first_dp, &first_sorted, &first_bins, &cig_lane_list, &defer_list, &hits_big, &order_bin, &bin_cnt, &chain_left, &snap_ia, &snap_regs, &snap_nreg,
                &memo_idx, &memo_jobs, &memo_tab, &round_list, &todo_a, &todo_b, &spec_cnt, &seed3_buf, &job_key_in, &job_key_out, &job_val_in, &job_val_out, &job_sort_tmp, &pseg_jobs, &pseg_idx, &pseg_cnt, &gseg_jobs, &gseg_units, &gseg_wrec, &gseg_wout, &gseg_scratch, &gseg_cnt, &xseg_jobs, &xseg_state, &xseg_units, &xseg_out, &xseg_wrec, &xseg_wout, &xseg_scratch, &xseg_cnt,
                &o_hit_off, &o_rid, &o_pos, &o_flag, &o_mapq, &o_score, &o_nm, &o_na, &o_ncig, &o_cig_off, &o_cigar, &o_xa, &o_sub};
         for (auto &e : ev) e = nullptr;
@@ -162,6 +164,7 @@
     int cand_lane_seeds = 64;
     int cig_lanes = 1;
     int first_lanes = 1;
+    int chain_lds = 1;
     int first_diag = 1;
     int lane_narrow = 1;
     int lane_pad = 0;
diff --git a/seqlib_amd/csrc/slx_chunk.inc b/seqlib_amd/csrc/slx_chunk.inc
--- a/seqlib_amd/csrc/slx_chunk.inc
+++ b/seqlib_amd/csrc/slx_chunk.inc
@@ -500,6 +500,24 @@
 struct CvtI32U64 { __host__ __device__ unsigned long long operator()(int v) const { return (unsigned long long)v; } };
 
 template <typename I>
+static void launch_chain(slx_aligner *al, Worker *wk, const Chunk &ck, const DevOpt &dopt, const DevFM<I> &fm, hipStream_t st, const int *order, unsigned int *q,
+                         const unsigned int *n_slots, int n, int grid, int bs)
+{
+#ifndef SLX_WIDE
+    if (al->chain_lds && !ck.s_score && ck.spread <= 1) {
+        const size_t slice = LdsWS<I, CHAIN_LDS_SEEDS>::bytes();
+        const int waves_cu = std::max(1, (int)((160u << 10) / slice));
+        int *left = wk->chain_left.as<int>();
+        hipLaunchKernelGGL(k_chain_lds<I>, dim3(std::max(1, std::min(n / 64 + 1, al->n_cu * waves_cu))), dim3(64), slice, st, fm, al->ref, ck, dopt, order, q + 0, n_slots,
+                           left, q + 52, q + 50);
+        hipLaunchKernelGGL(k_chain<I>, dim3(grid), dim3(bs), 0, st, fm, al->ref, ck, dopt, (const int *)left, q + 53, (const unsigned int *)(q + 52), 0);
+        return;
+    }
+#endif
+    hipLaunchKernelGGL(k_chain<I>, dim3(grid), dim3(bs), 0, st, fm, al->ref, ck, dopt, order, q + 0, n_slots, ck.spread > 1 ? 1 : 0);
+}
+
+template <typename I>
 static void launch_coop(slx_aligner *al, Worker *wk, const Chunk &ck, const DevOpt &dopt, const DevFM<I> &fm, hipStream_t st, unsigned int *q,
                         unsigned int *counts, int n, bool both_tables = false)
 {
@@ -700,6 +718,7 @@
         unsigned int *q = wk->queues.as<unsigned int>();
         unsigned int *counts = q + 24;
         ENS(part_flag, (size_t)n * 4); ENS(part_pos, (size_t)n * 4); ENS(order_in, (size_t)n * 4); ENS(order_out, (size_t)n * 4);
+        if (al->chain_lds) ENS(chain_left, (size_t)n * 4);
         {
             size_t tb = 0;
             HIPCHK(hipcub::DeviceScan::ExclusiveSum(nullptr, tb, wk->part_flag.as<unsigned int>(), wk->part_pos.as<unsigned int>(), n + 1, st));
@@ -716,12 +735,12 @@
                 HIPCHK(hipcub::DeviceScan::ExclusiveSum(wk->scan_tmp.p, tb, wk->part_flag.as<unsigned int>(), wk->part_pos.as<unsigned int>(), n, st));
                 hipLaunchKernelGGL(k_part_scatter, dim3((unsigned)((n + 255) / 256)), dim3(256), 0, st, wk->part_flag.as<unsigned int>(),
                                    wk->part_pos.as<unsigned int>(), n, wk->order_in.as<int>(), wk->order_out.as<int>(), counts);
-                hipLaunchKernelGGL(k_chain<I>, dim3(spread > 1 ? seed_grid : grid), dim3(bs), 0, st, fm, al->ref, ck, dopt, wk->order_in.as<int>(), q + 0, counts, spread > 1 ? 1 : 0);
+                launch_chain<I>(al, wk, ck, dopt, fm, st, wk->order_in.as<int>(), q, counts, n, spread > 1 ? seed_grid : grid, bs);
                 launch_coop<I>(al, wk, ck, dopt, fm, st, q, counts, n, max_len > 704);
                 hipLaunchKernelGGL(k_set_u32, dim3(1), dim3(1), 0, st, counts, (unsigned int)n);
             } else {
             hipLaunchKernelGGL(k_set_u32, dim3(1), dim3(1), 0, st, counts, (unsigned int)n);
-            hipLaunchKernelGGL(k_chain<I>, dim3(spread > 1 ? seed_grid : grid), dim3(bs), 0, st, fm, al->ref, ck, dopt, (const int *)nullptr, q + 0, counts, spread > 1 ? 1 : 0);
+            launch_chain<I>(al, wk, ck, dopt, fm, st, (const int *)nullptr, q, counts, n, spread > 1 ? seed_grid : grid, bs);
             }
             if (has_long) {
                 hipLaunchKernelGGL(k_long_list, dim3((unsigned)((n + 255) / 256)), dim3(256), 0, st, ck, dopt, wk->long_list.as<int>(), q + 16);
@@ -798,7 +817,7 @@
                                    wk->order_bin.as<int>());
                 light = wk->order_bin.as<int>();
             } else (void)hipGetLastError();
-            hipLaunchKernelGGL(k_chain<I>, dim3(grid), dim3(bs), 0, st, fm, al->ref, ck, dopt, light, q + 0, counts, 0);
+            launch_chain<I>(al, wk, ck, dopt, fm, st, light, q, counts, n, grid, bs);
             launch_coop<I>(al, wk, ck, dopt, fm, st, q, counts, n);
             (void)hipEventRecord(wk->ev_probe[2], st);
             if (use_cand) {
@@ -931,7 +950,8 @@
         ms.src[2] = (const unsigned int *)ck.flags; ms.words[2] = 1;
         ms.src[3] = wk->queues.as<unsigned int>() + 46; ms.words[3] = 1;
         ms.src[4] = wk->queues.as<unsigned int>() + 48; ms.words[4] = 1;
-        ms.n = 5;
+        ms.src[5] = wk->queues.as<unsigned int>() + 50; ms.words[5] = 2;
+        ms.n = 6;
         hipLaunchKernelGGL(k_mail, dim3(1), dim3(64), 0, st, ms, wk->h_mail);
     }
     HIPCHK(slx_wait_stream(st));
@@ -939,6 +959,7 @@
     const uint32_t fl = wk->h_mail[4];
     wk->fin_stat[0] += wk->h_mail[5]; wk->fin_stat[1] += wk->h_mail[6];
     if (fl) { *flags_out = fl; return SLX_OK; }
+    wk->chain_stat[0] += wk->h_mail[7]; wk->chain_stat[1] += wk->h_mail[8];
     const size_t H = (size_t)*hit_base + Hc, C = (size_t)*cig_base + Cc;
 #define GROW(buf, bytes, keep) if ((rc = wk->buf.grow((size_t)(bytes), (size_t)(keep), st)) != SLX_OK) return rc
     GROW(o_rid, (H + 1) * 4, *hit_base * 4); GROW(o_pos, (H + 1) * 8, *hit_base * 8); GROW(o_flag, (H + 1) * 2, *hit_base * 2);
```
